# libvips/libvips

Measured on NVIDIA H100. Metric: Mpixels/s for thumbnail(4K->512,lanczos3), higher is better.
Workload: dtype u8

## Files before the change

include/vb200.h:

```cpp
#ifndef VB200_H
#define VB200_H

#include <stddef.h>
#include <stdint.h>

#ifdef __cplusplus
extern "C" {
#endif


typedef enum {
	VB200_FORMAT_UCHAR = 0,
	VB200_FORMAT_CHAR = 1,
	VB200_FORMAT_USHORT = 2,
	VB200_FORMAT_SHORT = 3,
	VB200_FORMAT_UINT = 4,
	VB200_FORMAT_INT = 5,
	VB200_FORMAT_FLOAT = 6,
	VB200_FORMAT_COMPLEX = 7,
	VB200_FORMAT_DOUBLE = 8,
	VB200_FORMAT_DPCOMPLEX = 9
} VB200BandFormat;

typedef enum {
	VB200_INTERPRETATION_MULTIBAND = 0,
	VB200_INTERPRETATION_B_W = 1,
	VB200_INTERPRETATION_CMYK = 15,
	VB200_INTERPRETATION_XYZ = 12,
	VB200_INTERPRETATION_LAB = 13,
	VB200_INTERPRETATION_LCH = 19,
	VB200_INTERPRETATION_LABS = 21,
	VB200_INTERPRETATION_sRGB = 22,
	VB200_INTERPRETATION_YXY = 23,
	VB200_INTERPRETATION_RGB16 = 25,
	VB200_INTERPRETATION_GREY16 = 26,
	VB200_INTERPRETATION_scRGB = 28,
	VB200_INTERPRETATION_HSV = 29
} VB200Interpretation;

typedef enum {
	VB200_KERNEL_NEAREST = 0,
	VB200_KERNEL_LINEAR = 1,
	VB200_KERNEL_CUBIC = 2,
	VB200_KERNEL_MITCHELL = 3,
	VB200_KERNEL_LANCZOS2 = 4,
	VB200_KERNEL_LANCZOS3 = 5,
	VB200_KERNEL_MKS2013 = 6,
	VB200_KERNEL_MKS2021 = 7
} VB200Kernel;

typedef enum {
	VB200_SIZE_BOTH = 0,
	VB200_SIZE_UP = 1,
	VB200_SIZE_DOWN = 2,
	VB200_SIZE_FORCE = 3
} VB200Size;

typedef enum {
	VB200_PRECISION_INTEGER = 0,
	VB200_PRECISION_FLOAT = 1,
	VB200_PRECISION_APPROXIMATE = 2
} VB200Precision;

typedef enum {
	VB200_HOST = 0,
	VB200_DEVICE = 1
} VB200Where;


typedef struct {
	int left;
	int top;
	int width;
	int height;
} VB200Rect;

typedef struct {
	int Xsize;
	int Ysize;
	int Bands;
	int BandFmt;
	int Type;
	int where;
	void *data;
	size_t bpl;
} VB200Image;

typedef struct {
	VB200Image im;
	VB200Rect valid;
	void *data;
	int bpl;
} VB200Region;


int vb200_init(int device);
void vb200_shutdown(void);
const char *vb200_error_buffer(void);
void vb200_error_clear(void);
int vb200_isenabled(void);
void vb200_set_stream(void *cuda_stream);
void *vb200_get_stream(void);
void vb200_set_tile_geometry(int tile_width, int tile_height, int fatstrip_height, int thinstrip_height);
uint64_t vb200_launch_count(void);
void vb200_image_free(VB200Image *image);
size_t vb200_format_sizeof(int band_format);


int vb200_shrinkv(const VB200Image *in, VB200Image *out, int vshrink, int ceil_mode);
int vb200_shrinkh(const VB200Image *in, VB200Image *out, int hshrink, int ceil_mode);
int vb200_reducev(const VB200Image *in, VB200Image *out, double vshrink, int kernel, double gap);
int vb200_reduceh(const VB200Image *in, VB200Image *out, double hshrink, int kernel, double gap);
int vb200_reduce(const VB200Image *in, VB200Image *out, double hshrink, double vshrink, int kernel, double gap);
int vb200_resize(const VB200Image *in, VB200Image *out, double scale, double vscale, int kernel, double gap);
int vb200_premultiply(const VB200Image *in, VB200Image *out, double max_alpha, int uchar_mode);
int vb200_unpremultiply(const VB200Image *in, VB200Image *out, double max_alpha, int uchar_mode);
int vb200_thumbnail_image(const VB200Image *in, VB200Image *out, int width, int height, int size, int linear);

int vb200_colourspace(const VB200Image *in, VB200Image *out, int space);

typedef struct {
	int width;
	int height;
	const double *coeff;
	double scale;
	double offset;
} VB200Mask;

int vb200_conv(const VB200Image *in, VB200Image *out, const VB200Mask *mask, int precision);
int vb200_convsep(const VB200Image *in, VB200Image *out, const VB200Mask *mask, int precision);
int vb200_gaussblur(const VB200Image *in, VB200Image *out, double sigma, double min_ampl, int precision);
int vb200_gaussmat(VB200Mask *out, double sigma, double min_ampl, int separable, int precision);
void vb200_mask_free(VB200Mask *mask);
int vb200_sharpen(const VB200Image *in, VB200Image *out, double sigma, double x1, double y2, double y3, double m1,
	double m2);
int vb200_sharpen_batch_device(const void *in, size_t in_frame_stride, void *out, size_t out_frame_stride, int n_frames, int width,
	int height, int bands, double sigma, double x1, double y2, double y3, double m1, double m2);
void vb200_set_vector_convi(int on);

typedef struct {
	int n_point;
	int kernel;
	double residual_shrink;
	double offset;
} VB200ReduceParams;

int vb200_reducev_gen(const VB200Region *out, const VB200Region *in, const VB200ReduceParams *params);
int vb200_reduceh_gen(const VB200Region *out, const VB200Region *in, const VB200ReduceParams *params);
int vb200_shrinkv_gen(const VB200Region *out, const VB200Region *in, int vshrink);
int vb200_shrinkh_gen(const VB200Region *out, const VB200Region *in, int hshrink);
int vb200_conv_gen(const VB200Region *out, const VB200Region *in, const VB200Mask *mask, int precision);
int vb200_colour_gen(const VB200Region *out, const VB200Region *in, int space);

void vips_reducev_uchar_hwy(uint8_t *pout, uint8_t *pin, int n, int ne, int lskip, const short *k);
void vips_reduceh_uchar_hwy(uint8_t *pout, uint8_t *pin, int n, int width, int bands, short *cs[65], double X,
	double hshrink);
void vips_shrinkh_uchar_hwy(uint8_t *pout, uint8_t *pin, int width, int hshrink, int bands);
void vips_shrinkv_add_line_uchar_hwy(uint8_t *pin, int ne, unsigned int *sum);
void vips_shrinkv_write_line_uchar_hwy(uint8_t *pout, int ne, int vshrink, unsigned int *sum);

typedef struct VB200ThumbnailPlan VB200ThumbnailPlan;

VB200ThumbnailPlan *vb200_thumbnail_plan_new(int width, int height, int bands, int band_format, int has_alpha,
	int target_width, int target_height, int size, int linear);
void vb200_thumbnail_plan_free(VB200ThumbnailPlan *plan);
int vb200_thumbnail_plan_output(const VB200ThumbnailPlan *plan, int *out_width, int *out_height);
int vb200_thumbnail_batch_device(VB200ThumbnailPlan *plan, const void *in, size_t in_frame_stride, void *out,
	size_t out_frame_stride, int n_frames);
int vb200_thumbnail_batch_host(VB200ThumbnailPlan *plan, const void *in, size_t in_frame_stride, void *out,
	size_t out_frame_stride, int n_frames);
int vb200_thumbnail_plan_set_sharpen(VB200ThumbnailPlan *plan, double sigma, double x1, double y2, double y3, double m1, double m2);
int vb200_thumbnail_plan_is_fused(const VB200ThumbnailPlan *plan);
size_t vb200_thumbnail_plan_bytes_per_frame(const VB200ThumbnailPlan *plan);
const char *vb200_thumbnail_plan_kernel(const VB200ThumbnailPlan *plan);

typedef struct {
	const void *input_profile;
	size_t input_len;
	const void *output_profile;
	size_t output_len;
	const void *builtin_rgb;
	size_t builtin_rgb_len;
	const void *builtin_grey;
	size_t builtin_grey_len;
	int intent;
} VB200ThumbnailIcc;

int vb200_thumbnail_plan_set_icc(VB200ThumbnailPlan *plan, const VB200ThumbnailIcc *icc);
int vb200_thumbnail_plan_output_bands(const VB200ThumbnailPlan *plan);
int vb200_thumbnail_batch_device_icc(VB200ThumbnailPlan *plan, const void *in, size_t in_frame_stride, void *out,
	size_t out_frame_stride, int n_frames, const void *const *embedded, const size_t *embedded_lens);
int vb200_thumbnail_batch_host_icc(VB200ThumbnailPlan *plan, const void *in, size_t in_frame_stride, void *out,
	size_t out_frame_stride, int n_frames, const void *const *embedded, const size_t *embedded_lens);
int vb200_thumbnail_image_icc(const VB200Image *in, VB200Image *out, int width, int height, int size, const VB200ThumbnailIcc *icc,
	const void *embedded, size_t embedded_len);
int vb200_thumbnail_buffer_icc(const void *buf, size_t len, VB200Image *out, int width, int height, int size,
	const VB200ThumbnailIcc *icc);
int vb200_thumbnail_plan_set_linear_icc(VB200ThumbnailPlan *plan, const VB200ThumbnailIcc *icc);
int vb200_thumbnail_image_linear_icc(const VB200Image *in, VB200Image *out, int width, int height, int size,
	const VB200ThumbnailIcc *icc, const void *embedded, size_t embedded_len);
int vb200_thumbnail_buffer_linear_icc(const void *buf, size_t len, VB200Image *out, int width, int height, int size,
	const VB200ThumbnailIcc *icc);
int vb200_debug_icc_select_linear(const VB200ThumbnailIcc *icc, int bands, const void *embedded, size_t embedded_len,
	int *branch, int *source, int *export_from);

int vb200_jpeg_icc_profile(const void *buf, size_t len, void *out, size_t cap, size_t *profile_len);

int vb200_debug_hsv_host(const void *in, size_t n, int to_hsv, void *out);

int vb200_flatten(const VB200Image *in, VB200Image *out, const double *background, int n, double max_alpha);
int vb200_debug_flatten_host(const void *in, int width, int height, int bands, int band_format, int interpretation,
	const double *background, int n, double max_alpha, int x4, void *out);

enum { VB200_MORPHOLOGY_ERODE = 0, VB200_MORPHOLOGY_DILATE = 1 };
int vb200_morph(const VB200Image *in, VB200Image *out, const VB200Mask *mask, int morph);
int vb200_rank(const VB200Image *in, VB200Image *out, int width, int height, int index);
int vb200_median(const VB200Image *in, VB200Image *out, int size);
int vb200_debug_rank_host(const void *in, int width, int height, int bands, int band_format, int rank_width, int rank_height,
	int index, void *out);

typedef struct VB200Chain VB200Chain;
VB200Chain *vb200_chain_new(void);
void vb200_chain_free(VB200Chain *chain);
int vb200_chain_add_resize(VB200Chain *chain, double scale, double vscale, int kernel, double gap);
int vb200_chain_add_reduce(VB200Chain *chain, double hshrink, double vshrink, int kernel, double gap);
int vb200_chain_add_colourspace(VB200Chain *chain, int space);
int vb200_chain_add_conv(VB200Chain *chain, const VB200Mask *mask, int precision);
int vb200_chain_add_convsep(VB200Chain *chain, const VB200Mask *mask, int precision);
int vb200_chain_add_gaussblur(VB200Chain *chain, double sigma, double min_ampl, int precision);
int vb200_chain_add_sharpen(VB200Chain *chain, double sigma, double x1, double y2, double y3, double m1, double m2);
int vb200_chain_add_premultiply(VB200Chain *chain, double max_alpha, int uchar_mode);
int vb200_chain_add_unpremultiply(VB200Chain *chain, double max_alpha, int uchar_mode);
int vb200_chain_add_morph(VB200Chain *chain, const VB200Mask *mask, int morph);
int vb200_chain_add_rank(VB200Chain *chain, int width, int height, int index);
int vb200_chain_add_flatten(VB200Chain *chain, const double *background, int n, double max_alpha);
int vb200_chain_run_host(VB200Chain *chain, const VB200Image *in, VB200Image *out, int n_images);

enum { VB200_INTENT_PERCEPTUAL = 0, VB200_INTENT_RELATIVE = 1, VB200_INTENT_SATURATION = 2, VB200_INTENT_ABSOLUTE = 3 };
enum { VB200_PCS_LAB = 0, VB200_PCS_XYZ = 1 };
int vb200_icc_import(const VB200Image *in, VB200Image *out, const void *profile, size_t profile_len, int intent, int pcs);
int vb200_icc_export(const VB200Image *in, VB200Image *out, const void *profile, size_t profile_len, int intent, int depth,
	int pcs);
int vb200_icc_transform(const VB200Image *in, VB200Image *out, const void *in_profile, size_t in_len,
	const void *out_profile, size_t out_len, int intent, int depth);
int vb200_debug_icc_eval(int mode, const void *in, int in_fmt, int in_bands, void *out, int n, const void *pa, size_t la,
	const void *pb, size_t lb, int intent, int depth, int pcs);
int vb200_debug_icc_select(const VB200ThumbnailIcc *icc, int bands, const void *embedded, size_t embedded_len, int *source);
int vb200_debug_icc_classify(const void *profile, size_t len, int want_bands, int intent);
float vb200_debug_icc_stage_ms(void);
float vb200_debug_linear_thumb_ms(void);

int vb200_debug_mma_tables(int in_size, double shrink, int rect_size, int *int_shrink, int *shrunk_size, int *out_size,
	int *n_point, int *embed, int *first, int *phase, short *mask65, int *vchunk, unsigned *bfrag, int cap_rows,
	int *rows_per_chunk);

int vb200_debug_thumbnail_bands(int width, int height, int target_width, int *out_width, int *n_bands, int *xa, int *xb,
	int *c_lo, int *c_hi, int *seam, int cap, int *box_width, int *n_box);
int vb200_debug_thumbnail_kernel(int width, int height, int bands, int has_alpha, int target_width, int target_height, int size,
	char *name, int cap);

int vb200_jpeg_decode_batch(const void *const *bufs, const size_t *lens, int n, int shrink, void *out, int out_location,
	size_t out_bpl, size_t out_frame_stride, int *width, int *height, int *bands);
int vb200_jpegload_buffer(const void *buf, size_t len, int shrink, VB200Image *out);
int vb200_thumbnail_jpegshrink(int width, int height, int target_width, int target_height, int size);
int vb200_thumbnail_buffer(const void *buf, size_t len, VB200Image *out, int width, int height, int size);
int vb200_thumbnail_plan_run_jpeg(VB200ThumbnailPlan *plan, const void *const *bufs, const size_t *lens, int n, int shrink,
	void *out, int out_location, size_t out_frame_stride);
int vb200_debug_jpeg_decode(const void *buf, size_t len, int shrink, void *out, size_t out_bpl, int *width, int *height,
	int *bands);
int vb200_debug_jpeg_decode_sync(const void *buf, size_t len, int shrink, int sub_bytes, int max_passes, void *out, size_t out_bpl,
	int *width, int *height, int *bands, int *passes_used);
int vb200_jpegsave_batch(const void *frames, int frames_location, size_t bpl, size_t frame_stride, int n, int width, int height, int bands,
	int Q, int subsample_mode, void *out, int out_location, size_t out_stride, size_t *lengths);
typedef struct {
	int Q;
	int subsample_mode;
	int optimize_coding;
	int restart_interval;
	int interlace;
} VB200JpegSaveOptions;
int vb200_jpegsave_batch_opts(const void *frames, int frames_location, size_t bpl, size_t frame_stride, int n, int width, int height,
	int bands, const VB200JpegSaveOptions *options, void *out, int out_location, size_t out_stride, size_t *lengths);
int vb200_debug_jpeg_encode(const void *pixels, size_t bpl, int width, int height, int bands, int quality, int subsample_mode, void *out,
	size_t cap, size_t *len);
int vb200_debug_jpeg_encode_opts(const void *pixels, size_t bpl, int width, int height, int bands, const VB200JpegSaveOptions *options,
	void *out, size_t cap, size_t *len);
int vb200_debug_jpeg_prog_events(const void *pixels, size_t bpl, int width, int height, int bands, const VB200JpegSaveOptions *options,
	unsigned long long *events);
int vb200_debug_jpeg_optimal_table(const unsigned *freq, unsigned char *bits, unsigned char *huffval);
void vb200_debug_jpeg_times(float *huffman_ms, float *idct_ms);

enum { VB200_DZ_LAYOUT_DZ = 0, VB200_DZ_LAYOUT_ZOOMIFY = 1, VB200_DZ_LAYOUT_GOOGLE = 2, VB200_DZ_LAYOUT_IIIF = 3, VB200_DZ_LAYOUT_IIIF3 = 4 };
enum { VB200_DZ_DEPTH_DEFAULT = 0, VB200_DZ_DEPTH_ONEPIXEL = 1, VB200_DZ_DEPTH_ONETILE = 2, VB200_DZ_DEPTH_ONE = 3 };
typedef struct {
	int layout;
	int tile_size;
	int overlap;
	int depth;
	int region_shrink;
	int skip_blanks;
	int container;
	const char *suffix;
	VB200JpegSaveOptions jpeg;
} VB200DzOptions;

typedef struct VB200DzPyramid VB200DzPyramid;

int vb200_dzsave(const VB200Image *in, const VB200DzOptions *options, VB200DzPyramid **out);
int vb200_debug_dzsave(const VB200Image *in, const VB200DzOptions *options, VB200DzPyramid **out);
void vb200_dz_free(VB200DzPyramid *pyramid);
int vb200_dz_levels(const VB200DzPyramid *pyramid);
int vb200_dz_level_geometry(const VB200DzPyramid *pyramid, int n, int *width, int *height, int *tiles_across, int *tiles_down);
long vb200_dz_tiles(const VB200DzPyramid *pyramid);
int vb200_dz_tile(const VB200DzPyramid *pyramid, long i, int *level, int *x, int *y, int *left, int *top, int *width, int *height,
	const void **stream, size_t *len);
int vb200_dz_tile_name(const VB200DzPyramid *pyramid, long i, const char *basename, char *name, size_t cap);
int vb200_dz_sidecar(const VB200DzPyramid *pyramid, const char *basename, char *name, size_t ncap, char *text, size_t tcap, size_t *len);
int vb200_dz_pyramid_level(const VB200Image *in, int n_from_top, VB200Image *out);
int vb200_debug_dz_pyramid_level(const void *pixels, size_t bpl, int width, int height, int bands, int n_from_top, void *out);
void vb200_debug_dz_set_budget(size_t bytes);
size_t vb200_debug_dz_pool_used(void);
void vb200_debug_dz_times(float *ms);

void *vb200_host_alloc(size_t bytes);
void vb200_host_free(void *p);
int vb200_device_numa_node(void);

#ifdef __cplusplus
}
#endif

#endif
```

libvips_b200/csrc/thumbnail_fused.cu:

```cuda
#include <algorithm>
#include <climits>
#include <cmath>
#include <cstring>
#include <map>
#include <memory>
#include <mutex>
#include <vector>

#include <cuda.h>

#include "vb200_internal.h"

namespace vb200 {

namespace {

constexpr int kChunkRows = 8;
constexpr int kMaxThreads = 576;

struct FusedParams {
	int W, H;
	size_t in_bpl;
	int VS;
	int Hs;
	int vembed;
	int NPv;
	unsigned vmul8;
	int vshift;
	unsigned accmul;
	int HS, Ws, hembed, NPh;
	unsigned hmul8;
	int hshift;
	int OW, OH;
	size_t out_bpl;
	int TW;
	int RPC;
	int NT;
	int NEmax;
	int slots;
	int stage_pitch;
	int vgrid, hgrid;
	const int2 *vrow;
	const int2 *hcol;
	const int *vcoef;
	const int *hcoef;
	int nvsets, nhsets;
	const int2 *vchunk;
	const uint4 *vbfrag;
	int mma_rows;
	int premul;
	const unsigned char *opaque_hint;
	double max_alpha;
};

struct MmaBand {
	int xa, xb, ne, c_lo, c_hi;
};

__device__ __forceinline__ int
dp2a_lo(unsigned coef, unsigned bytes, int acc)
{
	int d;
	asm("dp2a.lo.s32.u32 %0, %1, %2, %3;" : "=r"(d) : "r"(coef), "r"(bytes), "r"(acc));
	return d;
}

__device__ __forceinline__ int
dp2a_hi(unsigned coef, unsigned bytes, int acc)
{
	int d;
	asm("dp2a.hi.s32.u32 %0, %1, %2, %3;" : "=r"(d) : "r"(coef), "r"(bytes), "r"(acc));
	return d;
}

__device__ __forceinline__ unsigned
ld_stream(const unsigned *p)
{
	unsigned v;
	asm volatile("ld.global.nc.L1::no_allocate.u32 %0, [%1];" : "=r"(v) : "l"(p));
	return v;
}

template <int VS, bool PREMUL>
__device__ __forceinline__ void
box_rows(const unsigned (&px)[VS], int vs, const int *pscale, bool lut, unsigned amend2, unsigned &rb, unsigned &ga)
{
	rb = amend2;
	ga = amend2;
#pragma unroll
	for (int k = 0; k < VS; k++) {
		const unsigned x = px[k];
		if (PREMUL) {
			const unsigned a = x >> 24;
			const unsigned s = lut ? (unsigned) pscale[a] : a + (a == 255u);
			const unsigned prb = (((x & 0x00ff00ffu) * s + 0x00800080u) >> 8) & 0x00ff00ffu;
			const unsigned pg = ((((x >> 8) & 0xffu) * s + 128u) >> 8) & 0xffu;
			rb += prb;
			ga += pg + (a << 16);
		}
		else {
			rb += x & 0x00ff00ffu;
			ga += (x >> 8) & 0x00ff00ffu;
		}
	}
}

__device__ __forceinline__ unsigned
box_average(unsigned lanes, unsigned mul8, int shift)
{
	if (shift >= 0)
		return (lanes >> shift) & 0x00ff00ffu;
	const unsigned lo = __umulhi(lanes & 0xffffu, mul8);
	const unsigned hi = __umulhi(lanes >> 16, mul8);
	return lo | (hi << 16);
}

template <int VS, bool PREMUL>
__global__ void __launch_bounds__(kMaxThreads, 2)
thumbnail_fused_kernel(const __grid_constant__ FusedParams P, const uint8_t *__restrict__ in, size_t in_frame_stride,
	uint8_t *__restrict__ out, size_t out_frame_stride, int frame0)
{
	extern __shared__ __align__(128) unsigned char smem_raw[];

	const int NT = P.NT;
	const int t = threadIdx.x;
	const int vs = VS > 0 ? VS : P.VS;

	uint2 *pairbuf = (uint2 *) smem_raw;
	unsigned *rv = (unsigned *) (pairbuf + (size_t) P.slots * NT);
	uint2 *sh = (uint2 *) (rv + (size_t) kChunkRows * NT);
	int *vcoef = (int *) (sh + (size_t) kChunkRows * (P.NEmax / 2));
	int *hcoef = vcoef + P.nvsets * P.NPv;
	int *pscale = hcoef + P.nhsets * P.NPh;
	int *uscale = pscale + 256;

	for (int i = t; i < P.nvsets * P.NPv; i += NT)
		vcoef[i] = P.vcoef[i];
	for (int i = t; i < P.nhsets * P.NPh; i += NT)
		hcoef[i] = P.hcoef[i];
	if (PREMUL)
		for (int i = t; i < 256; i += NT) {
			const double clip = fmax(0.0, fmin(P.max_alpha, (double) i));
			pscale[i] = (int) __ddiv_rn(__dmul_rn(256.0, clip), P.max_alpha);
			uscale[i] = clip == 0 ? 0 : (int) __ddiv_rn(__dmul_rn(256.0, P.max_alpha), clip);
		}
	const bool lut = PREMUL && P.max_alpha != 255.0;

	const int xa = blockIdx.x * P.TW;
	const int xb = min(xa + P.TW, P.OW);
	const int y_begin = blockIdx.y * P.RPC;
	const int y_end = min(y_begin + P.RPC, P.OH);
	const int frame = frame0 + blockIdx.z;
	const uint8_t *fin = in + (size_t) frame * in_frame_stride;
	uint8_t *fout = out + (size_t) frame * out_frame_stride;

	const int pair_h0 = __ldg(&P.hcol[xa]).x;
	const int E0 = 2 * pair_h0 + P.hgrid;
	const int NE = 2 * (__ldg(&P.hcol[xb - 1]).x + P.NPh - pair_h0);

	const bool col_active = t < NE * P.HS;
	int in_col;
	{
		const int e = E0 + t / P.HS;
		const int k = t - (t / P.HS) * P.HS;
		const int sc = max(0, min(e - P.hembed, P.Ws - 1));
		in_col = min(sc * P.HS + k, P.W - 1);
	}
	const unsigned *col_ptr = (const unsigned *) fin + in_col;

	const unsigned amend2 = (unsigned) (vs / 2) * 0x00010001u;

	__syncthreads();

	int pdone = INT_MIN;
	int P0_prev = 0;

	for (int ya = y_begin; ya < y_end; ya += kChunkRows) {
		const int yb = min(ya + kChunkRows, y_end);
		const int P0 = __ldg(&P.vrow[ya]).x;
		const int P1 = __ldg(&P.vrow[yb - 1]).x + P.NPv - 1;

		if (col_active) {
			int pfirst = P0;
			if (pdone > P0) {
				const int shift = P0 - P0_prev;
				if (shift > 0)
					for (int p = P0; p < pdone; p++)
						pairbuf[(size_t) (p - P0) * NT + t] = pairbuf[(size_t) (p - P0 + shift) * NT + t];
				pfirst = pdone;
			}

			for (int p = pfirst; p <= P1; p++) {
				unsigned rbA, gaA, rbB, gaB;
				const int sA = max(0, min(2 * p + P.vgrid - P.vembed, P.Hs - 1));
				const int sB = max(0, min(2 * p + P.vgrid + 1 - P.vembed, P.Hs - 1));
				if (VS > 0) {
					unsigned pa[VS > 0 ? VS : 1], pb[VS > 0 ? VS : 1];
#pragma unroll
					for (int k = 0; k < VS; k++) {
						const int ra = min(sA * VS + k, P.H - 1);
						const int rb_ = min(sB * VS + k, P.H - 1);
						pa[k] = ld_stream((const unsigned *) ((const char *) col_ptr + (size_t) ra * P.in_bpl));
						pb[k] = ld_stream((const unsigned *) ((const char *) col_ptr + (size_t) rb_ * P.in_bpl));
					}
					box_rows<(VS > 0 ? VS : 1), PREMUL>(pa, vs, pscale, lut, amend2, rbA, gaA);
					box_rows<(VS > 0 ? VS : 1), PREMUL>(pb, vs, pscale, lut, amend2, rbB, gaB);
				}
				else {
					rbA = gaA = rbB = gaB = amend2;
					for (int k = 0; k < vs; k++) {
						unsigned one[1], rb1, ga1;
						one[0] = ld_stream((const unsigned *) ((const char *) col_ptr + (size_t) min(sA * vs + k, P.H - 1) * P.in_bpl));
						box_rows<1, PREMUL>(one, 1, pscale, lut, 0u, rb1, ga1);
						rbA += rb1;
						gaA += ga1;
						one[0] = ld_stream((const unsigned *) ((const char *) col_ptr + (size_t) min(sB * vs + k, P.H - 1) * P.in_bpl));
						box_rows<1, PREMUL>(one, 1, pscale, lut, 0u, rb1, ga1);
						rbB += rb1;
						gaB += ga1;
					}
				}
				rbA = box_average(rbA, P.vmul8, P.vshift);
				gaA = box_average(gaA, P.vmul8, P.vshift);
				rbB = box_average(rbB, P.vmul8, P.vshift);
				gaB = box_average(gaB, P.vmul8, P.vshift);
				uint2 w;
				w.x = __byte_perm(rbA, rbB, 0x6240);
				w.y = __byte_perm(gaA, gaB, 0x6240);
				pairbuf[(size_t) (p - P0) * NT + t] = w;
			}

			for (int y = ya; y < yb; y++) {
				const int2 vr = __ldg(&P.vrow[y]);
				const uint2 *win = pairbuf + (size_t) (vr.x - P0) * NT + t;
				const int *cf = vcoef + vr.y * P.NPv;
				int r = VB200_INTERPOLATE_SCALE >> 1, g = r, b = r, a = r;
#pragma unroll 7
				for (int k = 0; k < P.NPv; k++) {
					const uint2 w = win[(size_t) k * NT];
					const unsigned c = (unsigned) cf[k];
					r = dp2a_lo(c, w.x, r);
					b = dp2a_hi(c, w.x, b);
					g = dp2a_lo(c, w.y, g);
					a = dp2a_hi(c, w.y, a);
				}
				r = max(0, min(r >> VB200_INTERPOLATE_SHIFT, 255));
				g = max(0, min(g >> VB200_INTERPOLATE_SHIFT, 255));
				b = max(0, min(b >> VB200_INTERPOLATE_SHIFT, 255));
				a = max(0, min(a >> VB200_INTERPOLATE_SHIFT, 255));
				rv[(size_t) (y - ya) * NT + t] = (unsigned) r | ((unsigned) g << 8) | ((unsigned) b << 16) | ((unsigned) a << 24);
			}
		}
		pdone = P1 + 1;
		P0_prev = P0;

		__syncthreads();

		const int rows = yb - ya;
		const int npairs = NE / 2;
		const unsigned hamend2 = (unsigned) (P.HS / 2) * 0x00010001u;
		for (int idx = t; idx < rows * npairs; idx += NT) {
			const int k = idx / npairs;
			const int j = idx - k * npairs;
			const unsigned *src = rv + (size_t) k * NT + (size_t) (2 * j) * P.HS;
			unsigned rbA = hamend2, gaA = hamend2, rbB = hamend2, gaB = hamend2;
			for (int i = 0; i < P.HS; i++) {
				const unsigned wA = src[i];
				const unsigned wB = src[P.HS + i];
				rbA += wA & 0x00ff00ffu;
				gaA += (wA >> 8) & 0x00ff00ffu;
				rbB += wB & 0x00ff00ffu;
				gaB += (wB >> 8) & 0x00ff00ffu;
			}
			rbA = box_average(rbA, P.hmul8, P.hshift);
			gaA = box_average(gaA, P.hmul8, P.hshift);
			rbB = box_average(rbB, P.hmul8, P.hshift);
			gaB = box_average(gaB, P.hmul8, P.hshift);
			uint2 w;
			w.x = __byte_perm(rbA, rbB, 0x6240);
			w.y = __byte_perm(gaA, gaB, 0x6240);
			sh[(size_t) k * (P.NEmax / 2) + j] = w;
		}

		__syncthreads();

		const int bw = xb - xa;
		for (int idx = t; idx < rows * bw; idx += NT) {
			const int k = idx / bw;
			const int x = xa + (idx - k * bw);
			const int2 hc = __ldg(&P.hcol[x]);
			const uint2 *win = sh + (size_t) k * (P.NEmax / 2) + (hc.x - pair_h0);
			const int *cf = hcoef + hc.y * P.NPh;
			int r = VB200_INTERPOLATE_SCALE >> 1, g = r, b = r, a = r;
#pragma unroll 7
			for (int kk = 0; kk < P.NPh; kk++) {
				const uint2 w = win[kk];
				const unsigned c = (unsigned) cf[kk];
				r = dp2a_lo(c, w.x, r);
				b = dp2a_hi(c, w.x, b);
				g = dp2a_lo(c, w.y, g);
				a = dp2a_hi(c, w.y, a);
			}
			r = max(0, min(r >> VB200_INTERPOLATE_SHIFT, 255));
			g = max(0, min(g >> VB200_INTERPOLATE_SHIFT, 255));
			b = max(0, min(b >> VB200_INTERPOLATE_SHIFT, 255));
			a = max(0, min(a >> VB200_INTERPOLATE_SHIFT, 255));
			if (PREMUL) {
				const int s = uscale[a];
				r = ((r * s + 128) >> 8) & 0xff;
				g = ((g * s + 128) >> 8) & 0xff;
				b = ((b * s + 128) >> 8) & 0xff;
			}
			*(unsigned *) (fout + (size_t) (ya + k) * P.out_bpl + (size_t) x * 4) =
				(unsigned) r | ((unsigned) g << 8) | ((unsigned) b << 16) | ((unsigned) a << 24);
		}
	}
}


constexpr int kStages = 3;
constexpr int kChunkRowsTma = 4;
constexpr int kColsPerThread = 2;
constexpr int kStagePitch = (kMaxThreads + 8) * 4;

__device__ __forceinline__ unsigned
smem_addr(const void *p)
{
	return (unsigned) __cvta_generic_to_shared(p);
}

__device__ __forceinline__ void
mbar_init(unsigned bar, unsigned count)
{
	asm volatile("mbarrier.init.shared::cta.b64 [%0], %1;" ::"r"(bar), "r"(count));
}

__device__ __forceinline__ void
mbar_wait(unsigned bar, unsigned parity)
{
	unsigned done;
	do {
		asm volatile("{\n\t.reg .pred p;\n\t"
					 "mbarrier.try_wait.parity.shared::cta.b64 p, [%1], %2, 0x989680;\n\t"
					 "selp.u32 %0, 1, 0, p;\n\t}"
					 : "=r"(done)
					 : "r"(bar), "r"(parity)
					 : "memory");
	} while (!done);
}

__device__ __forceinline__ void
mbar_arrive(unsigned bar)
{
	asm volatile("{\n\t.reg .b64 st;\n\tmbarrier.arrive.shared::cta.b64 st, [%0];\n\t}" ::"r"(bar) : "memory");
}

__device__ __forceinline__ void
mbar_expect_tx(unsigned bar, unsigned bytes)
{
	asm volatile("{\n\t.reg .b64 st;\n\tmbarrier.arrive.expect_tx.shared::cta.b64 st, [%0], %1;\n\t}" ::"r"(bar), "r"(bytes)
				 : "memory");
}

__device__ __forceinline__ void
bulk_copy_g2s(unsigned dst, const void *src, unsigned bytes, unsigned bar)
{
	asm volatile("cp.async.bulk.shared::cluster.global.mbarrier::complete_tx::bytes [%0], [%1], %2, [%3];" ::"r"(dst),
				 "l"(src), "r"(bytes), "r"(bar)
				 : "memory");
}

__device__ __forceinline__ int
fast_div(int idx, int d)
{
	int q = (int) (__int2float_rn(idx) * __frcp_rn(__int2float_rn(d)));
	const int r = idx - q * d;
	q += (r >= d) - (r < 0);
	return q;
}

__device__ __forceinline__ void
consumer_barrier(int n_threads)
{
	asm volatile("bar.sync 1, %0;" ::"r"(n_threads) : "memory");
}

template <bool PREMUL>
__device__ __forceinline__ void
accumulate_pixel(unsigned x, unsigned &rb, unsigned &ga)
{
	if (PREMUL) {
		const unsigned a = x >> 24;
		const unsigned s = (a * 257u + 1u) >> 8;
		const unsigned trb = (x & 0x00ff00ffu) * s + 0x00800080u;
		const unsigned tg = __byte_perm(x, 0, 0x4441) * s + 128u;
		rb += __byte_perm(trb, 0, 0x4341);
		ga += __byte_perm(tg, x, 0x3731);
	}
	else {
		rb += x & 0x00ff00ffu;
		ga += __byte_perm(x, 0, 0x4341);
	}
}

__device__ __forceinline__ unsigned
average_pair(unsigned lanesA, unsigned lanesB, unsigned mul8, int shift)
{
	if (shift >= 0)
		return __byte_perm(lanesA >> shift, lanesB >> shift, 0x6240);
	const unsigned a = __umulhi(lanesA & 0xffffu, mul8) | (__umulhi(lanesA >> 16, mul8) << 16);
	const unsigned b = __umulhi(lanesB & 0xffffu, mul8) | (__umulhi(lanesB >> 16, mul8) << 16);
	return __byte_perm(a, b, 0x6240);
}

__device__ __forceinline__ unsigned
hadd2_lanes(unsigned a, unsigned b)
{
	unsigned d;
	asm("add.f16x2 %0, %1, %2;" : "=r"(d) : "r"(a), "r"(b));
	return d;
}

template <bool PREMUL>
__device__ __forceinline__ void
accumulate_pixel_h(unsigned x, unsigned k16, unsigned &rb, unsigned &ga)
{
	if (PREMUL) {
		unsigned t0;
		asm("lop3.b32 %0, %1, 0xff000000, %2, 0xea;" : "=r"(t0) : "r"(x), "r"(k16));
		const unsigned s = __umulhi(t0, 257u);
		const unsigned trb = (x & 0x00ff00ffu) * s + 0x00800080u;
		const unsigned tg = (x & 0x0000ff00u) * s + 0x00008000u;
		rb = hadd2_lanes(rb, __byte_perm(trb, 0, 0x4341));
		ga = hadd2_lanes(ga, __byte_perm(tg, x, 0x3732));
	}
	else {
		rb = hadd2_lanes(rb, x & 0x00ff00ffu);
		ga = hadd2_lanes(ga, __byte_perm(x, 0, 0x4341));
	}
}

__device__ __forceinline__ unsigned
finalize_pack(int r, int g, int b, int a)
{
	r = max(0, min(r >> VB200_INTERPOLATE_SHIFT, 255));
	g = max(0, min(g >> VB200_INTERPOLATE_SHIFT, 255));
	b = max(0, min(b >> VB200_INTERPOLATE_SHIFT, 255));
	a = max(0, min(a >> VB200_INTERPOLATE_SHIFT, 255));
	return (unsigned) r + (unsigned) g * 256u + (unsigned) b * 65536u + (unsigned) a * 16777216u;
}

template <int VS, int NP, bool PREMUL, int CPT>
__global__ void __launch_bounds__(kMaxThreads / CPT + 32, 2)
thumbnail_fused_tma_kernel(const __grid_constant__ FusedParams P, const uint8_t *__restrict__ in, size_t in_frame_stride,
	uint8_t *__restrict__ out, size_t out_frame_stride, int frame0)
{
	extern __shared__ __align__(128) unsigned char smem_raw[];

	constexpr int K = kChunkRowsTma;
	constexpr int NPR = NP > 0 ? NP : 1;
	constexpr int VSR = VS > 0 ? VS : 1;
	const int NT = P.NT;
	const int NC = NT * CPT;
	const int t = threadIdx.x;
	const int vs = VS > 0 ? VS : P.VS;
	const int NPv = NP > 0 ? NP : P.NPv;
	const int NPh = NP > 0 ? NP : P.NPh;
	const int rows_per_stage = 2 * vs;
	const unsigned stage_bytes = (unsigned) rows_per_stage * kStagePitch;

	unsigned char *stages = smem_raw;
	uint64_t *bars = (uint64_t *) (smem_raw + kStages * stage_bytes);
	uint2 *pairbuf = (uint2 *) (bars + 2 * kStages);
	unsigned *rv = (unsigned *) (pairbuf + (size_t) P.slots * NC);
	uint2 *sh = (uint2 *) (rv + (size_t) K * NC);
	int *vcoef = (int *) (sh + (size_t) K * (P.NEmax / 2));
	int *hcoef = vcoef + P.nvsets * P.NPv;
	int *uscale = hcoef + P.nhsets * P.NPh;

	const unsigned stages_s = smem_addr(stages);
	const unsigned full_s = smem_addr(bars);
	const unsigned empty_s = full_s + 8u * kStages;

	if (t == 0) {
		for (int i = 0; i < kStages; i++) {
			mbar_init(full_s + 8u * i, 1);
			mbar_init(empty_s + 8u * i, NT / 32);
		}
		asm volatile("fence.mbarrier_init.release.cluster;" ::: "memory");
	}
	for (int i = t; i < P.nvsets * P.NPv; i += blockDim.x)
		vcoef[i] = P.vcoef[i];
	for (int i = t; i < P.nhsets * P.NPh; i += blockDim.x)
		hcoef[i] = P.hcoef[i];
	if (PREMUL)
		for (int i = t; i < 256; i += blockDim.x)
			uscale[i] = i == 0 ? 0 : (int) __ddiv_rn(__dmul_rn(256.0, 255.0), (double) i);

	const int xa = blockIdx.x * P.TW;
	const int xb = min(xa + P.TW, P.OW);
	const int y_begin = blockIdx.y * P.RPC;
	const int y_end = min(y_begin + P.RPC, P.OH);
	const int frame = frame0 + blockIdx.z;
	const uint8_t *fin = in + (size_t) frame * in_frame_stride;
	uint8_t *fout = out + (size_t) frame * out_frame_stride;

	const int pair_h0 = __ldg(&P.hcol[xa]).x;
	const int E0 = 2 * pair_h0 + P.hgrid;
	const int NE = 2 * (__ldg(&P.hcol[xb - 1]).x + P.NPh - pair_h0);

	auto column_of = [&](int tt) {
		const int e = E0 + tt / P.HS;
		const int k = tt - (tt / P.HS) * P.HS;
		const int sc = max(0, min(e - P.hembed, P.Ws - 1));
		return min(sc * P.HS + k, P.W - 1);
	};
	const int c_lo = column_of(0) & ~3;
	const int c_hi = min(P.W, (column_of(NE * P.HS - 1) + 4) & ~3);
	const unsigned row_bytes = (unsigned) (c_hi - c_lo) * 4u;

	__syncthreads();

	if (t >= NT) {
		const int lane = t - NT;
		const uint8_t *src0 = fin + (size_t) c_lo * 4;
		const int j = lane / vs, k = lane - j * vs;
		const bool copier = lane < rows_per_stage;
		int s = 0;
		unsigned phase = 0;
		int pdone = INT_MIN;
		for (int ya = y_begin; ya < y_end; ya += K) {
			const int yb = min(ya + K, y_end);
			const int P0 = __ldg(&P.vrow[ya]).x;
			const int P1 = __ldg(&P.vrow[yb - 1]).x + P.NPv - 1;
			for (int p = max(pdone, P0); p <= P1; p++) {
				mbar_wait(empty_s + 8u * s, phase ^ 1u);
				if (lane == 0)
					mbar_expect_tx(full_s + 8u * s, (unsigned) rows_per_stage * row_bytes);
				__syncwarp();
				if (copier) {
					const int sr = max(0, min(2 * p + P.vgrid + j - P.vembed, P.Hs - 1));
					const int row = min(sr * vs + k, P.H - 1);
					bulk_copy_g2s(stages_s + (unsigned) s * stage_bytes + (unsigned) lane * kStagePitch,
						src0 + (size_t) row * P.in_bpl, row_bytes, full_s + 8u * s);
				}
				if (++s == kStages) {
					s = 0;
					phase ^= 1u;
				}
			}
			pdone = P1 + 1;
		}
		return;
	}

	const unsigned char *my_col[CPT];
#pragma unroll
	for (int i = 0; i < CPT; i++)
		my_col[i] = stages + (size_t) (column_of(min(t * CPT + i, NE * P.HS - 1)) - c_lo) * 4u;
	const unsigned amend2 = (unsigned) (vs / 2) * 0x00010001u;
	const bool lane0 = (t & 31) == 0;
	const unsigned vmul8 = P.vmul8;
	const int vshift = VS == 1 ? 0 : VS == 2 ? 1 : VS == 4 ? 2 : VS == 8 ? 3 : P.vshift;
	const int tc = t * CPT;

	int s = 0;
	unsigned phase = 0;
	int pdone = INT_MIN;
	int P0_prev = 0;
	int cset = -1;
	unsigned cf[NPR];

	for (int ya = y_begin; ya < y_end; ya += K) {
		const int yb = min(ya + K, y_end);
		const int P0 = __ldg(&P.vrow[ya]).x;
		const int P1 = __ldg(&P.vrow[yb - 1]).x + P.NPv - 1;

		int pfirst = P0;
		if (pdone > P0) {
			const int shift = P0 - P0_prev;
			if (shift > 0) {
				const int cnt = pdone - P0;
				uint2 *dstp = pairbuf + tc;
				const uint2 *srcp = pairbuf + shift * NC + tc;
#pragma unroll 4
				for (int i = 0; i < cnt; i++) {
					if (CPT == 2)
						*(uint4 *) (dstp + i * NC) = *(const uint4 *) (srcp + i * NC);
					else
						dstp[i * NC] = srcp[i * NC];
				}
			}
			pfirst = pdone;
		}

		uint2 *pdst = pairbuf + (pfirst - P0) * NC + tc;
		for (int p = pfirst; p <= P1; p++, pdst += NC) {
			const unsigned soff = (unsigned) s * stage_bytes;
			unsigned rbA[CPT], gaA[CPT], rbB[CPT], gaB[CPT];
#pragma unroll
			for (int i = 0; i < CPT; i++)
				rbA[i] = gaA[i] = rbB[i] = gaB[i] = amend2;
			mbar_wait(full_s + 8u * s, phase);
			if (VS > 0) {
				unsigned pa[CPT][VSR], pb[CPT][VSR];
#pragma unroll
				for (int i = 0; i < CPT; i++)
#pragma unroll
					for (int k = 0; k < VSR; k++) {
						pa[i][k] = *(const unsigned *) (my_col[i] + soff + k * kStagePitch);
						pb[i][k] = *(const unsigned *) (my_col[i] + soff + (VSR + k) * kStagePitch);
					}
				__syncwarp();
				if (lane0)
					mbar_arrive(empty_s + 8u * s);
#pragma unroll
				for (int i = 0; i < CPT; i++)
#pragma unroll
					for (int k = 0; k < VSR; k++) {
						accumulate_pixel<PREMUL>(pa[i][k], rbA[i], gaA[i]);
						accumulate_pixel<PREMUL>(pb[i][k], rbB[i], gaB[i]);
					}
			}
			else {
				for (int k = 0; k < vs; k++)
#pragma unroll
					for (int i = 0; i < CPT; i++) {
						accumulate_pixel<PREMUL>(*(const unsigned *) (my_col[i] + soff + k * kStagePitch), rbA[i], gaA[i]);
						accumulate_pixel<PREMUL>(*(const unsigned *) (my_col[i] + soff + (vs + k) * kStagePitch), rbB[i], gaB[i]);
					}
				__syncwarp();
				if (lane0)
					mbar_arrive(empty_s + 8u * s);
			}
			if (++s == kStages) {
				s = 0;
				phase ^= 1u;
			}
			uint2 w[CPT];
#pragma unroll
			for (int i = 0; i < CPT; i++) {
				w[i].x = average_pair(rbA[i], rbB[i], vmul8, vshift);
				w[i].y = average_pair(gaA[i], gaB[i], vmul8, vshift);
			}
			if (CPT == 2)
				*(uint4 *) pdst = make_uint4(w[0].x, w[0].y, w[CPT - 1].x, w[CPT - 1].y);
			else
				*pdst = w[0];
		}

		unsigned *rvp = rv + tc;
		for (int y = ya; y < yb; y++, rvp += NC) {
			const int2 vr = __ldg(&P.vrow[y]);
			const uint2 *win = pairbuf + (vr.x - P0) * NC + tc;
			int acc[CPT][4];
#pragma unroll
			for (int i = 0; i < CPT; i++)
				acc[i][0] = acc[i][1] = acc[i][2] = acc[i][3] = VB200_INTERPOLATE_SCALE >> 1;
			if (NP > 0) {
				if (vr.y != cset) {
					cset = vr.y;
#pragma unroll
					for (int k = 0; k < NPR; k++)
						cf[k] = (unsigned) vcoef[cset * NPR + k];
				}
#pragma unroll
				for (int k = 0; k < NPR; k++) {
					uint2 w[CPT];
					if (CPT == 2) {
						const uint4 q = *(const uint4 *) (win + k * NC);
						w[0] = make_uint2(q.x, q.y);
						w[CPT - 1] = make_uint2(q.z, q.w);
					}
					else
						w[0] = win[k * NC];
#pragma unroll
					for (int i = 0; i < CPT; i++) {
						acc[i][0] = dp2a_lo(cf[k], w[i].x, acc[i][0]);
						acc[i][2] = dp2a_hi(cf[k], w[i].x, acc[i][2]);
						acc[i][1] = dp2a_lo(cf[k], w[i].y, acc[i][1]);
						acc[i][3] = dp2a_hi(cf[k], w[i].y, acc[i][3]);
					}
				}
			}
			else {
				const int *cfp = vcoef + vr.y * NPv;
				for (int k = 0; k < NPv; k++) {
					const unsigned c = (unsigned) cfp[k];
#pragma unroll
					for (int i = 0; i < CPT; i++) {
						const uint2 w = win[k * NC + i];
						acc[i][0] = dp2a_lo(c, w.x, acc[i][0]);
						acc[i][2] = dp2a_hi(c, w.x, acc[i][2]);
						acc[i][1] = dp2a_lo(c, w.y, acc[i][1]);
						acc[i][3] = dp2a_hi(c, w.y, acc[i][3]);
					}
				}
			}
			if (CPT == 2)
				*(uint2 *) rvp = make_uint2(finalize_pack(acc[0][0], acc[0][1], acc[0][2], acc[0][3]),
					finalize_pack(acc[CPT - 1][0], acc[CPT - 1][1], acc[CPT - 1][2], acc[CPT - 1][3]));
			else
				*rvp = finalize_pack(acc[0][0], acc[0][1], acc[0][2], acc[0][3]);
		}
		pdone = P1 + 1;
		P0_prev = P0;

		consumer_barrier(NT);

		const int rows = yb - ya;
		const int npairs = NE / 2;
		const unsigned hamend2 = (unsigned) (P.HS / 2) * 0x00010001u;
		for (int idx = t; idx < rows * npairs; idx += NT) {
			const int k = fast_div(idx, npairs);
			const int j = idx - k * npairs;
			const unsigned *src = rv + k * NC + (2 * j) * P.HS;
			unsigned rbA = hamend2, gaA = hamend2, rbB = hamend2, gaB = hamend2;
			if (P.HS == 4) {
				const uint4 A = *(const uint4 *) src;
				const uint4 B = *(const uint4 *) (src + 4);
				rbA += (A.x & 0x00ff00ffu) + (A.y & 0x00ff00ffu) + (A.z & 0x00ff00ffu) + (A.w & 0x00ff00ffu);
				gaA += __byte_perm(A.x, 0, 0x4341) + __byte_perm(A.y, 0, 0x4341) + __byte_perm(A.z, 0, 0x4341) +
					__byte_perm(A.w, 0, 0x4341);
				rbB += (B.x & 0x00ff00ffu) + (B.y & 0x00ff00ffu) + (B.z & 0x00ff00ffu) + (B.w & 0x00ff00ffu);
				gaB += __byte_perm(B.x, 0, 0x4341) + __byte_perm(B.y, 0, 0x4341) + __byte_perm(B.z, 0, 0x4341) +
					__byte_perm(B.w, 0, 0x4341);
			}
			else
				for (int i = 0; i < P.HS; i++) {
					const unsigned wA = src[i];
					const unsigned wB = src[P.HS + i];
					rbA += wA & 0x00ff00ffu;
					gaA += __byte_perm(wA, 0, 0x4341);
					rbB += wB & 0x00ff00ffu;
					gaB += __byte_perm(wB, 0, 0x4341);
				}
			uint2 w;
			w.x = average_pair(rbA, rbB, P.hmul8, P.hshift);
			w.y = average_pair(gaA, gaB, P.hmul8, P.hshift);
			sh[k * (P.NEmax / 2) + j] = w;
		}

		consumer_barrier(NT);

		const int bw = xb - xa;
		for (int idx = t; idx < rows * bw; idx += NT) {
			const int k = fast_div(idx, bw);
			const int x = xa + (idx - k * bw);
			const int2 hc = __ldg(&P.hcol[x]);
			const uint2 *win = sh + k * (P.NEmax / 2) + (hc.x - pair_h0);
			const int *cfp = hcoef + hc.y * NPh;
			int r = VB200_INTERPOLATE_SCALE >> 1, g = r, b = r, a = r;
			if (NP > 0) {
#pragma unroll
				for (int kk = 0; kk < NPR; kk++) {
					const uint2 w = win[kk];
					const unsigned c = (unsigned) cfp[kk];
					r = dp2a_lo(c, w.x, r);
					b = dp2a_hi(c, w.x, b);
					g = dp2a_lo(c, w.y, g);
					a = dp2a_hi(c, w.y, a);
				}
			}
			else
				for (int kk = 0; kk < NPh; kk++) {
					const uint2 w = win[kk];
					const unsigned c = (unsigned) cfp[kk];
					r = dp2a_lo(c, w.x, r);
					b = dp2a_hi(c, w.x, b);
					g = dp2a_lo(c, w.y, g);
					a = dp2a_hi(c, w.y, a);
				}
			r = max(0, min(r >> VB200_INTERPOLATE_SHIFT, 255));
			g = max(0, min(g >> VB200_INTERPOLATE_SHIFT, 255));
			b = max(0, min(b >> VB200_INTERPOLATE_SHIFT, 255));
			a = max(0, min(a >> VB200_INTERPOLATE_SHIFT, 255));
			if (PREMUL) {
				const int sc = uscale[a];
				r = ((r * sc + 128) >> 8) & 0xff;
				g = ((g * sc + 128) >> 8) & 0xff;
				b = ((b * sc + 128) >> 8) & 0xff;
			}
			*(unsigned *) (fout + (size_t) (ya + k) * P.out_bpl + (size_t) x * 4) =
				(unsigned) r | ((unsigned) g << 8) | ((unsigned) b << 16) | ((unsigned) a << 24);
		}
	}
}

#include "thumbnail_fused_mma.cuh"

#define VB200_V4_LIST(X) \
	X(4, 6, 4) X(4, 7, 4) X(2, 6, 2) X(2, 7, 2) X(8, 6, 8) X(8, 7, 8) \
	X(4, 0, 4) X(2, 0, 2) X(4, 0, 2) X(2, 0, 4) X(4, 0, 8) X(2, 0, 8) X(8, 0, 8) X(8, 0, 4) \
	X(3, 0, 3) X(5, 0, 5) X(6, 0, 6) X(7, 0, 7) X(2, 0, 3) X(3, 0, 2) X(3, 0, 4) X(4, 0, 3) \
	X(4, 0, 5) X(5, 0, 4) X(5, 0, 6) X(6, 0, 5) X(6, 0, 7) X(7, 0, 6) X(7, 0, 8) X(8, 0, 7)

int
v4_np(int vs, int nph, int hs)
{
	int np = -1;
#define X(VS_, NP_, HS_) \
	if (vs == VS_ && hs == HS_ && (NP_ == nph || (NP_ == 0 && np < 0))) \
		np = NP_;
	VB200_V4_LIST(X)
#undef X
	return np;
}

struct PairSets {
	int NP = 0;
	std::vector<int> coef;
	std::map<std::pair<int, int>, int> ids;

	int
	get(const AxisTable &t, int phase, int parity)
	{
		auto key = std::make_pair(phase, parity);
		auto it = ids.find(key);
		if (it != ids.end())
			return it->second;
		const int id = (int) ids.size();
		ids[key] = id;
		const short *c = &t.ms[(size_t) phase * t.n_point];
		for (int k = 0; k < NP; k++) {
			const int i0 = 2 * k - parity, i1 = 2 * k + 1 - parity;
			const int c0 = (i0 >= 0 && i0 < t.n_point) ? c[i0] : 0;
			const int c1 = (i1 >= 0 && i1 < t.n_point) ? c[i1] : 0;
			coef.push_back((int) (((unsigned) (c0 & 0xffff)) | ((unsigned) (c1 & 0xffff) << 16)));
		}
		return id;
	}

	void
	trim()
	{
		const int nsets = (int) ids.size();
		int keep = 1;
		for (int s = 0; s < nsets; s++)
			for (int k = 0; k < NP; k++)
				if (coef[(size_t) s * NP + k] != 0)
					keep = std::max(keep, k + 1);
		if (keep == NP)
			return;
		std::vector<int> packed;
		for (int s = 0; s < nsets; s++)
			for (int k = 0; k < keep; k++)
				packed.push_back(coef[(size_t) s * NP + k]);
		coef.swap(packed);
		NP = keep;
	}
};

}


struct LinearThumb;
int linear_thumb_new(const char *domain, int W, int H, int bands, bool premul, const ReduceGeom &gv, const ReduceGeom &gh,
	const AxisTable &tv, const AxisTable &th, LinearThumb **out);
int linear_thumb_run(const char *domain, LinearThumb *lt, const void *in, size_t in_stride, void *out, size_t out_stride, int n,
	cudaStream_t s, const LinIccBatch *icc = nullptr, int out_bands = 0);
void linear_thumb_free(LinearThumb *lt);

enum class FusedKernel {
	Ldg,
	Tma,
	Mma,
};

struct ThumbnailPlanImpl {
	int W = 0, H = 0, bands = 0, fmt = 0, has_alpha = 0;
	int target_w = 0, target_h = 0, size = 0, linear = 0;
	double hshrink = 1, vshrink = 1;
	int OW = 0, OH = 0;
	ReduceGeom gv{}, gh{};
	bool premul = false;
	bool fused = false;
	int device = -1;
	FusedKernel kernel = FusedKernel::Ldg;
	FusedParams fp{};
	void *tables = nullptr;
	size_t smem = 0;
	int slots_tma = 0;
	size_t smem_tma = 0;
	int mma_tw = 0, mma_nt = 0, mma_nemax = 0;
	std::vector<MmaBand> mma_bands;
	size_t smem_mma = 0;
	bool geometry_only = false;
	void *tables_mma = nullptr;
	static constexpr int kStreams = 3;
	cudaStream_t streams[kStreams] = {nullptr, nullptr, nullptr};
	void *stage_in[kStreams] = {nullptr, nullptr, nullptr};
	void *stage_out[kStreams] = {nullptr, nullptr, nullptr};
	cudaEvent_t drained[kStreams] = {nullptr, nullptr, nullptr};
	int stage_frames = 0;
	std::mutex pump_lock;
	static constexpr int kHintSlots = 4;
	std::mutex hint_lock;
	int *hint_counts = nullptr;
	cudaEvent_t hint_done[kHintSlots] = {nullptr, nullptr, nullptr, nullptr};
	bool hint_pending[kHintSlots] = {false, false, false, false};
	unsigned hint_slot_seq[kHintSlots] = {0, 0, 0, 0};
	unsigned hint_seq = 0, hint_seen = 0;
	bool opaque_mode = false;
	bool rgb_expand = false;
	LinearThumb *lin = nullptr;
	bool sharpen = false;
	double sh_sigma = 0.5, sh_x1 = 2.0, sh_y2 = 10.0, sh_y3 = 20.0, sh_m1 = 0.0, sh_m2 = 3.0;
	IccStage *icc = nullptr;
	int icc_bands = 0;
	IccStage *licc = nullptr;
	int licc_bands = 0;
	size_t stage_out_frame = 0;
	int out_bands() const { return icc ? icc_bands : licc ? licc_bands : bands; }
};

int dev_sharpen_fused(const char *domain, const void *in, size_t in_bpl, size_t in_frame_stride, void *out, size_t out_bpl,
	size_t out_frame_stride, int n_frames, int w, int h, int bands, double sigma, double x1, double y2, double y3, double m1,
	double m2, cudaStream_t s);

namespace {

void
thumbnail_shrink(int w, int h, int tw, int th, int size, double *hshrink, double *vshrink)
{
	double hs = (double) w / tw;
	double vs = (double) h / th;
	const bool horizontal = !(hs < vs);
	if (size != VB200_SIZE_FORCE) {
		if (horizontal)
			vs = hs;
		else
			hs = vs;
	}
	if (size == VB200_SIZE_UP) {
		hs = std::min(1.0, hs);
		vs = std::min(1.0, vs);
	}
	else if (size == VB200_SIZE_DOWN) {
		hs = std::max(1.0, hs);
		vs = std::max(1.0, vs);
	}
	*hshrink = std::min(hs, (double) w);
	*vshrink = std::min(vs, (double) h);
}

int
launch_status(const char *domain, const char *what)
{
	const cudaError_t e = cudaGetLastError();
	if (e != cudaSuccess)
		return cuda_fail(domain, e, what);
	count_launch();
	return 0;
}

int
rows_per_cta(int OH, int k, int min_chunks, int bands_x, int n, int ctas)
{
	int rpc = ((OH + k - 1) / k) * k;
	while ((long long) bands_x * ((OH + rpc - 1) / rpc) * n < ctas && rpc > min_chunks * k)
		rpc = ((rpc / 2 + k - 1) / k) * k;
	return rpc;
}

template <int VS, bool PREMUL>
int
launch_ldg_t(const char *domain, const FusedParams &fp, size_t smem, const void *in, size_t in_stride, void *out,
	size_t out_stride, int f0, dim3 grid, cudaStream_t s)
{
	auto kern = thumbnail_fused_kernel<VS, PREMUL>;
	VB200_CUDA(domain, cudaFuncSetAttribute(kern, cudaFuncAttributeMaxDynamicSharedMemorySize, (int) smem));
	kern<<<grid, fp.NT, smem, s>>>(fp, (const uint8_t *) in, in_stride, (uint8_t *) out, out_stride, f0);
	return launch_status(domain, "thumbnail_fused_kernel launch");
}

template <bool PREMUL>
int
launch_ldg_vs(const char *domain, const FusedParams &fp, size_t smem, const void *in, size_t is, void *out, size_t os, int f0,
	dim3 grid, cudaStream_t s)
{
	switch (fp.VS) {
	case 1: return launch_ldg_t<1, PREMUL>(domain, fp, smem, in, is, out, os, f0, grid, s);
	case 2: return launch_ldg_t<2, PREMUL>(domain, fp, smem, in, is, out, os, f0, grid, s);
	case 3: return launch_ldg_t<3, PREMUL>(domain, fp, smem, in, is, out, os, f0, grid, s);
	case 4: return launch_ldg_t<4, PREMUL>(domain, fp, smem, in, is, out, os, f0, grid, s);
	case 5: return launch_ldg_t<5, PREMUL>(domain, fp, smem, in, is, out, os, f0, grid, s);
	case 6: return launch_ldg_t<6, PREMUL>(domain, fp, smem, in, is, out, os, f0, grid, s);
	case 8: return launch_ldg_t<8, PREMUL>(domain, fp, smem, in, is, out, os, f0, grid, s);
	default: return launch_ldg_t<0, PREMUL>(domain, fp, smem, in, is, out, os, f0, grid, s);
	}
}

int
launch_ldg(const char *domain, const ThumbnailPlanImpl *pl, const void *in, size_t is, void *out, size_t os, int n, int f0,
	int nf, cudaStream_t s)
{
	FusedParams fp = pl->fp;
	const int bands_x = (pl->OW + fp.TW - 1) / fp.TW;
	fp.RPC = rows_per_cta(pl->OH, kChunkRows, 2, bands_x, n, 2 * sm_count());
	const dim3 grid(bands_x, (pl->OH + fp.RPC - 1) / fp.RPC, nf);
	return pl->premul ? launch_ldg_vs<true>(domain, fp, pl->smem, in, is, out, os, f0, grid, s)
					  : launch_ldg_vs<false>(domain, fp, pl->smem, in, is, out, os, f0, grid, s);
}

template <int VS, int NP, bool PREMUL>
int
launch_tma_t(const char *domain, const FusedParams &fp, size_t smem, const void *in, size_t in_stride, void *out,
	size_t out_stride, int f0, dim3 grid, cudaStream_t s)
{
	auto kern = thumbnail_fused_tma_kernel<VS, NP, PREMUL, kColsPerThread>;
	VB200_CUDA(domain, cudaFuncSetAttribute(kern, cudaFuncAttributeMaxDynamicSharedMemorySize, (int) smem));
	kern<<<grid, fp.NT + 32, smem, s>>>(fp, (const uint8_t *) in, in_stride, (uint8_t *) out, out_stride, f0);
	return launch_status(domain, "thumbnail_fused_tma_kernel launch");
}

template <int NP, bool PREMUL>
int
launch_tma_vs(const char *domain, const FusedParams &fp, size_t smem, const void *in, size_t is, void *out, size_t os, int f0,
	dim3 grid, cudaStream_t s)
{
	switch (fp.VS) {
	case 1: return launch_tma_t<1, NP, PREMUL>(domain, fp, smem, in, is, out, os, f0, grid, s);
	case 2: return launch_tma_t<2, NP, PREMUL>(domain, fp, smem, in, is, out, os, f0, grid, s);
	case 3: return launch_tma_t<3, NP, PREMUL>(domain, fp, smem, in, is, out, os, f0, grid, s);
	case 4: return launch_tma_t<4, NP, PREMUL>(domain, fp, smem, in, is, out, os, f0, grid, s);
	case 8: return launch_tma_t<8, NP, PREMUL>(domain, fp, smem, in, is, out, os, f0, grid, s);
	default: return launch_tma_t<0, NP, PREMUL>(domain, fp, smem, in, is, out, os, f0, grid, s);
	}
}

int
launch_tma(const char *domain, const ThumbnailPlanImpl *pl, const void *in, size_t is, void *out, size_t os, int n, int f0,
	int nf, cudaStream_t s)
{
	FusedParams fp = pl->fp;
	fp.slots = pl->slots_tma;
	fp.NT = ((pl->fp.NT / kColsPerThread + 31) / 32) * 32;
	const int bands_x = (pl->OW + fp.TW - 1) / fp.TW;
	fp.RPC = rows_per_cta(pl->OH, kChunkRowsTma, 4, bands_x, n, 2 * sm_count());
	const dim3 grid(bands_x, (pl->OH + fp.RPC - 1) / fp.RPC, nf);
	const size_t smem = pl->smem_tma;
	const int np = fp.NPv == fp.NPh ? fp.NPv : 0;
	if (np == 6)
		return pl->premul ? launch_tma_vs<6, true>(domain, fp, smem, in, is, out, os, f0, grid, s)
						  : launch_tma_vs<6, false>(domain, fp, smem, in, is, out, os, f0, grid, s);
	if (np == 7)
		return pl->premul ? launch_tma_vs<7, true>(domain, fp, smem, in, is, out, os, f0, grid, s)
						  : launch_tma_vs<7, false>(domain, fp, smem, in, is, out, os, f0, grid, s);
	return pl->premul ? launch_tma_vs<0, true>(domain, fp, smem, in, is, out, os, f0, grid, s)
					  : launch_tma_vs<0, false>(domain, fp, smem, in, is, out, os, f0, grid, s);
}

bool
make_stage_tensor_map(CUtensorMap *tm, const void *in, int W, int H, size_t in_bpl, size_t frame_stride, int frames,
	int box_cols, int box_rows)
{
	typedef CUresult (*encode_fn)(CUtensorMap *, CUtensorMapDataType, cuuint32_t, void *, const cuuint64_t *,
		const cuuint64_t *, const cuuint32_t *, const cuuint32_t *, CUtensorMapInterleave, CUtensorMapSwizzle,
		CUtensorMapL2promotion, CUtensorMapFloatOOBfill);
	static encode_fn encode = nullptr;
	static bool tried = false;
	if (!tried) {
		tried = true;
		void *fn = nullptr;
		cudaDriverEntryPointQueryResult qres;
		if (cudaGetDriverEntryPoint("cuTensorMapEncodeTiled", &fn, cudaEnableDefault, &qres) == cudaSuccess &&
			qres == cudaDriverEntryPointSuccess)
			encode = (encode_fn) fn;
		cudaGetLastError();
	}
	if (!encode || getenv("VB200_NO_TENSORMAP"))
		return false;
	if ((W & 1) || (in_bpl % 16) || (frame_stride % 16) || ((uintptr_t) in % 16) || box_cols / 2 > 256 || box_rows > 256)
		return false;
	const cuuint64_t dims[3] = {(cuuint64_t) W / 2, (cuuint64_t) H, (cuuint64_t) frames};
	const cuuint64_t strides[2] = {(cuuint64_t) in_bpl, (cuuint64_t) frame_stride};
	const cuuint32_t box[3] = {(cuuint32_t) box_cols / 2, (cuuint32_t) box_rows, 1};
	const cuuint32_t estr[3] = {1, 1, 1};
	return encode(tm, CU_TENSOR_MAP_DATA_TYPE_UINT64, 3, const_cast<void *>(in), dims, strides, box, estr,
			   CU_TENSOR_MAP_INTERLEAVE_NONE, CU_TENSOR_MAP_SWIZZLE_NONE, CU_TENSOR_MAP_L2_PROMOTION_L2_256B,
			   CU_TENSOR_MAP_FLOAT_OOB_FILL_NONE) == CUDA_SUCCESS;
}

constexpr int kHintThreads = 128, kHintSamples = 2;

__global__ void __launch_bounds__(kHintThreads)
alpha_hint_kernel(const uint8_t *__restrict__ in, size_t in_frame_stride, size_t in_bpl, int W, int H, unsigned char *__restrict__ hint,
	int *__restrict__ count)
{
	const uint8_t *f = in + (size_t) blockIdx.x * in_frame_stride;
	const unsigned npix = (unsigned) W * (unsigned) H;
	int opaque = 0;
#pragma unroll
	for (int i = 0; i < kHintSamples; i++) {
		const unsigned k = (unsigned) (threadIdx.x * kHintSamples + i);
		const unsigned p = (unsigned) (((unsigned long long) (k * 2654435761u) * npix) >> 32);
		const unsigned y = p / (unsigned) W, x = p - y * (unsigned) W;
		opaque += f[(size_t) y * in_bpl + (size_t) x * 4 + 3] == 255;
	}
	__shared__ int s_sum;
	if (threadIdx.x == 0)
		s_sum = 0;
	__syncthreads();
	opaque = __reduce_add_sync(0xffffffffu, opaque);
	if ((threadIdx.x & 31) == 0)
		atomicAdd(&s_sum, opaque);
	__syncthreads();
	if (threadIdx.x == 0) {
		const int h = s_sum * 4 >= kHintThreads * kHintSamples ? 1 : 0;
		hint[blockIdx.x] = (unsigned char) h;
		if (h)
			atomicAdd(count, 1);
	}
}

int
opaque_hint_begin(const char *domain, ThumbnailPlanImpl *pl, const FusedParams &fp, const void *in, size_t in_stride, int n,
	cudaStream_t s, void **hint, bool *use_opq)
{
	*hint = nullptr;
	*use_opq = false;
	const char *probe_env = getenv("VB200_OPAQUE_PROBE");
	if (!pl->premul || (probe_env && probe_env[0] == '0'))
		return 0;
	{
		std::lock_guard<std::mutex> lock(pl->hint_lock);
		if (!pl->hint_counts) {
			if (cudaHostAlloc((void **) &pl->hint_counts, sizeof(int) * ThumbnailPlanImpl::kHintSlots, cudaHostAllocDefault) != cudaSuccess) {
				cudaGetLastError();
				pl->hint_counts = nullptr;
				return 0;
			}
			for (int i = 0; i < ThumbnailPlanImpl::kHintSlots; i++)
				cudaEventCreateWithFlags(&pl->hint_done[i], cudaEventDisableTiming);
		}
		for (int i = 0; i < ThumbnailPlanImpl::kHintSlots; i++)
			if (pl->hint_pending[i] && cudaEventQuery(pl->hint_done[i]) == cudaSuccess) {
				pl->hint_pending[i] = false;
				if (pl->hint_slot_seq[i] + 1 > pl->hint_seen) {
					pl->hint_seen = pl->hint_slot_seq[i] + 1;
					pl->opaque_mode = pl->hint_counts[i] > 0;
				}
			}
		cudaGetLastError();
		*use_opq = pl->opaque_mode || (probe_env && probe_env[0] == '2');
	}
	const size_t count_off = ((size_t) n + 3) & ~(size_t) 3;
	if (dev_alloc(domain, hint, count_off + sizeof(int), s))
		return -1;
	int *count = (int *) ((char *) *hint + count_off);
	VB200_CUDA(domain, cudaMemsetAsync(count, 0, sizeof(int), s));
	alpha_hint_kernel<<<n, kHintThreads, 0, s>>>((const uint8_t *) in, in_stride, fp.in_bpl, fp.W, fp.H, (unsigned char *) *hint, count);
	cudaError_t e = cudaGetLastError();
	if (e != cudaSuccess) {
		dev_free(*hint, s);
		*hint = nullptr;
		return cuda_fail(domain, e, "alpha_hint_kernel launch");
	}
	count_launch();
	return 0;
}

void
opaque_hint_end(ThumbnailPlanImpl *pl, void *hint, int n, cudaStream_t s)
{
	if (!hint)
		return;
	{
		std::lock_guard<std::mutex> lock(pl->hint_lock);
		const int slot = (int) (pl->hint_seq % ThumbnailPlanImpl::kHintSlots);
		if (!pl->hint_pending[slot]) {
			const int *count = (const int *) ((const char *) hint + (((size_t) n + 3) & ~(size_t) 3));
			if (cudaMemcpyAsync(&pl->hint_counts[slot], count, sizeof(int), cudaMemcpyDeviceToHost, s) == cudaSuccess &&
				cudaEventRecord(pl->hint_done[slot], s) == cudaSuccess) {
				pl->hint_pending[slot] = true;
				pl->hint_slot_seq[slot] = pl->hint_seq;
			}
			cudaGetLastError();
		}
		pl->hint_seq++;
	}
	dev_free(hint, s);
}

template <int VS, int NP, bool PREMUL, int HSQ, bool OPQ>
int
launch_mma_k(const char *domain, const ThumbnailPlanImpl *pl, const FusedParams &fp, const CUtensorMap &tm, int use_tmap, const void *in,
	size_t in_stride, void *out, size_t out_stride, int f0, dim3 grid, cudaStream_t s)
{
	auto kern = thumbnail_fused_mma_kernel<VS, NP, PREMUL, HSQ, OPQ>;
	VB200_CUDA(domain, cudaFuncSetAttribute(kern, cudaFuncAttributeMaxDynamicSharedMemorySize, (int) pl->smem_mma));
	kern<<<grid, fp.NT + 32 * kV4HWarps + 32, pl->smem_mma, s>>>(fp, tm, use_tmap, (const uint8_t *) in, in_stride,
		(uint8_t *) out, out_stride, f0);
	return launch_status(domain, "thumbnail_fused_mma_kernel launch");
}

template <int VS, int NP, bool PREMUL, int HSQ>
int
launch_mma_t(const char *domain, ThumbnailPlanImpl *pl, FusedParams fp, const void *in, size_t in_stride, void *out,
	size_t out_stride, int n, int f0, dim3 grid, cudaStream_t s)
{
	CUtensorMap tm;
	memset(&tm, 0, sizeof(tm));
	const int use_tmap = make_stage_tensor_map(&tm, in, fp.W, fp.H, fp.in_bpl, in_stride, n, v4_boxw(HSQ), 2 * VS) ? 1 : 0;
	void *hint = nullptr;
	bool use_opq = false;
	if (PREMUL && opaque_hint_begin(domain, pl, fp, (const uint8_t *) in + (size_t) f0 * in_stride, in_stride, (int) grid.z, s, &hint, &use_opq))
		return -1;
	fp.opaque_hint = (const unsigned char *) hint;
	int rc;
	if constexpr (PREMUL)
		rc = use_opq ? launch_mma_k<VS, NP, PREMUL, HSQ, true>(domain, pl, fp, tm, use_tmap, in, in_stride, out, out_stride, f0, grid, s)
					 : launch_mma_k<VS, NP, PREMUL, HSQ, false>(domain, pl, fp, tm, use_tmap, in, in_stride, out, out_stride, f0, grid, s);
	else
		rc = launch_mma_k<VS, NP, PREMUL, HSQ, false>(domain, pl, fp, tm, use_tmap, in, in_stride, out, out_stride, f0, grid, s);
	opaque_hint_end(pl, hint, (int) grid.z, s);
	return rc;
}

template <bool PREMUL>
int
launch_mma_list(const char *domain, ThumbnailPlanImpl *pl, const FusedParams &fp, const void *in, size_t is, void *out, size_t os,
	int n, int f0, dim3 grid, cudaStream_t s)
{
	const int np = v4_np(fp.VS, fp.NPh, fp.HS);
#define X(VS_, NP_, HS_) \
	if (fp.VS == VS_ && np == NP_ && fp.HS == HS_) \
		return launch_mma_t<VS_, NP_, PREMUL, HS_>(domain, pl, fp, in, is, out, os, n, f0, grid, s);
	VB200_V4_LIST(X)
#undef X
	error(domain, "the tensor-pipe kernel has no instantiation for VS %d, HS %d", fp.VS, fp.HS);
	return -1;
}

int
launch_mma(const char *domain, ThumbnailPlanImpl *pl, const void *in, size_t is, void *out, size_t os, int n, int f0, int nf,
	cudaStream_t s)
{
	FusedParams fp = pl->fp;
	fp.TW = pl->mma_tw;
	fp.NT = pl->mma_nt;
	fp.NEmax = pl->mma_nemax;
	const int bands_x = (pl->OW + fp.TW - 1) / fp.TW;
	fp.RPC = rows_per_cta(pl->OH, fp.mma_rows, 4, bands_x, n, sm_count());
	const dim3 grid(bands_x, (pl->OH + fp.RPC - 1) / fp.RPC, nf);
	return pl->premul ? launch_mma_list<true>(domain, pl, fp, in, is, out, os, n, f0, grid, s)
					  : launch_mma_list<false>(domain, pl, fp, in, is, out, os, n, f0, grid, s);
}

void
plan_axis_tables(const ThumbnailPlanImpl *pl, AxisTable &tv, AxisTable &th)
{
	const TileGeometry tg = tile_geometry();
	int tile_w, tile_h;
	if (pl->gv.int_shrink > 1) {
		tile_w = tg.tile_width;
		tile_h = tg.tile_height;
	}
	else {
		tile_w = pl->OW;
		tile_h = tg.fatstrip_height;
	}
	int rect_h = tile_h;
	if (pl->gh.int_shrink > 1)
		rect_h = std::min(rect_h, tg.fatstrip_height);
	build_axis_table(tv, pl->OH, pl->gv.residual, pl->gv.offset, pl->gv.n_point, VB200_KERNEL_LANCZOS3, rect_h);
	build_axis_table(th, pl->OW, pl->gh.residual, pl->gh.offset, pl->gh.n_point, VB200_KERNEL_LANCZOS3, tile_w);
}

std::vector<MmaBand>
mma_bands_of(const FusedParams &fp, const std::vector<int2> &hcol, int tw, int clo_align)
{
	auto column_of = [&](int E0, int tt) {
		const int e = E0 + tt / fp.HS;
		const int k = tt % fp.HS;
		const int sc = std::max(0, std::min(e - fp.hembed, fp.Ws - 1));
		return std::min(sc * fp.HS + k, fp.W - 1);
	};
	std::vector<MmaBand> bands;
	for (int xa = 0; xa < fp.OW; xa += tw) {
		MmaBand b;
		b.xa = xa;
		b.xb = std::min(xa + tw, fp.OW);
		const int E0 = 2 * hcol[xa].x + fp.hgrid;
		b.ne = 2 * (hcol[b.xb - 1].x + fp.NPh - hcol[xa].x);
		b.c_lo = column_of(E0, 0) & ~(clo_align - 1);
		b.c_hi = std::min(fp.W, (column_of(E0, b.ne * fp.HS - 1) + 4) & ~3);
		bands.push_back(b);
	}
	return bands;
}

int
plan_build_fused(const char *domain, ThumbnailPlanImpl *pl)
{
	AxisTable tv, th;
	plan_axis_tables(pl, tv, th);

	auto build_sets = [](const AxisTable &t, int count, int grid, PairSets &sets, std::vector<int2> &idx) {
		sets = PairSets();
		sets.NP = (t.n_point + 2) / 2;
		idx.resize(count);
		for (int i = 0; i < count; i++) {
			const int rel = t.first[i] - grid;
			idx[i].x = rel >> 1;
			idx[i].y = sets.get(t, t.phase[i], rel & 1);
		}
		sets.trim();
	};
	PairSets sv, shh;
	std::vector<int2> vrow, hcol;
	int vgrid = 0, hgrid = 0;
	{
		PairSets alt;
		std::vector<int2> alt_idx;
		build_sets(tv, pl->OH, 0, sv, vrow);
		build_sets(tv, pl->OH, 1, alt, alt_idx);
		if (alt.NP < sv.NP) {
			sv = alt;
			vrow = alt_idx;
			vgrid = 1;
		}
		build_sets(th, pl->OW, 0, shh, hcol);
		build_sets(th, pl->OW, 1, alt, alt_idx);
		if (alt.NP < shh.NP) {
			shh = alt;
			hcol = alt_idx;
			hgrid = 1;
		}
	}

	FusedParams &fp = pl->fp;
	fp.W = pl->W;
	fp.H = pl->H;
	fp.in_bpl = (size_t) pl->W * 4;
	fp.VS = pl->gv.int_shrink;
	fp.Hs = pl->gv.shrunk_size;
	fp.vembed = tv.embed;
	fp.NPv = sv.NP;
	fp.vgrid = vgrid;
	fp.hgrid = hgrid;
	fp.vmul8 = (unsigned) (((1LL << 32) / (256LL * fp.VS)) << 8);
	fp.vshift = -1;
	fp.accmul = 1;
	for (int sft = 0; sft < 9; sft++)
		if ((1 << sft) == fp.VS) {
			fp.vshift = sft;
			fp.accmul = 256u >> sft;
		}
	fp.HS = pl->gh.int_shrink;
	fp.Ws = pl->gh.shrunk_size;
	fp.hembed = th.embed;
	fp.NPh = shh.NP;
	fp.hmul8 = (unsigned) (((1LL << 32) / (256LL * fp.HS)) << 8);
	fp.hshift = -1;
	for (int sft = 0; sft < 9; sft++)
		if ((1 << sft) == fp.HS)
			fp.hshift = sft;
	fp.OW = pl->OW;
	fp.OH = pl->OH;
	fp.out_bpl = (size_t) pl->OW * 4;
	fp.premul = pl->premul;
	fp.max_alpha = 255.0;
	fp.opaque_hint = nullptr;
	fp.nvsets = (int) sv.ids.size();
	fp.nhsets = (int) shh.ids.size();
	if (fp.VS > 256 || fp.HS > 256)
		return 1;

	int TW = 64;
	auto band_threads = [&](int tw, int *nemax) {
		int worst = 0;
		for (int xa = 0; xa < pl->OW; xa += tw) {
			const int xb = std::min(xa + tw, pl->OW);
			const int ne = 2 * (hcol[xb - 1].x + fp.NPh) - 2 * hcol[xa].x;
			worst = std::max(worst, ne);
		}
		*nemax = worst;
		return worst * fp.HS;
	};
	int nemax = 0;
	while (TW > 4 && band_threads(TW, &nemax) > kMaxThreads)
		TW /= 2;
	if (band_threads(TW, &nemax) > kMaxThreads)
		return 1;
	fp.TW = TW;
	fp.NEmax = nemax;
	fp.NT = std::min(kMaxThreads, ((nemax * fp.HS + 31) / 32) * 32);
	fp.NT = std::max(fp.NT, 64);

	int slots = 0;
	for (int ya = 0; ya < pl->OH; ya += kChunkRows) {
		const int yb = std::min(ya + kChunkRows, pl->OH);
		slots = std::max(slots, vrow[yb - 1].x + fp.NPv - 1 - vrow[ya].x + 1);
	}
	fp.slots = slots;

	pl->smem = (size_t) slots * fp.NT * 8 + (size_t) kChunkRows * fp.NT * 4 + (size_t) kChunkRows * (nemax / 2) * 8 +
		(size_t) (fp.nvsets * fp.NPv + fp.nhsets * fp.NPh + 512) * 4;
	if (pl->smem > 200 * 1024)
		return 1;

	pl->kernel = FusedKernel::Ldg;
	if ((fp.in_bpl % 16) == 0 && fp.VS <= 16) {
		int slots2 = 0;
		for (int ya = 0; ya < pl->OH; ya += kChunkRowsTma) {
			const int yb = std::min(ya + kChunkRowsTma, pl->OH);
			slots2 = std::max(slots2, vrow[yb - 1].x + fp.NPv - 1 - vrow[ya].x + 1);
		}
		int max_cols = 0;
		for (const MmaBand &b : mma_bands_of(fp, hcol, TW, 4))
			max_cols = std::max(max_cols, b.c_hi - b.c_lo);
		fp.stage_pitch = kStagePitch;
		pl->slots_tma = slots2;
		const int nc = ((fp.NT / kColsPerThread + 31) / 32) * 32 * kColsPerThread;
		pl->smem_tma = (size_t) kStages * 2 * fp.VS * kStagePitch + 2 * kStages * 8 + (size_t) slots2 * nc * 8 +
			(size_t) kChunkRowsTma * nc * 4 + (size_t) kChunkRowsTma * (nemax / 2) * 8 +
			(size_t) (fp.nvsets * fp.NPv + fp.nhsets * fp.NPh + 256) * 4;
		if (max_cols * 4 <= kStagePitch && pl->smem_tma <= 113 * 1024 && fp.max_alpha == 255.0)
			pl->kernel = FusedKernel::Tma;
	}

	const bool hpow2 = fp.HS == 2 || fp.HS == 4 || fp.HS == 8;
	const bool pairs_aligned = !hpow2 || fp.Ws * fp.HS <= fp.W;
	if ((fp.in_bpl % 16) == 0 && fp.max_alpha == 255.0 && pairs_aligned && v4_np(fp.VS, fp.NPh, fp.HS) >= 0) {
		std::vector<int> vchunk_flat;
		std::vector<unsigned> bfrag_flat;
		const int K = pick_mma_rows(tv, pl->OH, vchunk_flat, bfrag_flat);
		bool ok = K > 0;
		fp.mma_rows = K;
		const int chunks = ok ? (pl->OH + K - 1) / K : 0;
		std::vector<int2> vchunk(chunks);
		std::vector<uint4> bfrag((size_t) chunks * 32);
		if (ok) {
			memcpy(vchunk.data(), vchunk_flat.data(), vchunk.size() * sizeof(int2));
			memcpy(bfrag.data(), bfrag_flat.data(), bfrag.size() * sizeof(uint4));
		}
		const int warp_cols = hpow2 ? 0 : 2 * (32 / fp.HS) * fp.HS;
		const int pitch = v4_nbox(fp.HS) * v4_boxw(fp.HS) * 4;
		int tw4 = 0, nemax4 = 0;
		long best_cost = LONG_MAX;
		const int cols_per_warp = warp_cols ? warp_cols : 32 * kV4Cpt;
		const int col_budget = warp_cols ? (kV4Cols / (32 * kV4Cpt)) * warp_cols : kV4Cols;
		for (int tw = std::min(pl->OW, 256); tw >= 2 && ok; tw--) {
			int worst = 0, max_cols = 0;
			long cost = 0;
			for (const MmaBand &b : mma_bands_of(fp, hcol, tw, v4_clo_align(fp.HS))) {
				worst = std::max(worst, b.ne);
				max_cols = std::max(max_cols, b.c_hi - b.c_lo);
				cost += (b.ne * fp.HS + cols_per_warp - 1) / cols_per_warp + 1;
			}
			if (worst * fp.HS <= col_budget && max_cols * 4 <= pitch && cost < best_cost) {
				best_cost = cost;
				tw4 = tw;
				nemax4 = worst;
			}
		}
		if (ok && tw4 > 0) {
			pl->mma_tw = tw4;
			pl->mma_nemax = nemax4;
			pl->mma_nt = warp_cols ? std::max(64, ((nemax4 * fp.HS + warp_cols - 1) / warp_cols) * 32)
								   : std::max(64, ((nemax4 * fp.HS / kV4Cpt + 31) / 32) * 32);
			const int stages = fp.VS <= 2 ? 2 * VB200_V4_STAGES
				: (fp.VS >= 7 ? VB200_V4_STAGES / 2 : (fp.VS >= 5 ? (3 * VB200_V4_STAGES) / 4 : VB200_V4_STAGES));
			const int logical_cols = warp_cols ? (pl->mma_nt / 32) * warp_cols : pl->mma_nt * kV4Cpt;
			pl->mma_bands = mma_bands_of(fp, hcol, tw4, v4_clo_align(fp.HS));
			const int nbox = v4_nbox(fp.HS);
			const size_t box_bytes = ((size_t) 2 * fp.VS * (pitch / nbox) + 127) & ~(size_t) 127;
			pl->smem_mma = (size_t) stages * nbox * box_bytes + (2 * stages + 4) * 8 +
				(size_t) kV4Quads * ((size_t) pl->mma_nt * kV4Cpt * 16 + 16) +
				(size_t) 2 * kV4Rows * ((logical_cols / fp.HS + 1) / 2) * 8 +
				(size_t) (fp.nhsets * fp.NPh + 256) * 4;
			const size_t n_ch = vchunk.size() * sizeof(int2), n_bf = bfrag.size() * sizeof(uint4);
			if (pl->smem_mma <= 226 * 1024) {
				if (!pl->geometry_only) {
					VB200_CUDA(domain, cudaMalloc(&pl->tables_mma, n_bf + n_ch));
					VB200_CUDA(domain, cudaMemcpy(pl->tables_mma, bfrag.data(), n_bf, cudaMemcpyHostToDevice));
					VB200_CUDA(domain, cudaMemcpy((char *) pl->tables_mma + n_bf, vchunk.data(), n_ch, cudaMemcpyHostToDevice));
					fp.vbfrag = (const uint4 *) pl->tables_mma;
					fp.vchunk = (const int2 *) ((char *) pl->tables_mma + n_bf);
				}
				pl->kernel = FusedKernel::Mma;
			}
		}
	}
	if (pl->geometry_only)
		return 0;

	const size_t n_vrow = vrow.size() * sizeof(int2), n_hcol = hcol.size() * sizeof(int2);
	const size_t n_vc = sv.coef.size() * 4, n_hc = shh.coef.size() * 4;
	std::vector<char> host(n_vrow + n_hcol + n_vc + n_hc);
	memcpy(&host[0], vrow.data(), n_vrow);
	memcpy(&host[n_vrow], hcol.data(), n_hcol);
	memcpy(&host[n_vrow + n_hcol], sv.coef.data(), n_vc);
	memcpy(&host[n_vrow + n_hcol + n_vc], shh.coef.data(), n_hc);
	VB200_CUDA(domain, cudaMalloc(&pl->tables, host.size()));
	VB200_CUDA(domain, cudaMemcpy(pl->tables, host.data(), host.size(), cudaMemcpyHostToDevice));
	char *b = (char *) pl->tables;
	fp.vrow = (const int2 *) b;
	fp.hcol = (const int2 *) (b + n_vrow);
	fp.vcoef = (const int *) (b + n_vrow + n_hcol);
	fp.hcoef = (const int *) (b + n_vrow + n_hcol + n_vc);
	return 0;
}

}

namespace {

__global__ void __launch_bounds__(256)
rgb_expand_kernel(const uint8_t *__restrict__ in, size_t in_stride, uint8_t *__restrict__ out, size_t out_stride, size_t quads)
{
	const size_t q = (size_t) blockIdx.x * blockDim.x + threadIdx.x;
	if (q >= quads)
		return;
	const unsigned *p = (const unsigned *) (in + (size_t) blockIdx.y * in_stride) + q * 3;
	const unsigned w0 = __ldg(p), w1 = __ldg(p + 1), w2 = __ldg(p + 2);
	uint4 o;
	o.x = (w0 & 0x00ffffffu) | 0xff000000u;
	o.y = (w0 >> 24) | ((w1 & 0xffffu) << 8) | 0xff000000u;
	o.z = (w1 >> 16) | ((w2 & 0xffu) << 16) | 0xff000000u;
	o.w = (w2 >> 8) | 0xff000000u;
	((uint4 *) (out + (size_t) blockIdx.y * out_stride))[q] = o;
}

__global__ void __launch_bounds__(256)
rgbx_compact_kernel(const uint8_t *__restrict__ in, size_t in_stride, uint8_t *__restrict__ out, size_t out_stride, size_t pixels)
{
	const size_t i = (size_t) blockIdx.x * blockDim.x + threadIdx.x;
	if (i >= pixels)
		return;
	const unsigned px = __ldg((const unsigned *) (in + (size_t) blockIdx.y * in_stride) + i);
	uint8_t *q = out + (size_t) blockIdx.y * out_stride + i * 3;
	q[0] = (uint8_t) px;
	q[1] = (uint8_t) (px >> 8);
	q[2] = (uint8_t) (px >> 16);
}

}

int
thumbnail_plan_init(const char *domain, ThumbnailPlanImpl *pl)
{
	if (pl->fmt != VB200_FORMAT_UCHAR) {
		error(domain, "only uchar frames are on the batched device path");
		return -1;
	}
	thumbnail_shrink(pl->W, pl->H, pl->target_w, pl->target_h, pl->size, &pl->hshrink, &pl->vshrink);
	if (pl->linear && (pl->bands < 3 || pl->hshrink < 1.0 || pl->vshrink < 1.0)) {
		error(domain, pl->bands < 3 ? "linear thumbnails on the device path need an 8-bit image with 3+ bands"
									: "upsizing is not on the device path yet");
		return -1;
	}
	if (pl->hshrink < 1.0 || pl->vshrink < 1.0) {
		const double hscale = std::max(1.0 / pl->hshrink, 1.0 / pl->W);
		const double vscale = std::max(1.0 / pl->vshrink, 1.0 / pl->H);
		if (hscale < 1.0 || vscale < 1.0) {
			error(domain, "mixed up/down resize is not on the device path");
			return -1;
		}
		const double rw = (hscale > 1.0 ? hscale : 1.0) * pl->W, rh = (vscale > 1.0 ? vscale : 1.0) * pl->H;
		pl->OW = (int) (rw > 0 ? rw + 0.5 : rw - 0.5);
		pl->OH = (int) (rh > 0 ? rh + 0.5 : rh - 0.5);
		pl->premul = pl->has_alpha && pl->hshrink != 1.0 && pl->vshrink != 1.0;
		pl->fused = false;
		return 0;
	}
	double hscale = std::max(1.0 / pl->hshrink, 1.0 / pl->W);
	double vscale = std::max(1.0 / pl->vshrink, 1.0 / pl->H);
	const double vs = vscale < 1.0 ? 1.0 / vscale : 1.0;
	const double hs = hscale < 1.0 ? 1.0 / hscale : 1.0;
	pl->gv = ReduceGeom{pl->H, pl->H, 1, pl->H, 0, 1.0, 0.0};
	pl->gh = ReduceGeom{pl->W, pl->W, 1, pl->W, 0, 1.0, 0.0};
	if (vs > 1.0 && reduce_geometry(domain, pl->H, vs, VB200_KERNEL_LANCZOS3, 2.0, &pl->gv))
		return -1;
	if (hs > 1.0 && reduce_geometry(domain, pl->W, hs, VB200_KERNEL_LANCZOS3, 2.0, &pl->gh))
		return -1;
	pl->OW = pl->gh.out_size;
	pl->OH = pl->gv.out_size;
	pl->premul = pl->has_alpha && pl->hshrink != 1.0 && pl->vshrink != 1.0;

	pl->fused = false;
	if (pl->linear) {
		AxisTable tv, th;
		if (pl->gv.n_point > 0 && pl->gh.n_point > 0) {
			plan_axis_tables(pl, tv, th);
			if (linear_thumb_new(domain, pl->W, pl->H, pl->bands, pl->premul, pl->gv, pl->gh, tv, th, &pl->lin) < 0)
				return -1;
		}
		pl->fused = pl->lin != nullptr;
		return 0;
	}
	pl->rgb_expand = pl->bands == 3 && ((size_t) pl->W * pl->H) % 4 == 0 && getenv("VB200_NO_RGB_EXPAND") == nullptr;
	if ((pl->bands == 4 || pl->rgb_expand) && pl->gv.n_point > 0 && pl->gh.n_point > 0) {
		int r = plan_build_fused(domain, pl);
		if (r < 0)
			return -1;
		pl->fused = r == 0;
	}
	if (!pl->fused)
		pl->rgb_expand = false;
	return 0;
}

static int thumbnail_plan_run_thumbnail(const char *domain, ThumbnailPlanImpl *pl, const void *in, size_t in_stride, void *out,
	size_t out_stride, int n, cudaStream_t s);
static int thumbnail_plan_run_fused(const char *domain, ThumbnailPlanImpl *pl, const void *in, size_t in_stride, void *out,
	size_t out_stride, int n, cudaStream_t s);
static int thumbnail_plan_run_linear_icc(const char *domain, ThumbnailPlanImpl *pl, const void *in, size_t in_stride, void *out,
	size_t out_stride, int n, cudaStream_t s, const void *const *embedded, const size_t *embedded_lens, int frame0);

double
thumbnail_common_shrink(int w, int h, int tw, int th, int size)
{
	double hs, vs;
	thumbnail_shrink(w, h, tw, th, size, &hs, &vs);
	return std::min(hs, vs);
}

int
thumbnail_plan_run_device(const char *domain, ThumbnailPlanImpl *pl, const void *in, size_t in_stride, void *out,
	size_t out_stride, int n, cudaStream_t s, const void *const *embedded = nullptr, const size_t *embedded_lens = nullptr,
	int frame0 = 0)
{
	if (n <= 0)
		return 0;
	if (pl->licc)
		return thumbnail_plan_run_linear_icc(domain, pl, in, in_stride, out, out_stride, n, s, embedded, embedded_lens, frame0);
	if (!pl->sharpen && !pl->icc)
		return thumbnail_plan_run_thumbnail(domain, pl, in, in_stride, out, out_stride, n, s);
	const size_t frame = (size_t) pl->OW * pl->OH * pl->bands;
	const int sb = pl->out_bands();
	const size_t sframe = (size_t) pl->OW * pl->OH * sb;
	void *mid = nullptr, *mid2 = nullptr;
	if (dev_alloc(domain, &mid, frame * n, s))
		return -1;
	if (pl->icc && pl->sharpen && dev_alloc(domain, &mid2, sframe * n, s)) {
		dev_free(mid, s);
		return -1;
	}
	int rc = thumbnail_plan_run_thumbnail(domain, pl, in, in_stride, mid, frame, n, s);
	const void *sin = mid;
	if (!rc && pl->icc) {
		rc = icc_stage_run(domain, pl->icc, mid, frame, pl->sharpen ? mid2 : out, pl->sharpen ? sframe : out_stride, n,
			(size_t) pl->OW * pl->OH, embedded, embedded_lens, s, frame0);
		sin = mid2;
	}
	if (!rc && pl->sharpen) {
		if (sb != 3 && sb != 4) {
			error(domain, "the sharpen stage needs 3- or 4-band frames, the output profile gives %d bands", sb);
			rc = -1;
		}
		else
			rc = dev_sharpen_fused(domain, sin, (size_t) pl->OW * sb, sframe, out, (size_t) pl->OW * sb, out_stride, n, pl->OW, pl->OH, sb,
				pl->sh_sigma, pl->sh_x1, pl->sh_y2, pl->sh_y3, pl->sh_m1, pl->sh_m2, s);
		if (rc == 1) {
			error(domain, "sharpen parameters are not on the fused path (mask too wide)");
			rc = -1;
		}
	}
	dev_free(mid, s);
	if (mid2)
		dev_free(mid2, s);
	return rc;
}

static int
thumbnail_linear_chain(const char *domain, ThumbnailPlanImpl *pl, const void *in, void *out, cudaStream_t s)
{
	DevImage din, lin, pre, res, unpre, fin;
	din.w = pl->W;
	din.h = pl->H;
	din.bands = pl->bands;
	din.fmt = VB200_FORMAT_UCHAR;
	din.type = VB200_INTERPRETATION_sRGB;
	din.bpl = (size_t) pl->W * pl->bands;
	din.data = const_cast<void *>(in);
	int rc = dev_colourspace(domain, din, &lin, VB200_INTERPRETATION_scRGB, VB200_INTERPRETATION_sRGB, s);
	const DevImage *cur = &lin;
	if (!rc && pl->premul) {
		rc = dev_premultiply(domain, lin, &pre, 0.0, 0, s);
		cur = &pre;
	}
	if (!rc)
		rc = dev_resize(domain, *cur, &res, 1.0 / pl->hshrink, 1.0 / pl->vshrink, VB200_KERNEL_LANCZOS3, 2.0, s);
	cur = &res;
	if (!rc && pl->premul) {
		rc = dev_unpremultiply(domain, res, &unpre, 0.0, 0, s);
		cur = &unpre;
	}
	if (!rc)
		rc = dev_colourspace(domain, *cur, &fin, VB200_INTERPRETATION_sRGB, VB200_INTERPRETATION_scRGB, s);
	if (!rc) {
		const size_t line = (size_t) fin.w * fin.bands;
		if (cudaMemcpy2DAsync(out, line, fin.data, fin.bpl, line, fin.h, cudaMemcpyDeviceToDevice, s) != cudaSuccess)
			rc = cuda_fail(domain, cudaGetLastError(), "linear thumbnail copy");
	}
	dev_image_release(&lin, s);
	dev_image_release(&pre, s);
	dev_image_release(&res, s);
	dev_image_release(&unpre, s);
	dev_image_release(&fin, s);
	return rc;
}

static int
thumbnail_linear_icc_chain(const char *domain, ThumbnailPlanImpl *pl, const LinIccFrame &fr, const IccJob *jobs, const void *in,
	void *out, cudaStream_t s)
{
	DevImage din, lin, pre, res, unpre, xyz, fin;
	din.w = pl->W;
	din.h = pl->H;
	din.bands = pl->bands;
	din.fmt = VB200_FORMAT_UCHAR;
	din.type = VB200_INTERPRETATION_sRGB;
	din.bpl = (size_t) pl->W * pl->bands;
	din.data = const_cast<void *>(in);
	const bool imp = fr.kind == LIN_IMPORT;
	const double max_alpha = imp ? 255.0 : 1.0;
	int rc = imp ? icc_job_apply(domain, jobs, fr.imp, din, &lin, s)
				 : dev_colourspace(domain, din, &lin, VB200_INTERPRETATION_scRGB, VB200_INTERPRETATION_sRGB, s);
	const DevImage *cur = &lin;
	if (!rc && pl->premul) {
		rc = dev_premultiply(domain, lin, &pre, max_alpha, 0, s);
		cur = &pre;
	}
	if (!rc)
		rc = dev_resize(domain, *cur, &res, 1.0 / pl->hshrink, 1.0 / pl->vshrink, VB200_KERNEL_LANCZOS3, 2.0, s);
	cur = &res;
	if (!rc && pl->premul) {
		rc = dev_unpremultiply(domain, res, &unpre, max_alpha, 0, s);
		cur = &unpre;
	}
	if (!rc && !imp) {
		rc = dev_colourspace(domain, *cur, &xyz, VB200_INTERPRETATION_XYZ, VB200_INTERPRETATION_scRGB, s);
		cur = &xyz;
	}
	if (!rc)
		rc = icc_job_apply(domain, jobs, fr.exp, *cur, &fin, s);
	if (!rc) {
		const size_t line = (size_t) fin.w * fin.bands;
		if (cudaMemcpy2DAsync(out, line, fin.data, fin.bpl, line, fin.h, cudaMemcpyDeviceToDevice, s) != cudaSuccess)
			rc = cuda_fail(domain, cudaGetLastError(), "linear ICC thumbnail copy");
	}
	for (DevImage *d : {&lin, &pre, &res, &unpre, &xyz, &fin})
		dev_image_release(d, s);
	return rc;
}

static int
thumbnail_plan_run_linear_icc(const char *domain, ThumbnailPlanImpl *pl, const void *in, size_t in_stride, void *out,
	size_t out_stride, int n, cudaStream_t s, const void *const *embedded, const size_t *embedded_lens, int frame0)
{
	const int ob = pl->licc_bands;
	const size_t sframe = (size_t) pl->OW * pl->OH * ob;
	if (pl->sharpen && ob != 3 && ob != 4) {
		error(domain, "the sharpen stage needs 3- or 4-band frames, the output profile gives %d bands", ob);
		return -1;
	}
	void *mid = nullptr;
	if (pl->sharpen && dev_alloc(domain, &mid, sframe * n, s))
		return -1;
	void *dst = pl->sharpen ? mid : out;
	const size_t dst_stride = pl->sharpen ? sframe : out_stride;
	int rc = icc_stage_run_linear(domain, pl->licc, n, embedded, embedded_lens, s, frame0, [&](const LinIccBatch &b) {
		int r = pl->lin ? linear_thumb_run(domain, pl->lin, in, in_stride, dst, dst_stride, n, s, &b, ob) : 1;
		for (int i = 0; r == 1 && i < n; i++) {
			const void *fin = (const char *) in + (size_t) i * in_stride;
			void *fout = (char *) dst + (size_t) i * dst_stride;
			if (b.h_frames[i].kind == LIN_PLAIN ? thumbnail_linear_chain(domain, pl, fin, fout, s)
												: thumbnail_linear_icc_chain(domain, pl, b.h_frames[i], b.h_jobs, fin, fout, s))
				return -1;
		}
		return r == 1 ? 0 : r;
	});
	if (!rc && pl->sharpen) {
		rc = dev_sharpen_fused(domain, mid, (size_t) pl->OW * ob, sframe, out, (size_t) pl->OW * ob, out_stride, n, pl->OW, pl->OH, ob,
			pl->sh_sigma, pl->sh_x1, pl->sh_y2, pl->sh_y3, pl->sh_m1, pl->sh_m2, s);
		if (rc == 1) {
			error(domain, "sharpen parameters are not on the fused path (mask too wide)");
			rc = -1;
		}
	}
	if (mid)
		dev_free(mid, s);
	return rc;
}

static int
thumbnail_plan_run_thumbnail(const char *domain, ThumbnailPlanImpl *pl, const void *in, size_t in_stride, void *out,
	size_t out_stride, int n, cudaStream_t s)
{
	if (n <= 0)
		return 0;
	if (pl->linear) {
		if (pl->lin)
			return linear_thumb_run(domain, pl->lin, in, in_stride, out, out_stride, n, s);
		for (int i = 0; i < n; i++)
			if (thumbnail_linear_chain(domain, pl, (const char *) in + (size_t) i * in_stride, (char *) out + (size_t) i * out_stride, s))
				return -1;
		return 0;
	}
	if (pl->fused && pl->rgb_expand && pl->bands == 3) {
		if ((((uintptr_t) in) | in_stride) & 3) {
			error(domain, "RGB frames must be 4-byte aligned for the fused path");
			return -1;
		}
		const size_t px_in = (size_t) pl->W * pl->H, px_out = (size_t) pl->OW * pl->OH;
		const int sub = (int) std::max<size_t>(1,
			std::min<size_t>(std::min<size_t>((size_t) n, kMaxBatchFrames), ((size_t) 1 << 30) / (px_in * 4)));
		void *xin = nullptr, *xout = nullptr;
		if (dev_alloc(domain, &xin, px_in * 4 * sub, s) || dev_alloc(domain, &xout, px_out * 4 * sub, s)) {
			dev_free(xin, s);
			return -1;
		}
		int rc = 0;
		for (int f0 = 0; f0 < n && !rc; f0 += sub) {
			const int nf = std::min(sub, n - f0);
			rgb_expand_kernel<<<dim3((unsigned) ((px_in / 4 + 255) / 256), nf), 256, 0, s>>>(
				(const uint8_t *) in + (size_t) f0 * in_stride, in_stride, (uint8_t *) xin, px_in * 4, px_in / 4);
			cudaError_t e = cudaGetLastError();
			if (e != cudaSuccess) {
				rc = cuda_fail(domain, e, "rgb_expand_kernel");
				break;
			}
			count_launch();
			rc = thumbnail_plan_run_fused(domain, pl, xin, px_in * 4, xout, px_out * 4, nf, s);
			if (!rc) {
				rgbx_compact_kernel<<<dim3((unsigned) ((px_out + 255) / 256), nf), 256, 0, s>>>((const uint8_t *) xout, px_out * 4,
					(uint8_t *) out + (size_t) f0 * out_stride, out_stride, px_out);
				e = cudaGetLastError();
				if (e != cudaSuccess)
					rc = cuda_fail(domain, e, "rgbx_compact_kernel");
				else
					count_launch();
			}
		}
		dev_free(xin, s);
		dev_free(xout, s);
		return rc;
	}
	if (pl->fused)
		return thumbnail_plan_run_fused(domain, pl, in, in_stride, out, out_stride, n, s);

	for (int i = 0; i < n; i++) {
		DevImage d, pre, res, fin;
		d.w = pl->W;
		d.h = pl->H;
		d.bands = pl->bands;
		d.fmt = pl->fmt;
		d.type = pl->bands < 3 ? VB200_INTERPRETATION_B_W : VB200_INTERPRETATION_sRGB;
		d.bpl = (size_t) pl->W * pl->bands;
		d.data = (char *) in + (size_t) i * in_stride;
		const DevImage *src = &d;
		if (pl->premul) {
			if (dev_premultiply(domain, d, &pre, 255.0, 1, s))
				return -1;
			src = &pre;
		}
		if (dev_resize(domain, *src, &res, 1.0 / pl->hshrink, 1.0 / pl->vshrink, VB200_KERNEL_LANCZOS3, 2.0, s))
			return -1;
		const DevImage *last = &res;
		if (pl->premul) {
			if (dev_unpremultiply(domain, res, &fin, 255.0, 1, s))
				return -1;
			last = &fin;
		}
		const size_t line = (size_t) last->w * last->bands;
		VB200_CUDA(domain, cudaMemcpy2DAsync((char *) out + (size_t) i * out_stride, line, last->data, last->bpl, line,
							   last->h, cudaMemcpyDeviceToDevice, s));
		if (pl->premul) {
			dev_image_release(&pre, s);
			dev_image_release(&fin, s);
		}
		dev_image_release(&res, s);
	}
	return 0;
}

static int
thumbnail_plan_run_fused(const char *domain, ThumbnailPlanImpl *pl, const void *in, size_t in_stride, void *out,
	size_t out_stride, int n, cudaStream_t s)
{
	const bool aligned = (((uintptr_t) in) & 15) == 0 && (n == 1 || (in_stride & 15) == 0);
	const FusedKernel kernel = aligned ? pl->kernel : FusedKernel::Ldg;
	for (int f0 = 0; f0 < n; f0 += kMaxBatchFrames) {
		const int nf = std::min(kMaxBatchFrames, n - f0);
		int rc = 0;
		switch (kernel) {
		case FusedKernel::Ldg: rc = launch_ldg(domain, pl, in, in_stride, out, out_stride, n, f0, nf, s); break;
		case FusedKernel::Tma: rc = launch_tma(domain, pl, in, in_stride, out, out_stride, n, f0, nf, s); break;
		case FusedKernel::Mma: rc = launch_mma(domain, pl, in, in_stride, out, out_stride, n, f0, nf, s); break;
		}
		if (rc)
			return rc;
	}
	return 0;
}

static const char *
plan_kernel_name(const ThumbnailPlanImpl &pl, char *buf, size_t cap)
{
	if (!pl.fused)
		return "leaf kernels";
	if (pl.linear)
		return "linear_v_kernel + linear_h_kernel";
	const FusedParams &fp = pl.fp;
	const char *alpha = pl.premul ? "premul" : "plain";
	switch (pl.kernel) {
	case FusedKernel::Mma:
		snprintf(buf, cap, "thumbnail_fused_mma_kernel<VS=%d,NP=%d,%s,HS=%d,cols=%d,cpt=%d>", fp.VS, v4_np(fp.VS, fp.NPh, fp.HS), alpha,
			fp.HS, kV4Cols, kV4Cpt);
		break;
	case FusedKernel::Tma: snprintf(buf, cap, "thumbnail_fused_tma_kernel<VS=%d,%s>", fp.VS, alpha); break;
	case FusedKernel::Ldg: snprintf(buf, cap, "thumbnail_fused_kernel<VS=%d,%s>", fp.VS, alpha); break;
	}
	return buf;
}

void
thumbnail_plan_destroy(ThumbnailPlanImpl *pl)
{
	if (pl->tables)
		cudaFree(pl->tables);
	if (pl->tables_mma)
		cudaFree(pl->tables_mma);
	if (pl->lin)
		linear_thumb_free(pl->lin);
	pl->lin = nullptr;
	icc_stage_free(pl->icc);
	pl->icc = nullptr;
	icc_stage_free(pl->licc);
	pl->licc = nullptr;
	for (int i = 0; i < ThumbnailPlanImpl::kHintSlots; i++)
		if (pl->hint_done[i]) {
			cudaEventSynchronize(pl->hint_done[i]);
			cudaEventDestroy(pl->hint_done[i]);
		}
	if (pl->hint_counts)
		cudaFreeHost(pl->hint_counts);
	for (int i = 0; i < ThumbnailPlanImpl::kStreams; i++) {
		if (pl->stage_in[i])
			cudaFree(pl->stage_in[i]);
		if (pl->stage_out[i])
			cudaFree(pl->stage_out[i]);
		if (pl->drained[i])
			cudaEventDestroy(pl->drained[i]);
		if (pl->streams[i])
			cudaStreamDestroy(pl->streams[i]);
	}
}

}


using namespace vb200;

struct VB200ThumbnailPlan {
	ThumbnailPlanImpl impl;
};

extern "C" VB200ThumbnailPlan *
vb200_thumbnail_plan_new(int width, int height, int bands, int band_format, int has_alpha, int target_width,
	int target_height, int size, int linear)
{
	const char *domain = "thumbnail_plan";
	if (ensure_init(domain))
		return nullptr;
	if (width <= 0 || height <= 0 || bands <= 0 || target_width <= 0) {
		error(domain, "bad frame geometry");
		return nullptr;
	}
	auto *plan = new VB200ThumbnailPlan();
	ThumbnailPlanImpl &pl = plan->impl;
	pl.W = width;
	pl.H = height;
	pl.bands = bands;
	pl.fmt = band_format;
	pl.has_alpha = has_alpha;
	pl.target_w = target_width;
	pl.target_h = target_height > 0 ? target_height : target_width;
	pl.size = size;
	pl.linear = linear;
	if (thumbnail_plan_init(domain, &pl)) {
		thumbnail_plan_destroy(&pl);
		delete plan;
		return nullptr;
	}
	return plan;
}

extern "C" void
vb200_thumbnail_plan_free(VB200ThumbnailPlan *plan)
{
	if (!plan)
		return;
	thumbnail_plan_destroy(&plan->impl);
	delete plan;
}

extern "C" int
vb200_thumbnail_plan_output(const VB200ThumbnailPlan *plan, int *out_width, int *out_height)
{
	if (!plan)
		return -1;
	if (out_width)
		*out_width = plan->impl.OW;
	if (out_height)
		*out_height = plan->impl.OH;
	return 0;
}

extern "C" size_t
vb200_thumbnail_plan_bytes_per_frame(const VB200ThumbnailPlan *plan)
{
	const ThumbnailPlanImpl &pl = plan->impl;
	return (size_t) pl.W * pl.H * pl.bands + (size_t) pl.OW * pl.OH * pl.bands;
}

extern "C" int
vb200_thumbnail_plan_set_sharpen(VB200ThumbnailPlan *plan, double sigma, double x1, double y2, double y3, double m1, double m2)
{
	const char *domain = "thumbnail_plan_set_sharpen";
	if (!plan) {
		error(domain, "null plan");
		return -1;
	}
	ThumbnailPlanImpl &pl = plan->impl;
	if (sigma <= 0) {
		pl.sharpen = false;
		return 0;
	}
	if ((pl.bands != 3 && pl.bands != 4) || pl.fmt != VB200_FORMAT_UCHAR) {
		error(domain, "the sharpen stage needs 3- or 4-band 8-bit frames");
		return -1;
	}
	if (sigma < 0.000001 || sigma > 10.0) {
		error(domain, "parameter sigma out of range [0.000001, 10]");
		return -1;
	}
	pl.sh_sigma = sigma;
	pl.sh_x1 = x1;
	pl.sh_y2 = y2;
	pl.sh_y3 = y3;
	pl.sh_m1 = m1;
	pl.sh_m2 = m2;
	pl.sharpen = true;
	return 0;
}

extern "C" int
vb200_thumbnail_plan_is_fused(const VB200ThumbnailPlan *plan)
{
	return plan && plan->impl.fused;
}

extern "C" const char *
vb200_thumbnail_plan_kernel(const VB200ThumbnailPlan *plan)
{
	static thread_local char name[160];
	if (!plan)
		return "leaf kernels";
	return plan_kernel_name(plan->impl, name, sizeof(name));
}

extern "C" int
vb200_thumbnail_batch_device(VB200ThumbnailPlan *plan, const void *in, size_t in_frame_stride, void *out,
	size_t out_frame_stride, int n_frames)
{
	return vb200_thumbnail_batch_device_icc(plan, in, in_frame_stride, out, out_frame_stride, n_frames, nullptr, nullptr);
}

extern "C" int
vb200_thumbnail_batch_device_icc(VB200ThumbnailPlan *plan, const void *in, size_t in_frame_stride, void *out,
	size_t out_frame_stride, int n_frames, const void *const *embedded, const size_t *embedded_lens)
{
	const char *domain = "thumbnail_batch_device";
	if (!plan || !in || !out) {
		error(domain, "null argument");
		return -1;
	}
	if (ensure_init(domain))
		return -1;
	return thumbnail_plan_run_device(domain, &plan->impl, in, in_frame_stride, out, out_frame_stride, n_frames,
		current_stream(), embedded, embedded_lens);
}

extern "C" int
vb200_thumbnail_plan_set_icc(VB200ThumbnailPlan *plan, const VB200ThumbnailIcc *icc)
{
	const char *domain = "thumbnail_plan_set_icc";
	if (!plan) {
		error(domain, "null plan");
		return -1;
	}
	ThumbnailPlanImpl &pl = plan->impl;
	if (!icc || !icc->output_profile) {
		icc_stage_free(pl.icc);
		pl.icc = nullptr;
		return 0;
	}
	if (pl.linear) {
		error(domain, "linear thumbnails with an output profile are not supported on the device path");
		return -1;
	}
	if (pl.fmt != VB200_FORMAT_UCHAR) {
		error(domain, "colour-managed thumbnails need 8-bit frames");
		return -1;
	}
	IccStage *st = icc_stage_new();
	int ob = 0;
	if (icc_stage_set(domain, st, icc, pl.bands, &ob)) {
		icc_stage_free(st);
		return -1;
	}
	icc_stage_free(pl.icc);
	pl.icc = st;
	pl.icc_bands = ob;
	return 0;
}

extern "C" int
vb200_thumbnail_plan_set_linear_icc(VB200ThumbnailPlan *plan, const VB200ThumbnailIcc *icc)
{
	const char *domain = "thumbnail_plan_set_linear_icc";
	if (!plan) {
		error(domain, "null plan");
		return -1;
	}
	ThumbnailPlanImpl &pl = plan->impl;
	if (!pl.linear) {
		error(domain, "the plan is not linear: use vb200_thumbnail_plan_set_icc");
		return -1;
	}
	if (!icc) {
		icc_stage_free(pl.licc);
		pl.licc = nullptr;
		return 0;
	}
	IccStage *st = icc_stage_new();
	int ob = 0;
	if (icc_stage_set_linear(domain, st, icc, pl.bands, &ob)) {
		icc_stage_free(st);
		return -1;
	}
	icc_stage_free(pl.licc);
	pl.licc = st;
	pl.licc_bands = ob;
	return 0;
}

extern "C" int
vb200_thumbnail_plan_output_bands(const VB200ThumbnailPlan *plan)
{
	return plan ? plan->impl.out_bands() : -1;
}

extern "C" int
vb200_thumbnail_buffer(const void *buf, size_t len, VB200Image *out, int width, int height, int size)
{
	return vb200_thumbnail_buffer_icc(buf, len, out, width, height, size, nullptr);
}

static int
thumbnail_buffer_run(const void *buf, size_t len, VB200Image *out, int width, int height, int size, const VB200ThumbnailIcc *icc,
	bool linear)
{
	const char *domain = "thumbnail_buffer";
	if (!buf || !out) {
		error(domain, "null argument");
		return -1;
	}
	if (ensure_init(domain))
		return -1;
	std::vector<unsigned char> embedded;
	if (icc && (icc->output_profile || linear) && jpeg_icc_profile(domain, (const unsigned char *) buf, len, &embedded))
		return -1;
	cudaStream_t s = current_stream();
	int w0, h0, b0;
	if (dev_jpeg_decode_batch(domain, &buf, &len, 1, 1, nullptr, 0, 0, &w0, &h0, &b0, s))
		return -1;
	const int shrink = linear ? 1 : vb200_thumbnail_jpegshrink(w0, h0, width, height, size);
	int w, h, b;
	if (dev_jpeg_decode_batch(domain, &buf, &len, 1, shrink, nullptr, 0, 0, &w, &h, &b, s))
		return -1;
	DevImage dec;
	if (dev_image_new(domain, &dec, w, h, b, VB200_FORMAT_UCHAR, b == 1 ? VB200_INTERPRETATION_B_W : VB200_INTERPRETATION_sRGB, s))
		return -1;
	int rc = dev_jpeg_decode_batch(domain, &buf, &len, 1, shrink, dec.data, dec.bpl, dec.bpl * h, nullptr, nullptr, nullptr, s);
	if (!rc) {
		VB200Image din;
		memset(&din, 0, sizeof(din));
		din.Xsize = w;
		din.Ysize = h;
		din.Bands = b;
		din.BandFmt = VB200_FORMAT_UCHAR;
		din.Type = dec.type;
		din.where = VB200_DEVICE;
		din.data = dec.data;
		din.bpl = dec.bpl;
		const int where = out->where;
		VB200Image tmp;
		memset(&tmp, 0, sizeof(tmp));
		tmp.where = VB200_DEVICE;
		rc = linear ? vb200_thumbnail_image_linear_icc(&din, &tmp, width, height, size, icc, embedded.data(), embedded.size())
					: vb200_thumbnail_image_icc(&din, &tmp, width, height, size, icc, embedded.data(), embedded.size());
		if (!rc) {
			DevImage dt;
			dt.w = tmp.Xsize;
			dt.h = tmp.Ysize;
			dt.bands = tmp.Bands;
			dt.fmt = tmp.BandFmt;
			dt.type = tmp.Type;
			dt.data = tmp.data;
			dt.bpl = tmp.bpl;
			dt.owned = true;
			VB200Image like = *out;
			like.where = where;
			rc = deliver(domain, &dt, &like, out, s);
		}
	}
	dev_image_release(&dec, s);
	return rc;
}

extern "C" int
vb200_thumbnail_buffer_icc(const void *buf, size_t len, VB200Image *out, int width, int height, int size, const VB200ThumbnailIcc *icc)
{
	return thumbnail_buffer_run(buf, len, out, width, height, size, icc, false);
}

extern "C" int
vb200_thumbnail_buffer_linear_icc(const void *buf, size_t len, VB200Image *out, int width, int height, int size,
	const VB200ThumbnailIcc *icc)
{
	return thumbnail_buffer_run(buf, len, out, width, height, size, icc, true);
}

extern "C" int
vb200_thumbnail_plan_run_jpeg(VB200ThumbnailPlan *plan, const void *const *bufs, const size_t *lens, int n, int shrink, void *out,
	int out_location, size_t out_frame_stride)
{
	const char *domain = "thumbnail_plan_run_jpeg";
	if (!plan || !bufs || !lens || !out || n < 1) {
		error(domain, "null argument");
		return -1;
	}
	if (ensure_init(domain))
		return -1;
	ThumbnailPlanImpl &pl = plan->impl;
	cudaStream_t s = current_stream();
	const size_t in_frame = (size_t) pl.W * pl.H * pl.bands, out_frame = (size_t) pl.OW * pl.OH * pl.out_bands();
	if (out_frame_stride == 0)
		out_frame_stride = out_frame;
	std::vector<std::vector<unsigned char>> profiles(pl.icc || pl.licc ? n : 0);
	std::vector<const void *> emb(profiles.size());
	std::vector<size_t> emb_len(profiles.size());
	for (size_t i = 0; i < profiles.size(); i++) {
		if (jpeg_icc_profile(domain, (const unsigned char *) bufs[i], lens[i], &profiles[i])) {
			error(domain, "stream %d", (int) i);
			return -1;
		}
		emb[i] = profiles[i].empty() ? nullptr : profiles[i].data();
		emb_len[i] = profiles[i].size();
	}
	const void *const *embedded = pl.icc || pl.licc ? emb.data() : nullptr;
	const size_t *embedded_lens = pl.icc || pl.licc ? emb_len.data() : nullptr;
	void *dec = nullptr, *res = nullptr;
	if (dev_alloc(domain, &dec, in_frame * n, s))
		return -1;
	int rc = -1;
	do {
		int w, h, b;
		if (dev_jpeg_decode_batch(domain, bufs, lens, n, shrink, dec, (size_t) pl.W * pl.bands, in_frame, &w, &h, &b, s))
			break;
		if (w != pl.W || h != pl.H || b != pl.bands) {
			error(domain, "the plan is for %d x %d x %d frames, the streams decode to %d x %d x %d", pl.W, pl.H, pl.bands, w, h, b);
			break;
		}
		if (out_location == VB200_DEVICE) {
			rc = thumbnail_plan_run_device(domain, &pl, dec, in_frame, out, out_frame_stride, n, s, embedded, embedded_lens);
			break;
		}
		if (dev_alloc(domain, &res, out_frame * n, s))
			break;
		if (thumbnail_plan_run_device(domain, &pl, dec, in_frame, res, out_frame, n, s, embedded, embedded_lens))
			break;
		if (cudaMemcpy2DAsync(out, out_frame_stride, res, out_frame, out_frame, n, cudaMemcpyDeviceToHost, s) != cudaSuccess ||
			cudaStreamSynchronize(s) != cudaSuccess) {
			cuda_fail(domain, cudaGetLastError(), "copy to host");
			break;
		}
		rc = 0;
	} while (0);
	dev_free(dec, s);
	if (res)
		dev_free(res, s);
	return rc;
}

extern "C" int
vb200_thumbnail_batch_host(VB200ThumbnailPlan *plan, const void *in, size_t in_frame_stride, void *out,
	size_t out_frame_stride, int n_frames)
{
	return vb200_thumbnail_batch_host_icc(plan, in, in_frame_stride, out, out_frame_stride, n_frames, nullptr, nullptr);
}

extern "C" int
vb200_thumbnail_batch_host_icc(VB200ThumbnailPlan *plan, const void *in, size_t in_frame_stride, void *out,
	size_t out_frame_stride, int n_frames, const void *const *embedded, const size_t *embedded_lens)
{
	const char *domain = "thumbnail_batch_host";
	if (!plan || !in || !out) {
		error(domain, "null argument");
		return -1;
	}
	if (ensure_init(domain))
		return -1;
	ThumbnailPlanImpl &pl = plan->impl;
	std::lock_guard<std::mutex> lock(pl.pump_lock);
	const size_t in_frame = (size_t) pl.W * pl.H * pl.bands;
	const size_t out_frame = (size_t) pl.OW * pl.OH * pl.out_bands();
	const int per_slice = (int) std::max<size_t>(1, std::min<size_t>(n_frames, (64u << 20) / in_frame));
	if (pl.stage_frames < per_slice || pl.stage_out_frame != out_frame) {
		for (int i = 0; i < ThumbnailPlanImpl::kStreams; i++) {
			if (pl.streams[i])
				cudaStreamSynchronize(pl.streams[i]);
			if (pl.stage_in[i])
				cudaFree(pl.stage_in[i]);
			if (pl.stage_out[i])
				cudaFree(pl.stage_out[i]);
			pl.stage_in[i] = pl.stage_out[i] = nullptr;
			VB200_CUDA(domain, cudaMalloc(&pl.stage_in[i], in_frame * std::max(per_slice, pl.stage_frames)));
			VB200_CUDA(domain, cudaMalloc(&pl.stage_out[i], out_frame * std::max(per_slice, pl.stage_frames)));
			if (!pl.streams[i])
				VB200_CUDA(domain, cudaStreamCreateWithFlags(&pl.streams[i], cudaStreamNonBlocking));
			if (!pl.drained[i])
				VB200_CUDA(domain, cudaEventCreateWithFlags(&pl.drained[i], cudaEventDisableTiming | cudaEventBlockingSync));
		}
		pl.stage_frames = std::max(per_slice, pl.stage_frames);
		pl.stage_out_frame = out_frame;
	}

	bool used[ThumbnailPlanImpl::kStreams] = {false, false, false};
	int slot = 0;
	for (int f = 0; f < n_frames; f += per_slice, slot = (slot + 1) % ThumbnailPlanImpl::kStreams) {
		const int n = std::min(per_slice, n_frames - f);
		cudaStream_t s = pl.streams[slot];
		if (used[slot])
			VB200_CUDA(domain, cudaEventSynchronize(pl.drained[slot]));
		VB200_CUDA(domain, cudaMemcpy2DAsync(pl.stage_in[slot], in_frame, (const char *) in + (size_t) f * in_frame_stride,
							   in_frame_stride, in_frame, n, cudaMemcpyHostToDevice, s));
		if (thumbnail_plan_run_device(domain, &pl, pl.stage_in[slot], in_frame, pl.stage_out[slot], out_frame, n, s,
				embedded ? embedded + f : nullptr, embedded_lens ? embedded_lens + f : nullptr, f))
			return -1;
		VB200_CUDA(domain, cudaMemcpy2DAsync((char *) out + (size_t) f * out_frame_stride, out_frame_stride,
							   pl.stage_out[slot], out_frame, out_frame, n, cudaMemcpyDeviceToHost, s));
		VB200_CUDA(domain, cudaEventRecord(pl.drained[slot], s));
		used[slot] = true;
	}
	for (int i = 0; i < ThumbnailPlanImpl::kStreams; i++)
		if (used[i])
			VB200_CUDA(domain, cudaEventSynchronize(pl.drained[i]));
	return 0;
}

static int
thumbnail_image_run(const VB200Image *in, VB200Image *out, int width, int height, int size, int linear, const VB200ThumbnailIcc *icc,
	const void *embedded, size_t embedded_len, bool linear_icc = false)
{
	const char *domain = "thumbnail";
	if (!in || !out) {
		error(domain, "null argument");
		return -1;
	}
	if (linear_icc && icc && !(in->Type == VB200_INTERPRETATION_sRGB && in->Bands >= 3)) {
		error(domain, "linear colour-managed thumbnails of interpretation %d with %d bands are not supported on the device path",
			in->Type, in->Bands);
		return -1;
	}
	if (linear_icc && icc) {
		IccStage *st = icc_stage_new();
		int ob = 0;
		const int rc = icc_stage_set_linear(domain, st, icc, in->Bands, &ob);
		icc_stage_free(st);
		if (rc)
			return -1;
	}
	if (icc && icc->output_profile &&
		!((in->Type == VB200_INTERPRETATION_sRGB && in->Bands >= 3) || (in->Type == VB200_INTERPRETATION_B_W && in->Bands < 3))) {
		error(domain, "colour-managed thumbnails of interpretation %d with %d bands are not supported on the device path", in->Type,
			in->Bands);
		return -1;
	}
	if (ensure_init(domain))
		return -1;
	if (linear && (in->BandFmt != VB200_FORMAT_UCHAR || in->Bands < 3)) {
		error(domain, "linear thumbnails on the device path need an 8-bit image with 3+ bands");
		return -1;
	}
	const int has_alpha = image_hasalpha(in->Type, in->Bands);
	VB200ThumbnailPlan *plan = vb200_thumbnail_plan_new(in->Xsize, in->Ysize, in->Bands, in->BandFmt, has_alpha, width,
		height, size, linear);
	if (!plan)
		return -1;
	if (icc && (linear_icc ? vb200_thumbnail_plan_set_linear_icc(plan, icc) : vb200_thumbnail_plan_set_icc(plan, icc))) {
		vb200_thumbnail_plan_free(plan);
		return -1;
	}
	const int ob = plan->impl.out_bands();
	const int colour = ob - (in->Bands - (in->Bands < 3 ? 1 : 3));
	const int otype = !plan->impl.icc && !plan->impl.licc ? in->Type
		: colour == 1				  ? VB200_INTERPRETATION_B_W
		: colour == 3				  ? VB200_INTERPRETATION_sRGB
									  : VB200_INTERPRETATION_CMYK;
	cudaStream_t s = current_stream();
	DevImage din, dout;
	int rc = to_device(domain, in, &din, s);
	if (!rc && din.bpl != (size_t) din.w * din.bands) {
		error(domain, "device frames must be packed");
		rc = -1;
	}
	if (!rc)
		rc = dev_image_new(domain, &dout, plan->impl.OW, plan->impl.OH, ob, in->BandFmt, otype, s);
	if (!rc) {
		const void *emb[1] = {embedded};
		const size_t emb_len[1] = {embedded ? embedded_len : 0};
		rc = thumbnail_plan_run_device(domain, &plan->impl, din.data, 0, dout.data, 0, 1, s, emb, emb_len);
	}
	if (!rc)
		rc = deliver(domain, &dout, in, out, s);
	if (!rc && in->where == VB200_DEVICE)
		cudaStreamSynchronize(s);
	dev_image_release(&din, s);
	vb200_thumbnail_plan_free(plan);
	return rc;
}

extern "C" int
vb200_thumbnail_image(const VB200Image *in, VB200Image *out, int width, int height, int size, int linear)
{
	return thumbnail_image_run(in, out, width, height, size, linear, nullptr, nullptr, 0);
}

extern "C" int
vb200_thumbnail_image_icc(const VB200Image *in, VB200Image *out, int width, int height, int size, const VB200ThumbnailIcc *icc,
	const void *embedded, size_t embedded_len)
{
	return thumbnail_image_run(in, out, width, height, size, 0, icc, embedded, embedded_len);
}

extern "C" int
vb200_thumbnail_image_linear_icc(const VB200Image *in, VB200Image *out, int width, int height, int size, const VB200ThumbnailIcc *icc,
	const void *embedded, size_t embedded_len)
{
	return thumbnail_image_run(in, out, width, height, size, 1, icc, embedded, embedded_len, true);
}

extern "C" int
vb200_debug_thumbnail_bands(int width, int height, int target_width, int *out_width, int *n_bands, int *xa, int *xb,
	int *c_lo, int *c_hi, int *seam, int cap, int *box_width, int *n_box)
{
	if (width <= 0 || height <= 0 || target_width <= 0 || cap <= 0)
		return -1;
	ThumbnailPlanImpl pl;
	pl.W = width;
	pl.H = height;
	pl.bands = 4;
	pl.fmt = VB200_FORMAT_UCHAR;
	pl.has_alpha = 1;
	pl.target_w = pl.target_h = target_width;
	pl.size = VB200_SIZE_BOTH;
	pl.geometry_only = true;
	if (thumbnail_plan_init("debug_thumbnail_bands", &pl))
		return -1;
	if (!pl.fused || pl.kernel != FusedKernel::Mma)
		return 1;
	const int nb = (int) pl.mma_bands.size();
	if (nb > cap)
		return -1;
	*out_width = pl.OW;
	*n_bands = nb;
	for (int b = 0; b < nb; b++) {
		const MmaBand &m = pl.mma_bands[b];
		xa[b] = m.xa;
		xb[b] = m.xb;
		c_lo[b] = m.c_lo;
		c_hi[b] = m.c_hi;
		seam[b] = b + 1 < nb ? std::max(0, m.c_hi - pl.mma_bands[b + 1].c_lo) : 0;
	}
	*n_box = v4_nbox(pl.fp.HS);
	*box_width = v4_boxw(pl.fp.HS);
	return 0;
}

extern "C" int
vb200_debug_thumbnail_kernel(int width, int height, int bands, int has_alpha, int target_width, int target_height, int size,
	char *name, int cap)
{
	if (width <= 0 || height <= 0 || bands <= 0 || target_width <= 0 || !name || cap <= 0)
		return -1;
	ThumbnailPlanImpl pl;
	pl.W = width;
	pl.H = height;
	pl.bands = bands;
	pl.fmt = VB200_FORMAT_UCHAR;
	pl.has_alpha = has_alpha;
	pl.target_w = target_width;
	pl.target_h = target_height > 0 ? target_height : target_width;
	pl.size = size;
	pl.geometry_only = true;
	if (thumbnail_plan_init("debug_thumbnail_kernel", &pl))
		return -1;
	char buf[160];
	const char *k = plan_kernel_name(pl, buf, sizeof(buf));
	if ((int) strlen(k) >= cap)
		return -1;
	strcpy(name, k);
	return 0;
}
```

libvips_b200/csrc/thumbnail_fused_mma.cuh:

```cuda

constexpr int kV4Rows = 8;
constexpr int kV4Quads = 8;
constexpr int kV4Cols = 768;
constexpr int kV4Cpt = 2;

#ifndef VB200_V4_STAGES
#define VB200_V4_STAGES 4
#endif
#ifndef VB200_V4_NH768
#define VB200_V4_NH768 3
#endif
#ifndef VB200_V4_MMA_UNROLL
#define VB200_V4_MMA_UNROLL 2
#endif

constexpr int kV4OpaqueSkip = 7;

constexpr int kV4HWarps = VB200_V4_NH768;

#ifndef VB200_V4_BOXPAD
#define VB200_V4_BOXPAD 64
#endif
#ifndef VB200_V4_CLO_ALIGN
#define VB200_V4_CLO_ALIGN 32
#endif
constexpr bool
v4_lines(int hs)
{
	return hs > 2;
}
constexpr int
v4_clo_align(int hs)
{
	return v4_lines(hs) ? VB200_V4_CLO_ALIGN : 4;
}
constexpr int
v4_nbox(int hs)
{
	return kV4Cols + (v4_lines(hs) ? VB200_V4_BOXPAD : 8) > 512 ? 2 : 1;
}
constexpr int
v4_boxw(int hs)
{
	return (kV4Cols + (v4_lines(hs) ? VB200_V4_BOXPAD : 8)) / v4_nbox(hs);
}

template <int VS>
struct V4Stages {
	static constexpr int value = VS <= 2 ? 2 * VB200_V4_STAGES
		: (VS >= 7 ? VB200_V4_STAGES / 2 : (VS >= 5 ? (3 * VB200_V4_STAGES) / 4 : VB200_V4_STAGES));
};

template <int HSQ>
struct V4Group {
	static constexpr bool pow2 = (HSQ & (HSQ - 1)) == 0;
	static constexpr int value = pow2 ? 32 : (32 / HSQ) * HSQ;
};

__device__ __forceinline__ void
mma_u8s8(int (&d)[4], const unsigned (&a)[4], unsigned b0, unsigned b1)
{
	asm volatile("mma.sync.aligned.m16n8k32.row.col.s32.u8.s8.s32 {%0,%1,%2,%3}, {%4,%5,%6,%7}, {%8,%9}, {%0,%1,%2,%3};"
				 : "+r"(d[0]), "+r"(d[1]), "+r"(d[2]), "+r"(d[3])
				 : "r"(a[0]), "r"(a[1]), "r"(a[2]), "r"(a[3]), "r"(b0), "r"(b1));
}

__device__ __forceinline__ void
mma_u8u8(int (&d)[4], const unsigned (&a)[4], unsigned b0, unsigned b1)
{
	asm volatile("mma.sync.aligned.m16n8k32.row.col.s32.u8.u8.s32 {%0,%1,%2,%3}, {%4,%5,%6,%7}, {%8,%9}, {%0,%1,%2,%3};"
				 : "+r"(d[0]), "+r"(d[1]), "+r"(d[2]), "+r"(d[3])
				 : "r"(a[0]), "r"(a[1]), "r"(a[2]), "r"(a[3]), "r"(b0), "r"(b1));
}

__device__ __forceinline__ int
v4_finish(int hi, int lo, int k20)
{
	const int v = __mulhi(hi * 256 + lo, k20);
	return max(0, min(v, 255));
}

template <int VS, int NP, bool PREMUL, int HSQ, bool OPQ = false>
__global__ void __launch_bounds__(kV4Cols / kV4Cpt + 32 * kV4HWarps + 32, 1)
thumbnail_fused_mma_kernel(const __grid_constant__ FusedParams P, const __grid_constant__ CUtensorMap tmap, int use_tmap,
	const uint8_t *__restrict__ in, size_t in_frame_stride, uint8_t *__restrict__ out, size_t out_frame_stride, int frame0)
{
	extern __shared__ __align__(128) unsigned char smem_raw[];

	constexpr int KM = kV4Rows;
	const int K = P.mma_rows;
	constexpr int S = V4Stages<VS>::value;
	constexpr int NH = kV4HWarps;
	constexpr int CPT = kV4Cpt;
	constexpr int kMmaUnroll = VB200_V4_MMA_UNROLL;
	constexpr int NBOX = v4_nbox(HSQ);
	constexpr int BOXW = v4_boxw(HSQ);
	static_assert(BOXW % 4 == 0 && BOXW <= 512, "a box row is whole 16-byte units, at most 256 u64 elements");
	constexpr int PITCH = BOXW * 4;
	constexpr int NPR = NP > 0 ? NP : 1;
	constexpr int HSHIFT = HSQ == 2 ? 1 : HSQ == 4 ? 2 : 3;
	constexpr bool VPOW2 = (VS & (VS - 1)) == 0;
	constexpr bool HPOW2 = V4Group<HSQ>::pow2;
	constexpr int G = V4Group<HSQ>::value;
	constexpr int rows_per_stage = 2 * VS;
	constexpr unsigned box_bytes = ((unsigned) rows_per_stage * PITCH + 127u) & ~127u;
	constexpr unsigned stage_bytes = NBOX * box_bytes;

	const int NT = P.NT;
	const int NC = NT * CPT;
	const int t = threadIdx.x;
	const int NPh = NP > 0 ? NP : P.NPh;
	const int LC = HPOW2 ? NC : (NT / 32) * 2 * G;
	const int shs = (LC / HSQ + 1) / 2;
	const unsigned QS = (unsigned) NC * 16u + 16u;

	unsigned char *stages = smem_raw;
	uint64_t *bars = (uint64_t *) (smem_raw + S * stage_bytes);
	unsigned char *quadbuf = (unsigned char *) (bars + 2 * S + 4);
	uint2 *sh = (uint2 *) (quadbuf + (size_t) kV4Quads * QS);
	int *hcoef = (int *) (sh + (size_t) 2 * KM * shs);
	int *uscale = hcoef + P.nhsets * P.NPh;

	const unsigned stages_s = smem_addr(stages);
	const unsigned full_s = smem_addr(bars);
	const unsigned empty_s = full_s + 8u * S;
	const unsigned shfull_s = empty_s + 8u * S;
	const unsigned shempty_s = shfull_s + 16u;

	for (int i = t; i < P.nhsets * P.NPh; i += blockDim.x)
		hcoef[i] = P.hcoef[i];
	if (PREMUL)
		for (int i = t; i < 256; i += blockDim.x)
			uscale[i] = i == 0 ? 0 : (int) __ddiv_rn(__dmul_rn(256.0, 255.0), (double) i);

	const int xa = blockIdx.x * P.TW;
	const int xb = min(xa + P.TW, P.OW);
	const int y_begin = blockIdx.y * P.RPC;
	const int y_end = min(y_begin + P.RPC, P.OH);
	const int frame = frame0 + blockIdx.z;
	const uint8_t *fin = in + (size_t) frame * in_frame_stride;
	uint8_t *fout = out + (size_t) frame * out_frame_stride;

	const int pair_h0 = __ldg(&P.hcol[xa]).x;
	const int E0 = 2 * pair_h0 + P.hgrid;
	const int NE = 2 * (__ldg(&P.hcol[xb - 1]).x + P.NPh - pair_h0);

	auto column_of = [&](int tt) {
		const int e = E0 + tt / HSQ;
		const int k = tt - (tt / HSQ) * HSQ;
		const int sc = max(0, min(e - P.hembed, P.Ws - 1));
		return min(sc * HSQ + k, P.W - 1);
	};
	const int c_lo = column_of(0) & ~(v4_clo_align(HSQ) - 1);
	const int c_hi = min(P.W, (column_of(NE * HSQ - 1) + 4) & ~3);
	const unsigned row_bytes = (unsigned) (c_hi - c_lo) * 4u;
	const int chunk0 = y_begin / K;
	const int q_first = __ldg(&P.vchunk[chunk0]).x;
	const int NTa = HPOW2 ? min(NT, ((NE * HSQ + 32 * CPT - 1) / (32 * CPT)) * 32) : min(NT, ((NE * HSQ + 2 * G - 1) / (2 * G)) * 32);

	if (t == 0) {
		for (int i = 0; i < S; i++) {
			mbar_init(full_s + 8u * i, 1);
			mbar_init(empty_s + 8u * i, NTa / 32);
		}
		for (int i = 0; i < 2; i++) {
			mbar_init(shfull_s + 8u * i, NTa / 32);
			mbar_init(shempty_s + 8u * i, NH);
		}
		asm volatile("fence.mbarrier_init.release.cluster;" ::: "memory");
	}
	__syncthreads();

	if (t >= NT + 32 * NH) {
		const int lane = t - NT - 32 * NH;
		const uint8_t *src0 = fin + (size_t) c_lo * 4;
		const int j = lane / VS, k = lane - j * VS;
		const bool copier = lane < rows_per_stage;
		int s = 0;
		unsigned phase = 0;
		int pdone = 2 * q_first;
		for (int ya = y_begin, cc = chunk0; ya < y_end; ya += K, cc++) {
			const int P1 = 2 * __ldg(&P.vchunk[cc]).y + 1;
			for (int p = pdone; p <= P1; p++) {
				do
					mbar_wait(empty_s + 8u * s, phase ^ 1u);
				while (0);
				const int sr0 = 2 * p - P.vembed;
				const bool interior = use_tmap && sr0 >= 0 && sr0 + 1 <= P.Hs - 1 && (sr0 + 2) * VS <= P.H;
				if (interior) {
					if (lane == 0) {
						mbar_expect_tx(full_s + 8u * s, (unsigned) NBOX * rows_per_stage * PITCH);
#pragma unroll
						for (int h = 0; h < NBOX; h++)
							asm volatile("cp.async.bulk.tensor.3d.shared::cluster.global.tile.mbarrier::complete_tx::bytes [%0], [%1, {%2, %3, %4}], [%5];" ::"r"(
											 stages_s + (unsigned) s * stage_bytes + (unsigned) h * box_bytes),
										 "l"(&tmap), "r"((c_lo + h * BOXW) >> 1), "r"(sr0 * VS), "r"(frame), "r"(full_s + 8u * s)
										 : "memory");
					}
				}
				else {
					if (lane == 0)
						mbar_expect_tx(full_s + 8u * s, (unsigned) rows_per_stage * row_bytes);
					__syncwarp();
					if (copier) {
						const int sr = max(0, min(2 * p + j - P.vembed, P.Hs - 1));
						const int row = min(sr * VS + k, P.H - 1);
#pragma unroll
						for (int h = 0; h < NBOX; h++) {
							const int nb = min((int) row_bytes - h * PITCH, PITCH);
							if (nb > 0)
								bulk_copy_g2s(stages_s + (unsigned) s * stage_bytes + (unsigned) h * box_bytes + (unsigned) lane * PITCH,
									src0 + (size_t) row * P.in_bpl + (size_t) h * PITCH, (unsigned) nb, full_s + 8u * s);
						}
					}
				}
				if (++s == S) {
					s = 0;
					phase ^= 1u;
				}
			}
			pdone = max(pdone, P1 + 1);
		}
		return;
	}

	if (t >= NT) {
		const int ht = t - NT;
		const int lane = ht & 31;
		const int bw = xb - xa;
		int chunk = 0;
		for (int ya = y_begin; ya < y_end; ya += K, chunk++) {
			const int yb = min(ya + K, y_end);
			const int rows = yb - ya;
			const int buf = chunk & 1;
			const uint2 *shb = sh + (size_t) buf * KM * shs;
			mbar_wait(shfull_s + 8u * buf, (unsigned) (chunk >> 1) & 1u);
			for (int idx = ht; idx < rows * bw; idx += 32 * NH) {
				const int k = fast_div(idx, bw);
				const int x = xa + (idx - k * bw);
				const int2 hc = __ldg(&P.hcol[x]);
				const uint2 *win = shb + k * shs + (hc.x - pair_h0);
				const int *cfp = hcoef + hc.y * NPh;
				int r = VB200_INTERPOLATE_SCALE >> 1, g = r, b = r, a = r;
				if (NP > 0) {
#pragma unroll
					for (int kk = 0; kk < NPR; kk++) {
						const uint2 w = win[kk];
						const unsigned c = (unsigned) cfp[kk];
						r = dp2a_lo(c, w.x, r);
						b = dp2a_hi(c, w.x, b);
						g = dp2a_lo(c, w.y, g);
						a = dp2a_hi(c, w.y, a);
					}
				}
				else
					for (int kk = 0; kk < NPh; kk++) {
						const uint2 w = win[kk];
						const unsigned c = (unsigned) cfp[kk];
						r = dp2a_lo(c, w.x, r);
						b = dp2a_hi(c, w.x, b);
						g = dp2a_lo(c, w.y, g);
						a = dp2a_hi(c, w.y, a);
					}
				r = max(0, min(r >> VB200_INTERPOLATE_SHIFT, 255));
				g = max(0, min(g >> VB200_INTERPOLATE_SHIFT, 255));
				b = max(0, min(b >> VB200_INTERPOLATE_SHIFT, 255));
				a = max(0, min(a >> VB200_INTERPOLATE_SHIFT, 255));
				if (PREMUL) {
					const int sc = uscale[a];
					r = ((r * sc + 128) >> 8) & 0xff;
					g = ((g * sc + 128) >> 8) & 0xff;
					b = ((b * sc + 128) >> 8) & 0xff;
				}
				*(unsigned *) (fout + (size_t) (ya + k) * P.out_bpl + (size_t) x * 4) =
					(unsigned) r | ((unsigned) g << 8) | ((unsigned) b << 16) | ((unsigned) a << 24);
			}
			__syncwarp();
			if (lane == 0)
				mbar_arrive(shempty_s + 8u * buf);
		}
		return;
	}

	if (t >= NTa)
		return;
	const int lane_ = t & 31;
	const int tt0 = HPOW2 ? t * CPT
						  : (t >> 5) * 2 * G + (lane_ >> 4) * G + min((lane_ & 15) * 2, G - 2);
	const int my_c = column_of(min(tt0, NE * HSQ - CPT)) - c_lo;
	const unsigned char *my_cols = stages + (size_t) (my_c / BOXW) * box_bytes + (size_t) (my_c % BOXW) * 4u;
	constexpr bool PAIR64 = HPOW2;
	const int my_c1 = column_of(min(tt0 + 1, NE * HSQ - 1)) - c_lo;
	const unsigned char *my_cols1 = stages + (size_t) (my_c1 / BOXW) * box_bytes + (size_t) (my_c1 % BOXW) * 4u;
	const unsigned accm = P.accmul;
	unsigned k16;
	asm volatile("mov.u32 %0, 0x10000;" : "=r"(k16));
	int k20;
	asm volatile("mov.u32 %0, 0x100000;" : "=r"(k20));
	const unsigned amend2 = (unsigned) (VS / 2) * 0x00010001u;
	const unsigned vmul8 = P.vmul8, hmul8 = P.hmul8;
	const int lane = t & 31;
	const bool lane0 = lane == 0;
	const int tig = lane & 3, g = lane >> 2, ch = g & 3, jj = g >> 2;
	const int warp_col0 = (t & ~31) * CPT;
	const unsigned char *a_base = quadbuf + (size_t) tig * QS + (size_t) (warp_col0 + (HPOW2 ? 4 : 32) * jj) * 16u + (unsigned) ch * 4u;
	unsigned char *q_store = quadbuf + (size_t) (t * CPT) * 16u;
	const int ch_off = ch == 0 ? 0 : ch == 1 ? 4 : ch == 2 ? 2 : 6;
	const int warp_sx0 = HPOW2 ? warp_col0 / HSQ : (t >> 5) * (2 * G / HSQ) + jj * (G / HSQ);

	int s = 0;
	unsigned phase = 0;
	int qdone = q_first;
	int chunk = 0;
	const bool opq_on = OPQ && PREMUL && P.opaque_hint != nullptr && __ldg(P.opaque_hint + blockIdx.z) != 0;
	int opq_skip = 0;

	for (int ya = y_begin; ya < y_end; ya += K, chunk++) {
		const int q1 = __ldg(&P.vchunk[chunk0 + chunk]).y;

		for (int q = qdone; q <= q1; q++) {
			unsigned rb[4][CPT], ga[4][CPT];
#pragma unroll
			for (int r = 0; r < 4; r++)
#pragma unroll
				for (int i = 0; i < CPT; i++)
					rb[r][i] = ga[r][i] = amend2;
#pragma unroll
			for (int half = 0; half < 2; half++) {
				const unsigned soff = (unsigned) s * stage_bytes;
				mbar_wait(full_s + 8u * s, phase);
				uint2 pa[VS], pb[VS];
#pragma unroll
				for (int k = 0; k < VS; k++) {
					if (PAIR64) {
						pa[k] = *(const uint2 *) (my_cols + soff + k * PITCH);
						pb[k] = *(const uint2 *) (my_cols + soff + (VS + k) * PITCH);
					}
					else {
						pa[k].x = *(const unsigned *) (my_cols + soff + k * PITCH);
						pa[k].y = *(const unsigned *) (my_cols1 + soff + k * PITCH);
						pb[k].x = *(const unsigned *) (my_cols + soff + (VS + k) * PITCH);
						pb[k].y = *(const unsigned *) (my_cols1 + soff + (VS + k) * PITCH);
					}
				}
				__syncwarp();
				if (lane0)
					mbar_arrive(empty_s + 8u * s);
				bool opaque = false;
				if (OPQ && PREMUL && opq_on) {
					if (opq_skip == 0) {
						unsigned m = 0xffffffffu;
#pragma unroll
						for (int k = 0; k < VS; k++)
							m &= pa[k].x & pa[k].y & pb[k].x & pb[k].y;
						opaque = __all_sync(0xffffffffu, m >= 0xff000000u);
						if (!opaque)
							opq_skip = kV4OpaqueSkip;
					}
					else
						opq_skip--;
				}
				if (opaque) {
#pragma unroll
					for (int k = 0; k < VS; k++) {
						accumulate_pixel_h<false>(pa[k].x, k16, rb[2 * half][0], ga[2 * half][0]);
						accumulate_pixel_h<false>(pa[k].y, k16, rb[2 * half][CPT - 1], ga[2 * half][CPT - 1]);
						accumulate_pixel_h<false>(pb[k].x, k16, rb[2 * half + 1][0], ga[2 * half + 1][0]);
						accumulate_pixel_h<false>(pb[k].y, k16, rb[2 * half + 1][CPT - 1], ga[2 * half + 1][CPT - 1]);
					}
				}
				else {
#pragma unroll
					for (int k = 0; k < VS; k++) {
						accumulate_pixel_h<PREMUL>(pa[k].x, k16, rb[2 * half][0], ga[2 * half][0]);
						accumulate_pixel_h<PREMUL>(pa[k].y, k16, rb[2 * half][CPT - 1], ga[2 * half][CPT - 1]);
						accumulate_pixel_h<PREMUL>(pb[k].x, k16, rb[2 * half + 1][0], ga[2 * half + 1][0]);
						accumulate_pixel_h<PREMUL>(pb[k].y, k16, rb[2 * half + 1][CPT - 1], ga[2 * half + 1][CPT - 1]);
					}
				}
				if (++s == S) {
					s = 0;
					phase ^= 1u;
				}
			}
#pragma unroll
			for (int i = 0; i < CPT; i++) {
				if (!VPOW2) {
					unsigned av[4][4];
#pragma unroll
					for (int r = 0; r < 4; r++) {
						av[r][0] = __umulhi(rb[r][i] & 0xffffu, vmul8);
						av[r][1] = __umulhi(rb[r][i] >> 16, vmul8);
						av[r][2] = __umulhi(ga[r][i] & 0xffffu, vmul8);
						av[r][3] = __umulhi(ga[r][i] >> 16, vmul8);
					}
					uint4 w;
					w.x = __byte_perm(__byte_perm(av[0][0], av[1][0], 0x0040), __byte_perm(av[2][0], av[3][0], 0x0040), 0x5410);
					w.y = __byte_perm(__byte_perm(av[0][2], av[1][2], 0x0040), __byte_perm(av[2][2], av[3][2], 0x0040), 0x5410);
					w.z = __byte_perm(__byte_perm(av[0][1], av[1][1], 0x0040), __byte_perm(av[2][1], av[3][1], 0x0040), 0x5410);
					w.w = __byte_perm(__byte_perm(av[0][3], av[1][3], 0x0040), __byte_perm(av[2][3], av[3][3], 0x0040), 0x5410);
					*(uint4 *) (q_store + (size_t) (q & (kV4Quads - 1)) * QS + i * 16) = w;
				}
				else {
#pragma unroll
					for (int r = 0; r < 4; r++) {
						rb[r][i] *= accm;
						ga[r][i] *= accm;
					}
					const unsigned rb01 = __byte_perm(rb[0][i], rb[1][i], 0x7351);
					const unsigned rb23 = __byte_perm(rb[2][i], rb[3][i], 0x7351);
					const unsigned ga01 = __byte_perm(ga[0][i], ga[1][i], 0x7351);
					const unsigned ga23 = __byte_perm(ga[2][i], ga[3][i], 0x7351);
					uint4 w;
					w.x = __byte_perm(rb01, rb23, 0x5410);
					w.y = __byte_perm(ga01, ga23, 0x5410);
					w.z = __byte_perm(rb01, rb23, 0x7632);
					w.w = __byte_perm(ga01, ga23, 0x7632);
					*(uint4 *) (q_store + (size_t) (q & (kV4Quads - 1)) * QS + i * 16) = w;
				}
			}
		}
		qdone = max(qdone, q1 + 1);
		__syncwarp();

		const int buf = chunk & 1;
		const uint4 bf = __ldg(&P.vbfrag[(size_t) (chunk0 + chunk) * 32 + lane]);
		mbar_wait(shempty_s + 8u * buf, ((unsigned) (chunk >> 1) & 1u) ^ 1u);
		unsigned char *shb = (unsigned char *) (sh + (size_t) buf * KM * shs) + (size_t) (2 * tig) * shs * 8 + ch_off;
		int bsum[2] = {0, 0};
		int bcnt = 0, bidx = 0;
#pragma unroll kMmaUnroll
		for (int tp = 0; tp < 4 * CPT; tp++) {
			unsigned a[2][4];
			int dh[2][4], dl[2][4];
#pragma unroll
			for (int T = 0; T < 2; T++) {
				const unsigned char *ap = a_base + tp * (HPOW2 ? 128 : 64) + T * 32;
				a[T][0] = *(const unsigned *) (ap);
				a[T][1] = *(const unsigned *) (ap + 16);
				a[T][2] = *(const unsigned *) (ap + 4 * (size_t) QS);
				a[T][3] = *(const unsigned *) (ap + 4 * (size_t) QS + 16);
			}
#pragma unroll
			for (int T = 0; T < 2; T++) {
#pragma unroll
				for (int i = 0; i < 4; i++) {
					dh[T][i] = 0;
					dl[T][i] = VB200_INTERPOLATE_SCALE >> 1;
				}
				mma_u8s8(dh[T], a[T], bf.x, bf.y);
				mma_u8u8(dl[T], a[T], bf.z, bf.w);
			}
#pragma unroll
			for (int r = 0; r < 2; r++) {
				const int v00 = v4_finish(dh[0][r], dl[0][r], k20);
				const int v01 = v4_finish(dh[0][2 + r], dl[0][2 + r], k20);
				const int v10 = v4_finish(dh[1][r], dl[1][r], k20);
				const int v11 = v4_finish(dh[1][2 + r], dl[1][2 + r], k20);
				if (!HPOW2)
					continue;
				if (HSQ == 2) {
					const int sx = warp_sx0 + tp * 4 + 2 * jj;
					unsigned char *d = shb + (size_t) r * shs * 8 + (sx >> 1) * 8;
					d[0] = (unsigned char) ((v00 + v01 + 1) >> 1);
					d[1] = (unsigned char) ((v10 + v11 + 1) >> 1);
				}
				else if (HSQ == 4) {
					const int sx = warp_sx0 + tp * 2 + jj;
					shb[(size_t) r * shs * 8 + (sx >> 1) * 8 + (sx & 1)] = (unsigned char) ((v00 + v01 + v10 + v11 + 2) >> 2);
				}
				else {
					int sum = v00 + v01 + v10 + v11;
					sum += __shfl_xor_sync(0xffffffffu, sum, 16);
					const int sx = warp_sx0 + tp;
					if (jj == 0)
						shb[(size_t) r * shs * 8 + (sx >> 1) * 8 + (sx & 1)] = (unsigned char) ((sum + 4) >> HSHIFT);
				}
			}
			if (!HPOW2) {
#pragma unroll
				for (int sl = 0; sl < 4; sl++) {
					const int T = sl >> 1, h = sl & 1;
					if (4 * tp + sl < G) {
						bsum[0] += v4_finish(dh[T][2 * h], dl[T][2 * h], k20);
						bsum[1] += v4_finish(dh[T][2 * h + 1], dl[T][2 * h + 1], k20);
						if (++bcnt == HSQ) {
							const int sx = warp_sx0 + bidx;
							unsigned char *d = shb + (sx >> 1) * 8 + (sx & 1);
							d[0] = (unsigned char) __umulhi((unsigned) (bsum[0] + HSQ / 2), hmul8);
							d[(size_t) shs * 8] = (unsigned char) __umulhi((unsigned) (bsum[1] + HSQ / 2), hmul8);
							bsum[0] = bsum[1] = 0;
							bcnt = 0;
							bidx++;
						}
					}
				}
			}
		}
		__syncwarp();
		if (lane0)
			mbar_arrive(shfull_s + 8u * buf);
	}
}
```

Before: 704,500.

## Make the tensor-pipe thumbnail kernel persistent with atomic ticket work-stealing

Replaces the static 3D grid (band x row-block x frame) with a persistent grid of one CTA per SM that pulls work items from a global atomic ticket counter. The producer warp fetches tickets and passes them to the consumer warps through an mbarrier-protected ring in shared memory. Whole frames are processed as full-height column bands, and the tail frames are split into row-chunk pieces to balance the last wave. This targets tail imbalance and per-CTA setup cost. It adds a per-launch device allocation and memset, more shared memory, and extra synchronisation per item.

Measured after the change: 714,600 (median of 6 runs). 1.4% higher.

```diff
diff --git a/include/vb200.h b/include/vb200.h
--- a/include/vb200.h
+++ b/include/vb200.h
@@ -256,6 +256,8 @@
 
 int vb200_debug_thumbnail_bands(int width, int height, int target_width, int *out_width, int *n_bands, int *xa, int *xb,
 	int *c_lo, int *c_hi, int *seam, int cap, int *box_width, int *n_box);
+int vb200_debug_thumbnail_items(int width, int height, int has_alpha, int target_width, int target_height, int size, int frames,
+	int sms, int *items, int cap, int *n_items, int *ctas, int *chunk_rows);
 int vb200_debug_thumbnail_kernel(int width, int height, int bands, int has_alpha, int target_width, int target_height, int size,
 	char *name, int cap);
 
diff --git a/libvips_b200/csrc/thumbnail_fused.cu b/libvips_b200/csrc/thumbnail_fused.cu
--- a/libvips_b200/csrc/thumbnail_fused.cu
+++ b/libvips_b200/csrc/thumbnail_fused.cu
@@ -48,6 +48,8 @@
 	const int2 *vchunk;
 	const uint4 *vbfrag;
 	int mma_rows;
+	int v4_whole_frames, v4_pieces, v4_piece_chunks, v4_items;
+	int *v4_ticket;
 	int premul;
 	const unsigned char *opaque_hint;
 	double max_alpha;
@@ -963,6 +965,25 @@
 	return rpc;
 }
 
+struct MmaSplit {
+	int whole_frames, pieces, piece_chunks, items;
+};
+
+MmaSplit
+mma_split(int frames, int bands, int chunks, int sms)
+{
+	MmaSplit sp;
+	const long long whole = (long long) frames * bands;
+	const long long tail = std::min(whole, whole % sms + sms);
+	const int tail_frames = (int) ((tail + bands - 1) / bands);
+	const long long tail_chunks = (long long) tail_frames * bands * chunks;
+	sp.whole_frames = frames - tail_frames;
+	sp.piece_chunks = (int) std::min<long long>(chunks, std::max<long long>(4, (tail_chunks + 8LL * sms - 1) / (8LL * sms)));
+	sp.pieces = (chunks + sp.piece_chunks - 1) / sp.piece_chunks;
+	sp.items = sp.whole_frames * bands + tail_frames * bands * sp.pieces;
+	return sp;
+}
+
 template <int VS, bool PREMUL>
 int
 launch_ldg_t(const char *domain, const FusedParams &fp, size_t smem, const void *in, size_t in_stride, void *out,
@@ -1198,15 +1219,31 @@
 template <int VS, int NP, bool PREMUL, int HSQ>
 int
 launch_mma_t(const char *domain, ThumbnailPlanImpl *pl, FusedParams fp, const void *in, size_t in_stride, void *out,
-	size_t out_stride, int n, int f0, dim3 grid, cudaStream_t s)
+	size_t out_stride, int n, int f0, int nf, cudaStream_t s)
 {
 	CUtensorMap tm;
 	memset(&tm, 0, sizeof(tm));
 	const int use_tmap = make_stage_tensor_map(&tm, in, fp.W, fp.H, fp.in_bpl, in_stride, n, v4_boxw(HSQ), 2 * VS) ? 1 : 0;
+	const MmaSplit sp = mma_split(nf, (fp.OW + fp.TW - 1) / fp.TW, (fp.OH + fp.mma_rows - 1) / fp.mma_rows, sm_count());
+	fp.v4_whole_frames = sp.whole_frames;
+	fp.v4_pieces = sp.pieces;
+	fp.v4_piece_chunks = sp.piece_chunks;
+	fp.v4_items = sp.items;
+	const dim3 grid(std::min(sm_count(), sp.items));
+	void *ticket = nullptr;
+	if (dev_alloc(domain, &ticket, sizeof(int), s))
+		return -1;
+	fp.v4_ticket = (int *) ticket;
+	if (cudaMemsetAsync(ticket, 0, sizeof(int), s) != cudaSuccess) {
+		dev_free(ticket, s);
+		return cuda_fail(domain, cudaGetLastError(), "ticket counter");
+	}
 	void *hint = nullptr;
 	bool use_opq = false;
-	if (PREMUL && opaque_hint_begin(domain, pl, fp, (const uint8_t *) in + (size_t) f0 * in_stride, in_stride, (int) grid.z, s, &hint, &use_opq))
-		return -1;
+	if (PREMUL && opaque_hint_begin(domain, pl, fp, (const uint8_t *) in + (size_t) f0 * in_stride, in_stride, nf, s, &hint, &use_opq)) {
+		dev_free(ticket, s);
+		return -1;
+	}
 	fp.opaque_hint = (const unsigned char *) hint;
 	int rc;
 	if constexpr (PREMUL)
@@ -1214,19 +1251,20 @@
 					 : launch_mma_k<VS, NP, PREMUL, HSQ, false>(domain, pl, fp, tm, use_tmap, in, in_stride, out, out_stride, f0, grid, s);
 	else
 		rc = launch_mma_k<VS, NP, PREMUL, HSQ, false>(domain, pl, fp, tm, use_tmap, in, in_stride, out, out_stride, f0, grid, s);
-	opaque_hint_end(pl, hint, (int) grid.z, s);
+	opaque_hint_end(pl, hint, nf, s);
+	dev_free(ticket, s);
 	return rc;
 }
 
 template <bool PREMUL>
 int
 launch_mma_list(const char *domain, ThumbnailPlanImpl *pl, const FusedParams &fp, const void *in, size_t is, void *out, size_t os,
-	int n, int f0, dim3 grid, cudaStream_t s)
+	int n, int f0, int nf, cudaStream_t s)
 {
 	const int np = v4_np(fp.VS, fp.NPh, fp.HS);
 #define X(VS_, NP_, HS_) \
 	if (fp.VS == VS_ && np == NP_ && fp.HS == HS_) \
-		return launch_mma_t<VS_, NP_, PREMUL, HS_>(domain, pl, fp, in, is, out, os, n, f0, grid, s);
+		return launch_mma_t<VS_, NP_, PREMUL, HS_>(domain, pl, fp, in, is, out, os, n, f0, nf, s);
 	VB200_V4_LIST(X)
 #undef X
 	error(domain, "the tensor-pipe kernel has no instantiation for VS %d, HS %d", fp.VS, fp.HS);
@@ -1241,11 +1279,8 @@
 	fp.TW = pl->mma_tw;
 	fp.NT = pl->mma_nt;
 	fp.NEmax = pl->mma_nemax;
-	const int bands_x = (pl->OW + fp.TW - 1) / fp.TW;
-	fp.RPC = rows_per_cta(pl->OH, fp.mma_rows, 4, bands_x, n, sm_count());
-	const dim3 grid(bands_x, (pl->OH + fp.RPC - 1) / fp.RPC, nf);
-	return pl->premul ? launch_mma_list<true>(domain, pl, fp, in, is, out, os, n, f0, grid, s)
-					  : launch_mma_list<false>(domain, pl, fp, in, is, out, os, n, f0, grid, s);
+	return pl->premul ? launch_mma_list<true>(domain, pl, fp, in, is, out, os, n, f0, nf, s)
+					  : launch_mma_list<false>(domain, pl, fp, in, is, out, os, n, f0, nf, s);
 }
 
 void
@@ -1467,10 +1502,10 @@
 			pl->mma_bands = mma_bands_of(fp, hcol, tw4, v4_clo_align(fp.HS));
 			const int nbox = v4_nbox(fp.HS);
 			const size_t box_bytes = ((size_t) 2 * fp.VS * (pitch / nbox) + 127) & ~(size_t) 127;
-			pl->smem_mma = (size_t) stages * nbox * box_bytes + (2 * stages + 4) * 8 +
+			pl->smem_mma = (size_t) stages * nbox * box_bytes + (2 * stages + 4 + 2 * kV4Items) * 8 +
 				(size_t) kV4Quads * ((size_t) pl->mma_nt * kV4Cpt * 16 + 16) +
 				(size_t) 2 * kV4Rows * ((logical_cols / fp.HS + 1) / 2) * 8 +
-				(size_t) (fp.nhsets * fp.NPh + 256) * 4;
+				(size_t) (fp.nhsets * fp.NPh + 256 + kV4Items) * 4;
 			const size_t n_ch = vchunk.size() * sizeof(int2), n_bf = bfrag.size() * sizeof(uint4);
 			if (pl->smem_mma <= 226 * 1024) {
 				if (!pl->geometry_only) {
@@ -2495,6 +2530,48 @@
 }
 
 extern "C" int
+vb200_debug_thumbnail_items(int width, int height, int has_alpha, int target_width, int target_height, int size, int frames,
+	int sms, int *items, int cap, int *n_items, int *ctas, int *chunk_rows)
+{
+	if (width <= 0 || height <= 0 || target_width <= 0 || frames <= 0 || frames > kMaxBatchFrames || sms <= 0 || cap < 0 ||
+		!n_items || !ctas || !chunk_rows)
+		return -1;
+	ThumbnailPlanImpl pl;
+	pl.W = width;
+	pl.H = height;
+	pl.bands = 4;
+	pl.fmt = VB200_FORMAT_UCHAR;
+	pl.has_alpha = has_alpha;
+	pl.target_w = target_width;
+	pl.target_h = target_height > 0 ? target_height : target_width;
+	pl.size = size;
+	pl.geometry_only = true;
+	if (thumbnail_plan_init("debug_thumbnail_items", &pl))
+		return -1;
+	if (!pl.fused || pl.kernel != FusedKernel::Mma)
+		return 1;
+	const int nbands = (int) pl.mma_bands.size();
+	const int K = pl.fp.mma_rows;
+	const int nchunks = (pl.OH + K - 1) / K;
+	const MmaSplit sp = mma_split(frames, nbands, nchunks, sms);
+	*n_items = sp.items;
+	*ctas = std::min(sms, sp.items);
+	*chunk_rows = K;
+	if (sp.items > cap)
+		return items ? -1 : 0;
+	for (int tk = 0; tk < sp.items; tk++) {
+		const V4Item it = v4_item(tk, sp.whole_frames, sp.pieces, sp.piece_chunks, nbands, nchunks);
+		int *o = items + 5 * (size_t) tk;
+		o[0] = it.f;
+		o[1] = it.band;
+		o[2] = it.c0 * K;
+		o[3] = std::min(it.c1 * K, pl.OH);
+		o[4] = pl.mma_bands[it.band].c_hi - pl.mma_bands[it.band].c_lo;
+	}
+	return 0;
+}
+
+extern "C" int
 vb200_debug_thumbnail_kernel(int width, int height, int bands, int has_alpha, int target_width, int target_height, int size,
 	char *name, int cap)
 {
diff --git a/libvips_b200/csrc/thumbnail_fused_mma.cuh b/libvips_b200/csrc/thumbnail_fused_mma.cuh
--- a/libvips_b200/csrc/thumbnail_fused_mma.cuh
+++ b/libvips_b200/csrc/thumbnail_fused_mma.cuh
@@ -3,6 +3,7 @@
 constexpr int kV4Quads = 8;
 constexpr int kV4Cols = 768;
 constexpr int kV4Cpt = 2;
+constexpr int kV4Items = 4;
 
 #ifndef VB200_V4_STAGES
 #define VB200_V4_STAGES 4
@@ -78,6 +79,35 @@
 {
 	const int v = __mulhi(hi * 256 + lo, k20);
 	return max(0, min(v, 255));
+}
+
+struct V4Item {
+	int f, band, c0, c1;
+};
+
+__host__ __device__ __forceinline__ V4Item
+v4_item(int tk, int whole_frames, int pieces, int piece_chunks, int nbands, int nchunks)
+{
+	V4Item it;
+	const int whole = whole_frames * nbands;
+	if (tk < whole) {
+		it.f = tk / nbands;
+		it.band = tk - it.f * nbands;
+		it.c0 = 0;
+		it.c1 = nchunks;
+	}
+	else {
+		const int per_frame = nbands * pieces;
+		const int i = tk - whole;
+		const int fi = i / per_frame;
+		const int r = i - fi * per_frame;
+		const int piece = r / nbands;
+		it.f = whole_frames + fi;
+		it.band = r - piece * nbands;
+		it.c0 = piece * piece_chunks;
+		it.c1 = min(nchunks, it.c0 + piece_chunks);
+	}
+	return it;
 }
 
 template <int VS, int NP, bool PREMUL, int HSQ, bool OPQ = false>
@@ -116,16 +146,19 @@
 
 	unsigned char *stages = smem_raw;
 	uint64_t *bars = (uint64_t *) (smem_raw + S * stage_bytes);
-	unsigned char *quadbuf = (unsigned char *) (bars + 2 * S + 4);
+	unsigned char *quadbuf = (unsigned char *) (bars + 2 * S + 4 + 2 * kV4Items);
 	uint2 *sh = (uint2 *) (quadbuf + (size_t) kV4Quads * QS);
 	int *hcoef = (int *) (sh + (size_t) 2 * KM * shs);
 	int *uscale = hcoef + P.nhsets * P.NPh;
+	volatile int *item_ring = uscale + 256;
 
 	const unsigned stages_s = smem_addr(stages);
 	const unsigned full_s = smem_addr(bars);
 	const unsigned empty_s = full_s + 8u * S;
 	const unsigned shfull_s = empty_s + 8u * S;
 	const unsigned shempty_s = shfull_s + 16u;
+	const unsigned ifull_s = shempty_s + 16u;
+	const unsigned iempty_s = ifull_s + 8u * kV4Items;
 
 	for (int i = t; i < P.nhsets * P.NPh; i += blockDim.x)
 		hcoef[i] = P.hcoef[i];
@@ -133,165 +166,208 @@
 		for (int i = t; i < 256; i += blockDim.x)
 			uscale[i] = i == 0 ? 0 : (int) __ddiv_rn(__dmul_rn(256.0, 255.0), (double) i);
 
-	const int xa = blockIdx.x * P.TW;
-	const int xb = min(xa + P.TW, P.OW);
-	const int y_begin = blockIdx.y * P.RPC;
-	const int y_end = min(y_begin + P.RPC, P.OH);
-	const int frame = frame0 + blockIdx.z;
-	const uint8_t *fin = in + (size_t) frame * in_frame_stride;
-	uint8_t *fout = out + (size_t) frame * out_frame_stride;
-
-	const int pair_h0 = __ldg(&P.hcol[xa]).x;
-	const int E0 = 2 * pair_h0 + P.hgrid;
-	const int NE = 2 * (__ldg(&P.hcol[xb - 1]).x + P.NPh - pair_h0);
-
-	auto column_of = [&](int tt) {
-		const int e = E0 + tt / HSQ;
-		const int k = tt - (tt / HSQ) * HSQ;
-		const int sc = max(0, min(e - P.hembed, P.Ws - 1));
-		return min(sc * HSQ + k, P.W - 1);
+	auto v_threads = [&](int NE) {
+		return HPOW2 ? min(NT, ((NE * HSQ + 32 * CPT - 1) / (32 * CPT)) * 32) : min(NT, ((NE * HSQ + 2 * G - 1) / (2 * G)) * 32);
 	};
-	const int c_lo = column_of(0) & ~(v4_clo_align(HSQ) - 1);
-	const int c_hi = min(P.W, (column_of(NE * HSQ - 1) + 4) & ~3);
-	const unsigned row_bytes = (unsigned) (c_hi - c_lo) * 4u;
-	const int chunk0 = y_begin / K;
-	const int q_first = __ldg(&P.vchunk[chunk0]).x;
-	const int NTa = HPOW2 ? min(NT, ((NE * HSQ + 32 * CPT - 1) / (32 * CPT)) * 32) : min(NT, ((NE * HSQ + 2 * G - 1) / (2 * G)) * 32);
+	const int NTv = v_threads(P.NEmax);
 
 	if (t == 0) {
 		for (int i = 0; i < S; i++) {
 			mbar_init(full_s + 8u * i, 1);
-			mbar_init(empty_s + 8u * i, NTa / 32);
+			mbar_init(empty_s + 8u * i, NTv / 32);
 		}
 		for (int i = 0; i < 2; i++) {
-			mbar_init(shfull_s + 8u * i, NTa / 32);
+			mbar_init(shfull_s + 8u * i, NTv / 32);
 			mbar_init(shempty_s + 8u * i, NH);
+		}
+		for (int i = 0; i < kV4Items; i++) {
+			mbar_init(ifull_s + 8u * i, 1);
+			mbar_init(iempty_s + 8u * i, NTv / 32 + NH);
 		}
 		asm volatile("fence.mbarrier_init.release.cluster;" ::: "memory");
 	}
 	__syncthreads();
 
+	const int nbands = (P.OW + P.TW - 1) / P.TW;
+	const int nchunks = (P.OH + K - 1) / K;
+	auto item_of = [&](int tk) { return v4_item(tk, P.v4_whole_frames, P.v4_pieces, P.v4_piece_chunks, nbands, nchunks); };
+	int ii = 0;
+	unsigned iphase = 0;
+	auto next_ticket = [&]() {
+		mbar_wait(ifull_s + 8u * ii, iphase);
+		const int tk = item_ring[ii];
+		__syncwarp();
+		if ((t & 31) == 0)
+			mbar_arrive(iempty_s + 8u * ii);
+		if (++ii == kV4Items) {
+			ii = 0;
+			iphase ^= 1u;
+		}
+		return tk;
+	};
+
 	if (t >= NT + 32 * NH) {
 		const int lane = t - NT - 32 * NH;
-		const uint8_t *src0 = fin + (size_t) c_lo * 4;
 		const int j = lane / VS, k = lane - j * VS;
 		const bool copier = lane < rows_per_stage;
 		int s = 0;
 		unsigned phase = 0;
-		int pdone = 2 * q_first;
-		for (int ya = y_begin, cc = chunk0; ya < y_end; ya += K, cc++) {
-			const int P1 = 2 * __ldg(&P.vchunk[cc]).y + 1;
-			for (int p = pdone; p <= P1; p++) {
-				do
-					mbar_wait(empty_s + 8u * s, phase ^ 1u);
-				while (0);
-				const int sr0 = 2 * p - P.vembed;
-				const bool interior = use_tmap && sr0 >= 0 && sr0 + 1 <= P.Hs - 1 && (sr0 + 2) * VS <= P.H;
-				if (interior) {
-					if (lane == 0) {
-						mbar_expect_tx(full_s + 8u * s, (unsigned) NBOX * rows_per_stage * PITCH);
-#pragma unroll
-						for (int h = 0; h < NBOX; h++)
-							asm volatile("cp.async.bulk.tensor.3d.shared::cluster.global.tile.mbarrier::complete_tx::bytes [%0], [%1, {%2, %3, %4}], [%5];" ::"r"(
-											 stages_s + (unsigned) s * stage_bytes + (unsigned) h * box_bytes),
-										 "l"(&tmap), "r"((c_lo + h * BOXW) >> 1), "r"(sr0 * VS), "r"(frame), "r"(full_s + 8u * s)
-										 : "memory");
-					}
-				}
-				else {
-					if (lane == 0)
-						mbar_expect_tx(full_s + 8u * s, (unsigned) rows_per_stage * row_bytes);
-					__syncwarp();
-					if (copier) {
-						const int sr = max(0, min(2 * p + j - P.vembed, P.Hs - 1));
-						const int row = min(sr * VS + k, P.H - 1);
-#pragma unroll
-						for (int h = 0; h < NBOX; h++) {
-							const int nb = min((int) row_bytes - h * PITCH, PITCH);
-							if (nb > 0)
-								bulk_copy_g2s(stages_s + (unsigned) s * stage_bytes + (unsigned) h * box_bytes + (unsigned) lane * PITCH,
-									src0 + (size_t) row * P.in_bpl + (size_t) h * PITCH, (unsigned) nb, full_s + 8u * s);
-						}
-					}
-				}
-				if (++s == S) {
-					s = 0;
-					phase ^= 1u;
-				}
+		for (;;) {
+			int tk = 0;
+			if (lane == 0) {
+				tk = atomicAdd(P.v4_ticket, 1);
+				mbar_wait(iempty_s + 8u * ii, iphase ^ 1u);
+				item_ring[ii] = tk;
+				mbar_arrive(ifull_s + 8u * ii);
 			}
-			pdone = max(pdone, P1 + 1);
-		}
-		return;
+			tk = __shfl_sync(0xffffffffu, tk, 0);
+			if (++ii == kV4Items) {
+				ii = 0;
+				iphase ^= 1u;
+			}
+			if (tk >= P.v4_items)
+				return;
+			const V4Item it = item_of(tk);
+			const int f = it.f, band = it.band, c0 = it.c0, c1 = it.c1;
+			const int xa = band * P.TW;
+			const int xb = min(xa + P.TW, P.OW);
+			const int pair_h0 = __ldg(&P.hcol[xa]).x;
+			const int E0 = 2 * pair_h0 + P.hgrid;
+			const int NE = 2 * (__ldg(&P.hcol[xb - 1]).x + P.NPh - pair_h0);
+			auto column_of = [&](int tt) {
+				const int e = E0 + tt / HSQ;
+				const int kk = tt - (tt / HSQ) * HSQ;
+				const int sc = max(0, min(e - P.hembed, P.Ws - 1));
+				return min(sc * HSQ + kk, P.W - 1);
+			};
+			const int c_lo = column_of(0) & ~(v4_clo_align(HSQ) - 1);
+			const int c_hi = min(P.W, (column_of(NE * HSQ - 1) + 4) & ~3);
+			const unsigned row_bytes = (unsigned) (c_hi - c_lo) * 4u;
+			const int frame = frame0 + f;
+			const uint8_t *src0 = in + (size_t) frame * in_frame_stride + (size_t) c_lo * 4;
+			const int y_begin = c0 * K, y_end = min(c1 * K, P.OH);
+			int pdone = 2 * __ldg(&P.vchunk[c0]).x;
+			for (int ya = y_begin, cc = c0; ya < y_end; ya += K, cc++) {
+				const int P1 = 2 * __ldg(&P.vchunk[cc]).y + 1;
+				for (int p = pdone; p <= P1; p++) {
+					do
+						mbar_wait(empty_s + 8u * s, phase ^ 1u);
+					while (0);
+					const int sr0 = 2 * p - P.vembed;
+					const bool interior = use_tmap && sr0 >= 0 && sr0 + 1 <= P.Hs - 1 && (sr0 + 2) * VS <= P.H;
+					if (interior) {
+						if (lane == 0) {
+							mbar_expect_tx(full_s + 8u * s, (unsigned) NBOX * rows_per_stage * PITCH);
+#pragma unroll
+							for (int h = 0; h < NBOX; h++)
+								asm volatile("cp.async.bulk.tensor.3d.shared::cluster.global.tile.mbarrier::complete_tx::bytes [%0], [%1, {%2, %3, %4}], [%5];" ::"r"(
+												 stages_s + (unsigned) s * stage_bytes + (unsigned) h * box_bytes),
+											 "l"(&tmap), "r"((c_lo + h * BOXW) >> 1), "r"(sr0 * VS), "r"(frame), "r"(full_s + 8u * s)
+											 : "memory");
+						}
+					}
+					else {
+						if (lane == 0)
+							mbar_expect_tx(full_s + 8u * s, (unsigned) rows_per_stage * row_bytes);
+						__syncwarp();
+						if (copier) {
+							const int sr = max(0, min(2 * p + j - P.vembed, P.Hs - 1));
+							const int row = min(sr * VS + k, P.H - 1);
+#pragma unroll
+							for (int h = 0; h < NBOX; h++) {
+								const int nb = min((int) row_bytes - h * PITCH, PITCH);
+								if (nb > 0)
+									bulk_copy_g2s(stages_s + (unsigned) s * stage_bytes + (unsigned) h * box_bytes + (unsigned) lane * PITCH,
+										src0 + (size_t) row * P.in_bpl + (size_t) h * PITCH, (unsigned) nb, full_s + 8u * s);
+							}
+						}
+					}
+					if (++s == S) {
+						s = 0;
+						phase ^= 1u;
+					}
+				}
+				pdone = max(pdone, P1 + 1);
+			}
+		}
 	}
+
+	int chunk = 0;
 
 	if (t >= NT) {
 		const int ht = t - NT;
 		const int lane = ht & 31;
-		const int bw = xb - xa;
-		int chunk = 0;
-		for (int ya = y_begin; ya < y_end; ya += K, chunk++) {
-			const int yb = min(ya + K, y_end);
-			const int rows = yb - ya;
-			const int buf = chunk & 1;
-			const uint2 *shb = sh + (size_t) buf * KM * shs;
-			mbar_wait(shfull_s + 8u * buf, (unsigned) (chunk >> 1) & 1u);
-			for (int idx = ht; idx < rows * bw; idx += 32 * NH) {
-				const int k = fast_div(idx, bw);
-				const int x = xa + (idx - k * bw);
-				const int2 hc = __ldg(&P.hcol[x]);
-				const uint2 *win = shb + k * shs + (hc.x - pair_h0);
-				const int *cfp = hcoef + hc.y * NPh;
-				int r = VB200_INTERPOLATE_SCALE >> 1, g = r, b = r, a = r;
-				if (NP > 0) {
-#pragma unroll
-					for (int kk = 0; kk < NPR; kk++) {
-						const uint2 w = win[kk];
-						const unsigned c = (unsigned) cfp[kk];
-						r = dp2a_lo(c, w.x, r);
-						b = dp2a_hi(c, w.x, b);
-						g = dp2a_lo(c, w.y, g);
-						a = dp2a_hi(c, w.y, a);
-					}
-				}
-				else
-					for (int kk = 0; kk < NPh; kk++) {
-						const uint2 w = win[kk];
-						const unsigned c = (unsigned) cfp[kk];
-						r = dp2a_lo(c, w.x, r);
-						b = dp2a_hi(c, w.x, b);
-						g = dp2a_lo(c, w.y, g);
-						a = dp2a_hi(c, w.y, a);
-					}
-				r = max(0, min(r >> VB200_INTERPOLATE_SHIFT, 255));
-				g = max(0, min(g >> VB200_INTERPOLATE_SHIFT, 255));
-				b = max(0, min(b >> VB200_INTERPOLATE_SHIFT, 255));
-				a = max(0, min(a >> VB200_INTERPOLATE_SHIFT, 255));
-				if (PREMUL) {
-					const int sc = uscale[a];
-					r = ((r * sc + 128) >> 8) & 0xff;
-					g = ((g * sc + 128) >> 8) & 0xff;
-					b = ((b * sc + 128) >> 8) & 0xff;
-				}
-				*(unsigned *) (fout + (size_t) (ya + k) * P.out_bpl + (size_t) x * 4) =
-					(unsigned) r | ((unsigned) g << 8) | ((unsigned) b << 16) | ((unsigned) a << 24);
+		for (;;) {
+			const int tk = next_ticket();
+			if (tk >= P.v4_items)
+				return;
+			const V4Item it = item_of(tk);
+			const int f = it.f, band = it.band, c0 = it.c0, c1 = it.c1;
+			const int xa = band * P.TW;
+			const int xb = min(xa + P.TW, P.OW);
+			const int pair_h0 = __ldg(&P.hcol[xa]).x;
+			const int bw = xb - xa;
+			const int y_begin = c0 * K, y_end = min(c1 * K, P.OH);
+			uint8_t *fout = out + (size_t) (frame0 + f) * out_frame_stride;
+			for (int ya = y_begin; ya < y_end; ya += K, chunk++) {
+				const int yb = min(ya + K, y_end);
+				const int rows = yb - ya;
+				const int buf = chunk & 1;
+				const uint2 *shb = sh + (size_t) buf * KM * shs;
+				mbar_wait(shfull_s + 8u * buf, (unsigned) (chunk >> 1) & 1u);
+				for (int idx = ht; idx < rows * bw; idx += 32 * NH) {
+					const int k = fast_div(idx, bw);
+					const int x = xa + (idx - k * bw);
+					const int2 hc = __ldg(&P.hcol[x]);
+					const uint2 *win = shb + k * shs + (hc.x - pair_h0);
+					const int *cfp = hcoef + hc.y * NPh;
+					int r = VB200_INTERPOLATE_SCALE >> 1, g = r, b = r, a = r;
+					if (NP > 0) {
+#pragma unroll
+						for (int kk = 0; kk < NPR; kk++) {
+							const uint2 w = win[kk];
+							const unsigned c = (unsigned) cfp[kk];
+							r = dp2a_lo(c, w.x, r);
+							b = dp2a_hi(c, w.x, b);
+							g = dp2a_lo(c, w.y, g);
+							a = dp2a_hi(c, w.y, a);
+						}
+					}
+					else
+						for (int kk = 0; kk < NPh; kk++) {
+							const uint2 w = win[kk];
+							const unsigned c = (unsigned) cfp[kk];
+							r = dp2a_lo(c, w.x, r);
+							b = dp2a_hi(c, w.x, b);
+							g = dp2a_lo(c, w.y, g);
+							a = dp2a_hi(c, w.y, a);
+						}
+					r = max(0, min(r >> VB200_INTERPOLATE_SHIFT, 255));
+					g = max(0, min(g >> VB200_INTERPOLATE_SHIFT, 255));
+					b = max(0, min(b >> VB200_INTERPOLATE_SHIFT, 255));
+					a = max(0, min(a >> VB200_INTERPOLATE_SHIFT, 255));
+					if (PREMUL) {
+						const int sc = uscale[a];
+						r = ((r * sc + 128) >> 8) & 0xff;
+						g = ((g * sc + 128) >> 8) & 0xff;
+						b = ((b * sc + 128) >> 8) & 0xff;
+					}
+					*(unsigned *) (fout + (size_t) (ya + k) * P.out_bpl + (size_t) x * 4) =
+						(unsigned) r | ((unsigned) g << 8) | ((unsigned) b << 16) | ((unsigned) a << 24);
+				}
+				__syncwarp();
+				if (lane == 0)
+					mbar_arrive(shempty_s + 8u * buf);
 			}
-			__syncwarp();
-			if (lane == 0)
-				mbar_arrive(shempty_s + 8u * buf);
-		}
-		return;
+		}
 	}
 
-	if (t >= NTa)
+	if (t >= NTv)
 		return;
 	const int lane_ = t & 31;
 	const int tt0 = HPOW2 ? t * CPT
 						  : (t >> 5) * 2 * G + (lane_ >> 4) * G + min((lane_ & 15) * 2, G - 2);
-	const int my_c = column_of(min(tt0, NE * HSQ - CPT)) - c_lo;
-	const unsigned char *my_cols = stages + (size_t) (my_c / BOXW) * box_bytes + (size_t) (my_c % BOXW) * 4u;
 	constexpr bool PAIR64 = HPOW2;
-	const int my_c1 = column_of(min(tt0 + 1, NE * HSQ - 1)) - c_lo;
-	const unsigned char *my_cols1 = stages + (size_t) (my_c1 / BOXW) * box_bytes + (size_t) (my_c1 % BOXW) * 4u;
 	const unsigned accm = P.accmul;
 	unsigned k16;
 	asm volatile("mov.u32 %0, 0x10000;" : "=r"(k16));
@@ -310,195 +386,242 @@
 
 	int s = 0;
 	unsigned phase = 0;
-	int qdone = q_first;
-	int chunk = 0;
-	const bool opq_on = OPQ && PREMUL && P.opaque_hint != nullptr && __ldg(P.opaque_hint + blockIdx.z) != 0;
-	int opq_skip = 0;
-
-	for (int ya = y_begin; ya < y_end; ya += K, chunk++) {
-		const int q1 = __ldg(&P.vchunk[chunk0 + chunk]).y;
-
-		for (int q = qdone; q <= q1; q++) {
-			unsigned rb[4][CPT], ga[4][CPT];
-#pragma unroll
-			for (int r = 0; r < 4; r++)
-#pragma unroll
-				for (int i = 0; i < CPT; i++)
-					rb[r][i] = ga[r][i] = amend2;
-#pragma unroll
-			for (int half = 0; half < 2; half++) {
-				const unsigned soff = (unsigned) s * stage_bytes;
-				mbar_wait(full_s + 8u * s, phase);
-				uint2 pa[VS], pb[VS];
-#pragma unroll
-				for (int k = 0; k < VS; k++) {
-					if (PAIR64) {
-						pa[k] = *(const uint2 *) (my_cols + soff + k * PITCH);
-						pb[k] = *(const uint2 *) (my_cols + soff + (VS + k) * PITCH);
-					}
-					else {
-						pa[k].x = *(const unsigned *) (my_cols + soff + k * PITCH);
-						pa[k].y = *(const unsigned *) (my_cols1 + soff + k * PITCH);
-						pb[k].x = *(const unsigned *) (my_cols + soff + (VS + k) * PITCH);
-						pb[k].y = *(const unsigned *) (my_cols1 + soff + (VS + k) * PITCH);
-					}
-				}
+	for (;;) {
+		const int tk = next_ticket();
+		if (tk >= P.v4_items)
+			return;
+		const V4Item it = item_of(tk);
+		const int f = it.f, band = it.band, c0 = it.c0, c1 = it.c1;
+		const int xa = band * P.TW;
+		const int xb = min(xa + P.TW, P.OW);
+		const int pair_h0 = __ldg(&P.hcol[xa]).x;
+		const int E0 = 2 * pair_h0 + P.hgrid;
+		const int NE = 2 * (__ldg(&P.hcol[xb - 1]).x + P.NPh - pair_h0);
+		auto column_of = [&](int tt) {
+			const int e = E0 + tt / HSQ;
+			const int k = tt - (tt / HSQ) * HSQ;
+			const int sc = max(0, min(e - P.hembed, P.Ws - 1));
+			return min(sc * HSQ + k, P.W - 1);
+		};
+		const int c_lo = column_of(0) & ~(v4_clo_align(HSQ) - 1);
+		const int my_c = column_of(min(tt0, NE * HSQ - CPT)) - c_lo;
+		const unsigned char *my_cols = stages + (size_t) (my_c / BOXW) * box_bytes + (size_t) (my_c % BOXW) * 4u;
+		const int my_c1 = column_of(min(tt0 + 1, NE * HSQ - 1)) - c_lo;
+		const unsigned char *my_cols1 = stages + (size_t) (my_c1 / BOXW) * box_bytes + (size_t) (my_c1 % BOXW) * 4u;
+		const bool idle = t >= v_threads(NE);
+		const int y_begin = c0 * K, y_end = min(c1 * K, P.OH);
+		int qdone = __ldg(&P.vchunk[c0]).x;
+		const bool opq_on = OPQ && PREMUL && P.opaque_hint != nullptr && __ldg(P.opaque_hint + f) != 0;
+		int opq_skip = 0;
+		if (idle) {
+			for (int ya = y_begin, cc = c0; ya < y_end; ya += K, cc++, chunk++) {
+				const int q1 = __ldg(&P.vchunk[cc]).y;
+				for (int q = qdone; q <= q1; q++)
+					for (int half = 0; half < 2; half++) {
+						mbar_wait(full_s + 8u * s, phase);
+						__syncwarp();
+						if (lane0)
+							mbar_arrive(empty_s + 8u * s);
+						if (++s == S) {
+							s = 0;
+							phase ^= 1u;
+						}
+					}
+				qdone = max(qdone, q1 + 1);
+				const int buf = chunk & 1;
+				mbar_wait(shempty_s + 8u * buf, ((unsigned) (chunk >> 1) & 1u) ^ 1u);
 				__syncwarp();
 				if (lane0)
-					mbar_arrive(empty_s + 8u * s);
-				bool opaque = false;
-				if (OPQ && PREMUL && opq_on) {
-					if (opq_skip == 0) {
-						unsigned m = 0xffffffffu;
-#pragma unroll
-						for (int k = 0; k < VS; k++)
-							m &= pa[k].x & pa[k].y & pb[k].x & pb[k].y;
-						opaque = __all_sync(0xffffffffu, m >= 0xff000000u);
-						if (!opaque)
-							opq_skip = kV4OpaqueSkip;
-					}
-					else
-						opq_skip--;
-				}
-				if (opaque) {
+					mbar_arrive(shfull_s + 8u * buf);
+			}
+			continue;
+		}
+
+		for (int ya = y_begin, cc = c0; ya < y_end; ya += K, cc++, chunk++) {
+			const int q1 = __ldg(&P.vchunk[cc]).y;
+
+			for (int q = qdone; q <= q1; q++) {
+				unsigned rb[4][CPT], ga[4][CPT];
+#pragma unroll
+				for (int r = 0; r < 4; r++)
+#pragma unroll
+					for (int i = 0; i < CPT; i++)
+						rb[r][i] = ga[r][i] = amend2;
+#pragma unroll
+				for (int half = 0; half < 2; half++) {
+					const unsigned soff = (unsigned) s * stage_bytes;
+					mbar_wait(full_s + 8u * s, phase);
+					uint2 pa[VS], pb[VS];
 #pragma unroll
 					for (int k = 0; k < VS; k++) {
-						accumulate_pixel_h<false>(pa[k].x, k16, rb[2 * half][0], ga[2 * half][0]);
-						accumulate_pixel_h<false>(pa[k].y, k16, rb[2 * half][CPT - 1], ga[2 * half][CPT - 1]);
-						accumulate_pixel_h<false>(pb[k].x, k16, rb[2 * half + 1][0], ga[2 * half + 1][0]);
-						accumulate_pixel_h<false>(pb[k].y, k16, rb[2 * half + 1][CPT - 1], ga[2 * half + 1][CPT - 1]);
-					}
-				}
-				else {
-#pragma unroll
-					for (int k = 0; k < VS; k++) {
-						accumulate_pixel_h<PREMUL>(pa[k].x, k16, rb[2 * half][0], ga[2 * half][0]);
-						accumulate_pixel_h<PREMUL>(pa[k].y, k16, rb[2 * half][CPT - 1], ga[2 * half][CPT - 1]);
-						accumulate_pixel_h<PREMUL>(pb[k].x, k16, rb[2 * half + 1][0], ga[2 * half + 1][0]);
-						accumulate_pixel_h<PREMUL>(pb[k].y, k16, rb[2 * half + 1][CPT - 1], ga[2 * half + 1][CPT - 1]);
-					}
-				}
-				if (++s == S) {
-					s = 0;
-					phase ^= 1u;
+						if (PAIR64) {
+							pa[k] = *(const uint2 *) (my_cols + soff + k * PITCH);
+							pb[k] = *(const uint2 *) (my_cols + soff + (VS + k) * PITCH);
+						}
+						else {
+							pa[k].x = *(const unsigned *) (my_cols + soff + k * PITCH);
+							pa[k].y = *(const unsigned *) (my_cols1 + soff + k * PITCH);
+							pb[k].x = *(const unsigned *) (my_cols + soff + (VS + k) * PITCH);
+							pb[k].y = *(const unsigned *) (my_cols1 + soff + (VS + k) * PITCH);
+						}
+					}
+					__syncwarp();
+					if (lane0)
+						mbar_arrive(empty_s + 8u * s);
+					bool opaque = false;
+					if (OPQ && PREMUL && opq_on) {
+						if (opq_skip == 0) {
+							unsigned m = 0xffffffffu;
+#pragma unroll
+							for (int k = 0; k < VS; k++)
+								m &= pa[k].x & pa[k].y & pb[k].x & pb[k].y;
+							opaque = __all_sync(0xffffffffu, m >= 0xff000000u);
+							if (!opaque)
+								opq_skip = kV4OpaqueSkip;
+						}
+						else
+							opq_skip--;
+					}
+					if (opaque) {
+#pragma unroll
+						for (int k = 0; k < VS; k++) {
+							accumulate_pixel_h<false>(pa[k].x, k16, rb[2 * half][0], ga[2 * half][0]);
+							accumulate_pixel_h<false>(pa[k].y, k16, rb[2 * half][CPT - 1], ga[2 * half][CPT - 1]);
+							accumulate_pixel_h<false>(pb[k].x, k16, rb[2 * half + 1][0], ga[2 * half + 1][0]);
+							accumulate_pixel_h<false>(pb[k].y, k16, rb[2 * half + 1][CPT - 1], ga[2 * half + 1][CPT - 1]);
+						}
+					}
+					else {
+#pragma unroll
+						for (int k = 0; k < VS; k++) {
+							accumulate_pixel_h<PREMUL>(pa[k].x, k16, rb[2 * half][0], ga[2 * half][0]);
+							accumulate_pixel_h<PREMUL>(pa[k].y, k16, rb[2 * half][CPT - 1], ga[2 * half][CPT - 1]);
+							accumulate_pixel_h<PREMUL>(pb[k].x, k16, rb[2 * half + 1][0], ga[2 * half + 1][0]);
+							accumulate_pixel_h<PREMUL>(pb[k].y, k16, rb[2 * half + 1][CPT - 1], ga[2 * half + 1][CPT - 1]);
+						}
+					}
+					if (++s == S) {
+						s = 0;
+						phase ^= 1u;
+					}
+				}
+#pragma unroll
+				for (int i = 0; i < CPT; i++) {
+					if (!VPOW2) {
+						unsigned av[4][4];
+#pragma unroll
+						for (int r = 0; r < 4; r++) {
+							av[r][0] = __umulhi(rb[r][i] & 0xffffu, vmul8);
+							av[r][1] = __umulhi(rb[r][i] >> 16, vmul8);
+							av[r][2] = __umulhi(ga[r][i] & 0xffffu, vmul8);
+							av[r][3] = __umulhi(ga[r][i] >> 16, vmul8);
+						}
+						uint4 w;
+						w.x = __byte_perm(__byte_perm(av[0][0], av[1][0], 0x0040), __byte_perm(av[2][0], av[3][0], 0x0040), 0x5410);
+						w.y = __byte_perm(__byte_perm(av[0][2], av[1][2], 0x0040), __byte_perm(av[2][2], av[3][2], 0x0040), 0x5410);
+						w.z = __byte_perm(__byte_perm(av[0][1], av[1][1], 0x0040), __byte_perm(av[2][1], av[3][1], 0x0040), 0x5410);
+						w.w = __byte_perm(__byte_perm(av[0][3], av[1][3], 0x0040), __byte_perm(av[2][3], av[3][3], 0x0040), 0x5410);
+						*(uint4 *) (q_store + (size_t) (q & (kV4Quads - 1)) * QS + i * 16) = w;
+					}
+					else {
+#pragma unroll
+						for (int r = 0; r < 4; r++) {
+							rb[r][i] *= accm;
+							ga[r][i] *= accm;
+						}
+						const unsigned rb01 = __byte_perm(rb[0][i], rb[1][i], 0x7351);
+						const unsigned rb23 = __byte_perm(rb[2][i], rb[3][i], 0x7351);
+						const unsigned ga01 = __byte_perm(ga[0][i], ga[1][i], 0x7351);
+						const unsigned ga23 = __byte_perm(ga[2][i], ga[3][i], 0x7351);
+						uint4 w;
+						w.x = __byte_perm(rb01, rb23, 0x5410);
+						w.y = __byte_perm(ga01, ga23, 0x5410);
+						w.z = __byte_perm(rb01, rb23, 0x7632);
+						w.w = __byte_perm(ga01, ga23, 0x7632);
+						*(uint4 *) (q_store + (size_t) (q & (kV4Quads - 1)) * QS + i * 16) = w;
+					}
 				}
 			}
-#pragma unroll
-			for (int i = 0; i < CPT; i++) {
-				if (!VPOW2) {
-					unsigned av[4][4];
-#pragma unroll
-					for (int r = 0; r < 4; r++) {
-						av[r][0] = __umulhi(rb[r][i] & 0xffffu, vmul8);
-						av[r][1] = __umulhi(rb[r][i] >> 16, vmul8);
-						av[r][2] = __umulhi(ga[r][i] & 0xffffu, vmul8);
-						av[r][3] = __umulhi(ga[r][i] >> 16, vmul8);
-					}
-					uint4 w;
-					w.x = __byte_perm(__byte_perm(av[0][0], av[1][0], 0x0040), __byte_perm(av[2][0], av[3][0], 0x0040), 0x5410);
-					w.y = __byte_perm(__byte_perm(av[0][2], av[1][2], 0x0040), __byte_perm(av[2][2], av[3][2], 0x0040), 0x5410);
-					w.z = __byte_perm(__byte_perm(av[0][1], av[1][1], 0x0040), __byte_perm(av[2][1], av[3][1], 0x0040), 0x5410);
-					w.w = __byte_perm(__byte_perm(av[0][3], av[1][3], 0x0040), __byte_perm(av[2][3], av[3][3], 0x0040), 0x5410);
-					*(uint4 *) (q_store + (size_t) (q & (kV4Quads - 1)) * QS + i * 16) = w;
-				}
-				else {
-#pragma unroll
-					for (int r = 0; r < 4; r++) {
-						rb[r][i] *= accm;
-						ga[r][i] *= accm;
-					}
-					const unsigned rb01 = __byte_perm(rb[0][i], rb[1][i], 0x7351);
-					const unsigned rb23 = __byte_perm(rb[2][i], rb[3][i], 0x7351);
-					const unsigned ga01 = __byte_perm(ga[0][i], ga[1][i], 0x7351);
-					const unsigned ga23 = __byte_perm(ga[2][i], ga[3][i], 0x7351);
-					uint4 w;
-					w.x = __byte_perm(rb01, rb23, 0x5410);
-					w.y = __byte_perm(ga01, ga23, 0x5410);
-					w.z = __byte_perm(rb01, rb23, 0x7632);
-					w.w = __byte_perm(ga01, ga23, 0x7632);
-					*(uint4 *) (q_store + (size_t) (q & (kV4Quads - 1)) * QS + i * 16) = w;
+			qdone = max(qdone, q1 + 1);
+			__syncwarp();
+
+			const int buf = chunk & 1;
+			const uint4 bf = __ldg(&P.vbfrag[(size_t) cc * 32 + lane]);
+			mbar_wait(shempty_s + 8u * buf, ((unsigned) (chunk >> 1) & 1u) ^ 1u);
+			unsigned char *shb = (unsigned char *) (sh + (size_t) buf * KM * shs) + (size_t) (2 * tig) * shs * 8 + ch_off;
+			int bsum[2] = {0, 0};
+			int bcnt = 0, bidx = 0;
+#pragma unroll kMmaUnroll
+			for (int tp = 0; tp < 4 * CPT; tp++) {
+				unsigned a[2][4];
+				int dh[2][4], dl[2][4];
+#pragma unroll
+				for (int T = 0; T < 2; T++) {
+					const unsigned char *ap = a_base + tp * (HPOW2 ? 128 : 64) + T * 32;
+					a[T][0] = *(const unsigned *) (ap);
+					a[T][1] = *(const unsigned *) (ap + 16);
+					a[T][2] = *(const unsigned *) (ap + 4 * (size_t) QS);
+					a[T][3] = *(const unsigned *) (ap + 4 * (size_t) QS + 16);
+				}
+#pragma unroll
+				for (int T = 0; T < 2; T++) {
+#pragma unroll
+					for (int i = 0; i < 4; i++) {
+						dh[T][i] = 0;
+						dl[T][i] = VB200_INTERPOLATE_SCALE >> 1;
+					}
+					mma_u8s8(dh[T], a[T], bf.x, bf.y);
+					mma_u8u8(dl[T], a[T], bf.z, bf.w);
+				}
+#pragma unroll
+				for (int r = 0; r < 2; r++) {
+					const int v00 = v4_finish(dh[0][r], dl[0][r], k20);
+					const int v01 = v4_finish(dh[0][2 + r], dl[0][2 + r], k20);
+					const int v10 = v4_finish(dh[1][r], dl[1][r], k20);
+					const int v11 = v4_finish(dh[1][2 + r], dl[1][2 + r], k20);
+					if (!HPOW2)
+						continue;
+					if (HSQ == 2) {
+						const int sx = warp_sx0 + tp * 4 + 2 * jj;
+						unsigned char *d = shb + (size_t) r * shs * 8 + (sx >> 1) * 8;
+						d[0] = (unsigned char) ((v00 + v01 + 1) >> 1);
+						d[1] = (unsigned char) ((v10 + v11 + 1) >> 1);
+					}
+					else if (HSQ == 4) {
+						const int sx = warp_sx0 + tp * 2 + jj;
+						shb[(size_t) r * shs * 8 + (sx >> 1) * 8 + (sx & 1)] = (unsigned char) ((v00 + v01 + v10 + v11 + 2) >> 2);
+					}
+					else {
+						int sum = v00 + v01 + v10 + v11;
+						sum += __shfl_xor_sync(0xffffffffu, sum, 16);
+						const int sx = warp_sx0 + tp;
+						if (jj == 0)
+							shb[(size_t) r * shs * 8 + (sx >> 1) * 8 + (sx & 1)] = (unsigned char) ((sum + 4) >> HSHIFT);
+					}
+				}
+				if (!HPOW2) {
+#pragma unroll
+					for (int sl = 0; sl < 4; sl++) {
+						const int T = sl >> 1, h = sl & 1;
+						if (4 * tp + sl < G) {
+							bsum[0] += v4_finish(dh[T][2 * h], dl[T][2 * h], k20);
+							bsum[1] += v4_finish(dh[T][2 * h + 1], dl[T][2 * h + 1], k20);
+							if (++bcnt == HSQ) {
+								const int sx = warp_sx0 + bidx;
+								unsigned char *d = shb + (sx >> 1) * 8 + (sx & 1);
+								d[0] = (unsigned char) __umulhi((unsigned) (bsum[0] + HSQ / 2), hmul8);
+								d[(size_t) shs * 8] = (unsigned char) __umulhi((unsigned) (bsum[1] + HSQ / 2), hmul8);
+								bsum[0] = bsum[1] = 0;
+								bcnt = 0;
+								bidx++;
+							}
+						}
+					}
 				}
 			}
-		}
-		qdone = max(qdone, q1 + 1);
-		__syncwarp();
-
-		const int buf = chunk & 1;
-		const uint4 bf = __ldg(&P.vbfrag[(size_t) (chunk0 + chunk) * 32 + lane]);
-		mbar_wait(shempty_s + 8u * buf, ((unsigned) (chunk >> 1) & 1u) ^ 1u);
-		unsigned char *shb = (unsigned char *) (sh + (size_t) buf * KM * shs) + (size_t) (2 * tig) * shs * 8 + ch_off;
-		int bsum[2] = {0, 0};
-		int bcnt = 0, bidx = 0;
-#pragma unroll kMmaUnroll
-		for (int tp = 0; tp < 4 * CPT; tp++) {
-			unsigned a[2][4];
-			int dh[2][4], dl[2][4];
-#pragma unroll
-			for (int T = 0; T < 2; T++) {
-				const unsigned char *ap = a_base + tp * (HPOW2 ? 128 : 64) + T * 32;
-				a[T][0] = *(const unsigned *) (ap);
-				a[T][1] = *(const unsigned *) (ap + 16);
-				a[T][2] = *(const unsigned *) (ap + 4 * (size_t) QS);
-				a[T][3] = *(const unsigned *) (ap + 4 * (size_t) QS + 16);
-			}
-#pragma unroll
-			for (int T = 0; T < 2; T++) {
-#pragma unroll
-				for (int i = 0; i < 4; i++) {
-					dh[T][i] = 0;
-					dl[T][i] = VB200_INTERPOLATE_SCALE >> 1;
-				}
-				mma_u8s8(dh[T], a[T], bf.x, bf.y);
-				mma_u8u8(dl[T], a[T], bf.z, bf.w);
-			}
-#pragma unroll
-			for (int r = 0; r < 2; r++) {
-				const int v00 = v4_finish(dh[0][r], dl[0][r], k20);
-				const int v01 = v4_finish(dh[0][2 + r], dl[0][2 + r], k20);
-				const int v10 = v4_finish(dh[1][r], dl[1][r], k20);
-				const int v11 = v4_finish(dh[1][2 + r], dl[1][2 + r], k20);
-				if (!HPOW2)
-					continue;
-				if (HSQ == 2) {
-					const int sx = warp_sx0 + tp * 4 + 2 * jj;
-					unsigned char *d = shb + (size_t) r * shs * 8 + (sx >> 1) * 8;
-					d[0] = (unsigned char) ((v00 + v01 + 1) >> 1);
-					d[1] = (unsigned char) ((v10 + v11 + 1) >> 1);
-				}
-				else if (HSQ == 4) {
-					const int sx = warp_sx0 + tp * 2 + jj;
-					shb[(size_t) r * shs * 8 + (sx >> 1) * 8 + (sx & 1)] = (unsigned char) ((v00 + v01 + v10 + v11 + 2) >> 2);
-				}
-				else {
-					int sum = v00 + v01 + v10 + v11;
-					sum += __shfl_xor_sync(0xffffffffu, sum, 16);
-					const int sx = warp_sx0 + tp;
-					if (jj == 0)
-						shb[(size_t) r * shs * 8 + (sx >> 1) * 8 + (sx & 1)] = (unsigned char) ((sum + 4) >> HSHIFT);
-				}
-			}
-			if (!HPOW2) {
-#pragma unroll
-				for (int sl = 0; sl < 4; sl++) {
-					const int T = sl >> 1, h = sl & 1;
-					if (4 * tp + sl < G) {
-						bsum[0] += v4_finish(dh[T][2 * h], dl[T][2 * h], k20);
-						bsum[1] += v4_finish(dh[T][2 * h + 1], dl[T][2 * h + 1], k20);
-						if (++bcnt == HSQ) {
-							const int sx = warp_sx0 + bidx;
-							unsigned char *d = shb + (sx >> 1) * 8 + (sx & 1);
-							d[0] = (unsigned char) __umulhi((unsigned) (bsum[0] + HSQ / 2), hmul8);
-							d[(size_t) shs * 8] = (unsigned char) __umulhi((unsigned) (bsum[1] + HSQ / 2), hmul8);
-							bsum[0] = bsum[1] = 0;
-							bcnt = 0;
-							bidx++;
-						}
-					}
-				}
-			}
-		}
-		__syncwarp();
-		if (lane0)
-			mbar_arrive(shfull_s + 8u * buf);
+			__syncwarp();
+			if (lane0)
+				mbar_arrive(shfull_s + 8u * buf);
+		}
 	}
 }
```
